# icameling/lidar_camera_calibration

Hardware: AMD Instinct MI355X
Metric: chessboard-corner frames/sec + max corner error (mm), VLP-16 cloud (higher is better)
Workload: dtype f32

## Files before the change

### include/ilcc_hip.h

```cpp
#ifndef ILCC_HIP_H_
#define ILCC_HIP_H_

#include <stdint.h>

#ifdef __cplusplus
extern "C" {
#endif

#define ILCC_MAX_CORNERS 256
#define ILCC_ABI_VERSION 5

enum {
  ILCC_OK = 0,
  ILCC_NO_ROI_POINTS = 1,
  ILCC_NO_CLUSTER = 2,
  ILCC_NO_PLANE = 3,
  ILCC_DEGENERATE_HIST = 4,
  ILCC_TOO_FEW_POINTS = 5,
  ILCC_BAD_ARGUMENT = 6,
  ILCC_CAPACITY = 7,
  ILCC_HIP_ERROR = 8,
  ILCC_IO_ERROR = 9,
  ILCC_BOARD_NOT_FOUND = 10,
  ILCC_AMBIGUOUS = 11
};

enum {
  ILCC_FLAG_TIE_OVERFLOW = 1,
  ILCC_FLAG_REFINE_CAPPED = 2,
  ILCC_FLAG_BORDER_RISK = 8,
  ILCC_FLAG_LOW_COVERAGE = 4
};

enum {
  ILCC_SOLVER_REFERENCE_LOCAL = 0,
  ILCC_SOLVER_GRID = 1
};

enum {
  ILCC_CLOUD_ROI = 0,
  ILCC_CLOUD_CLUSTER = 1,
  ILCC_CLOUD_CHESSBOARD = 2,
  ILCC_CLOUD_PCA = 3,
  ILCC_CLOUD_OPTIM = 4
};

typedef struct ilcc_params {
  double roi_half[3];
  double cluster_tol;
  int32_t cluster_min;
  int32_t cluster_max;
  double ransac_thresh;
  int32_t ransac_hyp;
  uint32_t ransac_seed;
  int32_t hist_bins;
  double gray_rate;
  double huber_delta;
  double grid_length;
  int32_t board_w;
  int32_t board_h;
  int32_t solver;
  int32_t phase_mode;
  int32_t max_iterations;
  int32_t grid_prune;
  int32_t n_th, n_ty, n_tz;
  double th_min, th_step;
  double ty_min, ty_step;
  double tz_min, tz_step;
  int32_t refine_div;
  int32_t refine_max_rounds;
  int32_t refine_th_margin;
  int32_t reserved0;
  double ambiguity_eps;
  double online_cluster_tol;
  double min_cell_coverage;
  double ransac_probability;
} ilcc_params;


typedef struct ilcc_result {
  int32_t status;
  int32_t n_points;
  int32_t n_roi, n_cluster, n_plane;
  int32_t n_black, n_gray, n_white;
  int32_t n_corners;
  int32_t phase;
  int32_t iters_a, iters_b;
  int32_t grid_index;
  int32_t found_board;
  float grid_cost;
  float plane[4];
  float pca[16];
  double gray_zone[2];
  double theta_t[3];
  double cost_a, cost_b;
  double sel_cost;
  double basin_margin;
  int32_t flags;
  int32_t grid_ties;
  int32_t cells_hit;
  int32_t n_oob;
  float corners[ILCC_MAX_CORNERS * 3];
} ilcc_result;

typedef struct ilcc_handle ilcc_handle;

typedef struct ilcc_timing {
  float roi_crop, cluster, ransac_plane, plane_frame_hist, grid_cost, refine_corners, total;
  uint32_t grid_cost_launches;
  double grid_cost_ms_sum;
  uint64_t grid_cost_evals_sum;
  uint64_t grid_cost_evals_nominal_sum;
  uint64_t grid_cost_evals_interior_sum;
  uint64_t grid_cost_box_evals_sum;
  double grid_cost_kernel_ms_sum;
  double grid_cost_full_ms_sum;
  double walk_order_ms_sum;
  double grid_cost_prepass_ms_sum;
  double grid_cost_locate_ms_sum;
  uint64_t batches;
  double stage_ms_sum[7];
  double roi_count_ms_sum;
  uint64_t online_second_tier_frames;
} ilcc_timing;

int32_t ilcc_abi_version(void);
const char* ilcc_strerror(int32_t status);
const char* ilcc_last_error(const ilcc_handle* h);

void ilcc_default_params(ilcc_params* p);

int32_t ilcc_set_chessboard_param(ilcc_params* p, const char* cam_yaml);

ilcc_handle* ilcc_create(int32_t device, const ilcc_params* p, uint32_t max_frames,
                         uint64_t max_total_points);
void ilcc_destroy(ilcc_handle* h);
int32_t ilcc_set_params(ilcc_handle* h, const ilcc_params* p);
int32_t ilcc_reserve(ilcc_handle* h, uint32_t labelled_points_per_frame, uint32_t roi_points_per_frame);

int32_t ilcc_extract(ilcc_handle* h, const float* xyzi, uint32_t n, const float click[3],
                     ilcc_result* out);

int32_t ilcc_extract_batch(ilcc_handle* h, const float* xyzi, const uint64_t* offsets,
                           uint32_t n_frames, const float* clicks, ilcc_result* out);

int32_t ilcc_extract_batch_device(ilcc_handle* h, const float* d_xyzi, const uint64_t* offsets,
                                  uint32_t n_frames, const float* d_clicks, ilcc_result* out);

int32_t ilcc_submit_batch_device(ilcc_handle* h, const float* d_xyzi, const uint64_t* offsets,
                                 uint32_t n_frames, const float* d_clicks, int32_t* ticket);
int32_t ilcc_submit_batch(ilcc_handle* h, const float* xyzi, const uint64_t* offsets, uint32_t n_frames,
                          const float* clicks, int32_t* ticket);
int32_t ilcc_wait(ilcc_handle* h, int32_t ticket, ilcc_result* out);
#define ILCC_RECORD_HEADER 20
int32_t ilcc_wait_records_device(ilcc_handle* h, int32_t ticket, ilcc_result* out, void* d_records, uint32_t n_corners,
                                 uint32_t tag_base);

enum { ILCC_RESULTS_FULL = 0, ILCC_RESULTS_COMPACT = 1 };
int32_t ilcc_set_result_mode(ilcc_handle* h, int32_t mode);
int32_t ilcc_wait_compact(ilcc_handle* h, int32_t ticket, float* records, uint64_t capacity_floats);
uint32_t ilcc_record_floats(const ilcc_handle* h, int32_t ticket);
int32_t ilcc_fetch_results(ilcc_handle* h, uint32_t first, uint32_t n, ilcc_result* out);

int32_t ilcc_chessboard_by_point_batch(ilcc_handle* h, const float* xyzi, const uint64_t* offsets,
                                       uint32_t n_frames, const float* points, int32_t min_plane_points,
                                       ilcc_result* out);
int32_t ilcc_submit_chessboard_by_point(ilcc_handle* h, const float* xyzi, const uint64_t* offsets, uint32_t n_frames,
                                        const float* points, int32_t* ticket);
int32_t ilcc_wait_chessboard_by_point(ilcc_handle* h, int32_t ticket, int32_t min_plane_points, ilcc_result* out);
int64_t ilcc_fetch_classes(ilcc_handle* h, uint32_t frame, uint8_t* out_class, uint64_t cap_points);

int64_t ilcc_fetch_cloud(ilcc_handle* h, uint32_t frame, int32_t which, float* out_xyzi,
                         uint64_t cap_points);
int64_t ilcc_fetch_labelled(ilcc_handle* h, uint32_t frame, float* out_yz, uint8_t* out_label,
                            uint64_t cap_points);
int64_t ilcc_fetch_walk(ilcc_handle* h, uint32_t frame, float* out_yz, uint8_t* out_label, uint64_t cap_points,
                        uint32_t counts[2]);

int32_t ilcc_grid_cost(ilcc_handle* h, const float* yz, const uint8_t* label, uint32_t m,
                       int32_t use_oob, float* cost_out, int32_t* best_index, float* best_cost);

int32_t ilcc_grid_solve(ilcc_handle* h, const float* yz, const uint8_t* label, uint32_t m, int32_t* grid_index, float* grid_cost,
                        int32_t lat[3], int32_t* phase, int64_t* cost_q, int64_t* alt_cost_q, int32_t* rounds, int32_t* hops,
                        int32_t* flags, int32_t* ties);

int32_t ilcc_pattern_refine(ilcc_handle* h, const float* yz, const uint8_t* label, uint32_t m, int32_t lat[3],
                            int32_t* phase, int64_t* cost_q, int64_t* alt_cost_q, int32_t* rounds, int32_t* hops);

int32_t ilcc_get_theta_t(ilcc_handle* h, const float* yz, const uint8_t* label, uint32_t m,
                         int32_t topleft_white, int32_t use_oob, double theta_t[3], double* cost,
                         int32_t* iterations);

#define ILCC_SOLVE_REC_DOUBLES 6
#define ILCC_SOLVE_REC_INTS 4
int32_t ilcc_debug_reference_solve(ilcc_handle* h, const float* yz, const uint8_t* label, const uint64_t* offsets,
                                   const int32_t* status_in, uint32_t n_frames, double* rec_f64, int32_t* rec_i32,
                                   ilcc_result* results, uint32_t* lds_points);

#define ILCC_TIMELINE_COLS 15
int32_t ilcc_debug_timeline_enable(ilcc_handle* h, int32_t on);
int32_t ilcc_debug_timeline_fetch(ilcc_handle* h, double* rows, uint32_t cap_rows);

int32_t ilcc_debug_separate_launches(ilcc_handle* h, int32_t on);

#define ILCC_CLUSTER_HOME_RULE 0
#define ILCC_CLUSTER_HOME_LDS 1
#define ILCC_CLUSTER_HOME_L2 2
#define ILCC_CLUSTER_LAUNCH_WORDS 6
int32_t ilcc_debug_cluster_home(ilcc_handle* h, int32_t home);
int32_t ilcc_debug_cluster_launch(const ilcc_handle* h, uint32_t out[ILCC_CLUSTER_LAUNCH_WORDS]);

void ilcc_get_timing(const ilcc_handle* h, ilcc_timing* t);
void ilcc_reset_timing(ilcc_handle* h);

int32_t ilcc_save_corners2txt(const float* corners_xyz, uint32_t n_corners, const char* filename);
int32_t ilcc_read_lidar_corners(const char* filename, uint32_t num, double* out_xyz);

#ifdef __cplusplus
}
#endif
#endif
```

### lidar_camera_calibration_amd/_native.py

```python
from __future__ import annotations

import ctypes as C
import os

import numpy as np

_HERE = os.path.dirname(os.path.abspath(__file__))
LIB_PATH = os.environ.get("ILCC_HIP_LIB") or os.path.join(_HERE, "libilcc_hip.so")
MAX_CORNERS = 256

OK, NO_ROI_POINTS, NO_CLUSTER, NO_PLANE, DEGENERATE_HIST, TOO_FEW_POINTS, BAD_ARGUMENT, CAPACITY, \
    HIP_ERROR, IO_ERROR, BOARD_NOT_FOUND, AMBIGUOUS = range(12)
FLAG_TIE_OVERFLOW, FLAG_REFINE_CAPPED, FLAG_LOW_COVERAGE, FLAG_BORDER_RISK = 1, 2, 4, 8
FLAGS_FP32_ONLY = FLAG_TIE_OVERFLOW | FLAG_BORDER_RISK
RECORD_HEADER = 20
TIMELINE_COLS = 15
COST_Q_ONE = float(1 << 40)
SOLVER_REFERENCE_LOCAL, SOLVER_GRID = 0, 1
CLOUD_ROI, CLOUD_CLUSTER, CLOUD_CHESSBOARD, CLOUD_PCA, CLOUD_OPTIM = range(5)

EXPORTS = [
    "ilcc_abi_version", "ilcc_strerror", "ilcc_last_error", "ilcc_default_params",
    "ilcc_set_chessboard_param", "ilcc_create", "ilcc_destroy", "ilcc_set_params", "ilcc_reserve", "ilcc_extract",
    "ilcc_extract_batch", "ilcc_extract_batch_device", "ilcc_submit_batch_device", "ilcc_submit_batch", "ilcc_wait", "ilcc_wait_records_device", "ilcc_fetch_cloud", "ilcc_fetch_labelled", "ilcc_fetch_walk", "ilcc_chessboard_by_point_batch", "ilcc_submit_chessboard_by_point", "ilcc_wait_chessboard_by_point", "ilcc_fetch_classes",
    "ilcc_grid_cost", "ilcc_grid_solve", "ilcc_pattern_refine", "ilcc_get_theta_t", "ilcc_get_timing", "ilcc_reset_timing",
    "ilcc_save_corners2txt", "ilcc_read_lidar_corners",
    "ilcc_set_result_mode", "ilcc_wait_compact", "ilcc_record_floats", "ilcc_fetch_results",
    "ilcc_debug_timeline_enable", "ilcc_debug_timeline_fetch", "ilcc_debug_separate_launches",
    "ilcc_debug_cluster_home", "ilcc_debug_cluster_launch", "ilcc_debug_reference_solve",
]
ABI_VERSION = 5
RESULTS_FULL, RESULTS_COMPACT = 0, 1
CLUSTER_HOME_RULE, CLUSTER_HOME_LDS, CLUSTER_HOME_L2 = 0, 1, 2
CLUSTER_LAUNCH_WORDS = 6
SOLVE_REC_DOUBLES, SOLVE_REC_INTS = 6, 4


class Params(C.Structure):
    _fields_ = [
        ("roi_half", C.c_double * 3),
        ("cluster_tol", C.c_double),
        ("cluster_min", C.c_int32),
        ("cluster_max", C.c_int32),
        ("ransac_thresh", C.c_double),
        ("ransac_hyp", C.c_int32),
        ("ransac_seed", C.c_uint32),
        ("hist_bins", C.c_int32),
        ("gray_rate", C.c_double),
        ("huber_delta", C.c_double),
        ("grid_length", C.c_double),
        ("board_w", C.c_int32),
        ("board_h", C.c_int32),
        ("solver", C.c_int32),
        ("phase_mode", C.c_int32),
        ("max_iterations", C.c_int32),
        ("grid_prune", C.c_int32),
        ("n_th", C.c_int32), ("n_ty", C.c_int32), ("n_tz", C.c_int32),
        ("th_min", C.c_double), ("th_step", C.c_double),
        ("ty_min", C.c_double), ("ty_step", C.c_double),
        ("tz_min", C.c_double), ("tz_step", C.c_double),
        ("refine_div", C.c_int32), ("refine_max_rounds", C.c_int32),
        ("refine_th_margin", C.c_int32), ("reserved0", C.c_int32),
        ("ambiguity_eps", C.c_double),
        ("online_cluster_tol", C.c_double),
        ("min_cell_coverage", C.c_double),
        ("ransac_probability", C.c_double),
    ]


class Result(C.Structure):
    _fields_ = [
        ("status", C.c_int32),
        ("n_points", C.c_int32),
        ("n_roi", C.c_int32), ("n_cluster", C.c_int32), ("n_plane", C.c_int32),
        ("n_black", C.c_int32), ("n_gray", C.c_int32), ("n_white", C.c_int32),
        ("n_corners", C.c_int32),
        ("phase", C.c_int32),
        ("iters_a", C.c_int32), ("iters_b", C.c_int32),
        ("grid_index", C.c_int32),
        ("found_board", C.c_int32),
        ("grid_cost", C.c_float),
        ("plane", C.c_float * 4),
        ("pca", C.c_float * 16),
        ("gray_zone", C.c_double * 2),
        ("theta_t", C.c_double * 3),
        ("cost_a", C.c_double), ("cost_b", C.c_double),
        ("sel_cost", C.c_double),
        ("basin_margin", C.c_double),
        ("flags", C.c_int32),
        ("grid_ties", C.c_int32),
        ("cells_hit", C.c_int32),
        ("n_oob", C.c_int32),
        ("corners", C.c_float * (MAX_CORNERS * 3)),
    ]

    def corners_array(self) -> np.ndarray:
        return np.ctypeslib.as_array(self.corners)[:3 * self.n_corners].reshape(-1, 3).copy()


class Timing(C.Structure):
    _fields_ = [
        ("roi_crop", C.c_float), ("cluster", C.c_float), ("ransac_plane", C.c_float),
        ("plane_frame_hist", C.c_float), ("grid_cost", C.c_float), ("refine_corners", C.c_float),
        ("total", C.c_float),
        ("grid_cost_launches", C.c_uint32),
        ("grid_cost_ms_sum", C.c_double),
        ("grid_cost_evals_sum", C.c_uint64),
        ("grid_cost_evals_nominal_sum", C.c_uint64),
        ("grid_cost_evals_interior_sum", C.c_uint64),
        ("grid_cost_box_evals_sum", C.c_uint64),
        ("grid_cost_kernel_ms_sum", C.c_double),
        ("grid_cost_full_ms_sum", C.c_double),
        ("walk_order_ms_sum", C.c_double),
        ("grid_cost_prepass_ms_sum", C.c_double),
        ("grid_cost_locate_ms_sum", C.c_double),
        ("batches", C.c_uint64),
        ("stage_ms_sum", C.c_double * 7),
        ("roi_count_ms_sum", C.c_double),
        ("online_second_tier_frames", C.c_uint64),
    ]


_lib = None


def lib():
    global _lib
    if _lib is None:
        if not os.path.exists(LIB_PATH):
            raise OSError(f"{LIB_PATH} not found: build it with `python -c 'import __graft_entry__ as g; "
                          "g.build()'` (hipcc --offload-arch=gfx950); there is no CPU fallback")
        L = C.CDLL(LIB_PATH)
        vp, fp = C.c_void_p, C.POINTER(C.c_float)
        pp, rp = C.POINTER(Params), C.POINTER(Result)
        L.ilcc_abi_version.restype = C.c_int32
        got = L.ilcc_abi_version()
        if got != ABI_VERSION:
            raise OSError(f"{LIB_PATH} implements ABI {got}, this package declares ABI {ABI_VERSION}: rebuild it "
                          "(python -c 'import __graft_entry__ as g; g.build()')")
        L.ilcc_strerror.argtypes = [C.c_int32]
        L.ilcc_strerror.restype = C.c_char_p
        L.ilcc_last_error.argtypes = [vp]
        L.ilcc_last_error.restype = C.c_char_p
        L.ilcc_default_params.argtypes = [pp]
        L.ilcc_set_chessboard_param.argtypes = [pp, C.c_char_p]
        L.ilcc_set_chessboard_param.restype = C.c_int32
        L.ilcc_create.argtypes = [C.c_int32, pp, C.c_uint32, C.c_uint64]
        L.ilcc_create.restype = vp
        L.ilcc_destroy.argtypes = [vp]
        L.ilcc_set_params.argtypes = [vp, pp]
        L.ilcc_set_params.restype = C.c_int32
        L.ilcc_reserve.argtypes = [vp, C.c_uint32, C.c_uint32]
        L.ilcc_reserve.restype = C.c_int32
        L.ilcc_extract.argtypes = [vp, fp, C.c_uint32, fp, rp]
        L.ilcc_extract.restype = C.c_int32
        L.ilcc_extract_batch.argtypes = [vp, fp, C.POINTER(C.c_uint64), C.c_uint32, fp, rp]
        L.ilcc_extract_batch.restype = C.c_int32
        L.ilcc_extract_batch_device.argtypes = [vp, vp, C.POINTER(C.c_uint64), C.c_uint32, vp, rp]
        L.ilcc_extract_batch_device.restype = C.c_int32
        L.ilcc_submit_batch_device.argtypes = [vp, vp, C.POINTER(C.c_uint64), C.c_uint32, vp, C.POINTER(C.c_int32)]
        L.ilcc_submit_batch_device.restype = C.c_int32
        L.ilcc_submit_batch.argtypes = [vp, vp, C.POINTER(C.c_uint64), C.c_uint32, vp, C.POINTER(C.c_int32)]
        L.ilcc_submit_batch.restype = C.c_int32
        L.ilcc_wait.argtypes = [vp, C.c_int32, rp]
        L.ilcc_wait.restype = C.c_int32
        L.ilcc_wait_records_device.argtypes = [vp, C.c_int32, rp, vp, C.c_uint32, C.c_uint32]
        L.ilcc_wait_records_device.restype = C.c_int32
        L.ilcc_chessboard_by_point_batch.argtypes = [vp, fp, C.POINTER(C.c_uint64), C.c_uint32, fp, C.c_int32, rp]
        L.ilcc_chessboard_by_point_batch.restype = C.c_int32
        L.ilcc_submit_chessboard_by_point.argtypes = [vp, C.c_void_p, C.POINTER(C.c_uint64), C.c_uint32, C.c_void_p, C.POINTER(C.c_int32)]
        L.ilcc_submit_chessboard_by_point.restype = C.c_int32
        L.ilcc_wait_chessboard_by_point.argtypes = [vp, C.c_int32, C.c_int32, rp]
        L.ilcc_wait_chessboard_by_point.restype = C.c_int32
        L.ilcc_fetch_classes.argtypes = [vp, C.c_uint32, C.POINTER(C.c_uint8), C.c_uint64]
        L.ilcc_fetch_classes.restype = C.c_int64
        L.ilcc_fetch_cloud.argtypes = [vp, C.c_uint32, C.c_int32, fp, C.c_uint64]
        L.ilcc_fetch_cloud.restype = C.c_int64
        L.ilcc_fetch_labelled.argtypes = [vp, C.c_uint32, fp, C.POINTER(C.c_uint8), C.c_uint64]
        L.ilcc_fetch_labelled.restype = C.c_int64
        L.ilcc_fetch_walk.argtypes = [vp, C.c_uint32, fp, C.POINTER(C.c_uint8), C.c_uint64, C.POINTER(C.c_uint32)]
        L.ilcc_fetch_walk.restype = C.c_int64
        L.ilcc_grid_cost.argtypes = [vp, fp, C.POINTER(C.c_uint8), C.c_uint32, C.c_int32, fp,
                                     C.POINTER(C.c_int32), fp]
        L.ilcc_grid_cost.restype = C.c_int32
        L.ilcc_grid_solve.argtypes = [vp, fp, C.POINTER(C.c_uint8), C.c_uint32, C.POINTER(C.c_int32), fp, C.POINTER(C.c_int32),
                                      C.POINTER(C.c_int32), C.POINTER(C.c_int64), C.POINTER(C.c_int64), C.POINTER(C.c_int32),
                                      C.POINTER(C.c_int32), C.POINTER(C.c_int32), C.POINTER(C.c_int32)]
        L.ilcc_grid_solve.restype = C.c_int32
        L.ilcc_pattern_refine.argtypes = [vp, fp, C.POINTER(C.c_uint8), C.c_uint32, C.POINTER(C.c_int32),
                                          C.POINTER(C.c_int32), C.POINTER(C.c_int64), C.POINTER(C.c_int64),
                                          C.POINTER(C.c_int32), C.POINTER(C.c_int32)]
        L.ilcc_pattern_refine.restype = C.c_int32
        L.ilcc_get_theta_t.argtypes = [vp, fp, C.POINTER(C.c_uint8), C.c_uint32, C.c_int32, C.c_int32,
                                       C.POINTER(C.c_double), C.POINTER(C.c_double), C.POINTER(C.c_int32)]
        L.ilcc_get_theta_t.restype = C.c_int32
        L.ilcc_get_timing.argtypes = [vp, C.POINTER(Timing)]
        L.ilcc_reset_timing.argtypes = [vp]
        L.ilcc_save_corners2txt.argtypes = [fp, C.c_uint32, C.c_char_p]
        L.ilcc_save_corners2txt.restype = C.c_int32
        L.ilcc_read_lidar_corners.argtypes = [C.c_char_p, C.c_uint32, C.POINTER(C.c_double)]
        L.ilcc_read_lidar_corners.restype = C.c_int32
        L.ilcc_set_result_mode.argtypes = [vp, C.c_int32]
        L.ilcc_set_result_mode.restype = C.c_int32
        L.ilcc_wait_compact.argtypes = [vp, C.c_int32, fp, C.c_uint64]
        L.ilcc_wait_compact.restype = C.c_int32
        L.ilcc_record_floats.argtypes = [vp, C.c_int32]
        L.ilcc_record_floats.restype = C.c_uint32
        L.ilcc_debug_timeline_enable.argtypes = [vp, C.c_int32]
        L.ilcc_debug_timeline_enable.restype = C.c_int32
        L.ilcc_debug_timeline_fetch.argtypes = [vp, C.POINTER(C.c_double), C.c_uint32]
        L.ilcc_debug_timeline_fetch.restype = C.c_int32
        if hasattr(L, "ilcc_debug_separate_launches"):
            L.ilcc_debug_separate_launches.argtypes = [vp, C.c_int32]
            L.ilcc_debug_separate_launches.restype = C.c_int32
        if hasattr(L, "ilcc_debug_cluster_home"):
            L.ilcc_debug_cluster_home.argtypes = [vp, C.c_int32]
            L.ilcc_debug_cluster_home.restype = C.c_int32
            L.ilcc_debug_cluster_launch.argtypes = [vp, C.POINTER(C.c_uint32)]
            L.ilcc_debug_cluster_launch.restype = C.c_int32
        L.ilcc_debug_reference_solve.argtypes = [vp, fp, C.POINTER(C.c_uint8), C.POINTER(C.c_uint64), C.POINTER(C.c_int32), C.c_uint32,
                                                 C.POINTER(C.c_double), C.POINTER(C.c_int32), rp, C.POINTER(C.c_uint32)]
        L.ilcc_debug_reference_solve.restype = C.c_int32
        L.ilcc_fetch_results.argtypes = [vp, C.c_uint32, C.c_uint32, rp]
        L.ilcc_fetch_results.restype = C.c_int32
        _lib = L
    return _lib


def default_params() -> Params:
    p = Params()
    lib().ilcc_default_params(C.byref(p))
    return p


def strerror(status: int) -> str:
    return lib().ilcc_strerror(int(status)).decode()


def fptr(a: np.ndarray):
    return a.ctypes.data_as(C.POINTER(C.c_float))
```

### lidar_camera_calibration_amd/csrc/ilcc_api.cpp

```cpp
#include <hip/hip_runtime.h>

#include <array>
#include <cmath>
#include <cstdio>
#include <cstdlib>
#include <cstring>
#include <mutex>
#include <new>
#include <string>
#include <vector>

#include "ilcc_internal.h"
#include "k15_seed.h"
#include "k6_common.h"
#include "k7_common.h"

using namespace ilcc;

namespace ilcc {
bool params_ok(const ilcc_params& p, std::string& why);
}

#ifndef ILCC_SLOTS
#define ILCC_SLOTS 4
#endif
constexpr int kSlots = ILCC_SLOTS;
constexpr int kStreams = 3;

enum BatchEvent {
  kEvStart,
  kEvCropCounted,
  kEvCropped,
  kEvClustered,
  kEvPlane,
  kEvLabelled,
  kEvWalkOrdered,
  kEvSeeded,
  kEvRefined,
  kEvAnchored,
  kEvPrepassed,
  kEvFullStart,
  kEvSearched,
  kEvEnd,
  kEvCount
};
static_assert(kEvCount == ILCC_TIMELINE_COLS - 1, "a timeline row is the slot and one time per event");

enum BatchKind { kRoiPipeline, kByPoint };

struct Slot {
  hipEvent_t ev[kEvCount]{};
  hipEvent_t done = nullptr;
  hipEvent_t late = nullptr;
  hipEvent_t k6_done = nullptr;
  bool allocated = false;
  float4* d_xyzi = nullptr;
  float* d_clicks = nullptr;
  uint64_t* d_off = nullptr;
  ilcc_result* d_res = nullptr;
  float4 *d_roi = nullptr, *d_cluster = nullptr, *d_board = nullptr, *d_pca = nullptr, *d_optim = nullptr;
  float2 *d_yz = nullptr, *d_walk_yz = nullptr;
  uint8_t* d_walk_lab = nullptr;
  uint32_t *d_walk_mi = nullptr, *d_walk_nrim = nullptr;
  uint8_t *d_lab = nullptr, *d_cls = nullptr;
  uint32_t *d_nlab = nullptr, *d_walk = nullptr, *d_counts = nullptr, *d_parent = nullptr, *d_count = nullptr;
  unsigned long long* d_masks = nullptr;
  uint32_t *d_hash_head = nullptr, *d_hash_next = nullptr;
  uint32_t *d_flags = nullptr, *d_nfinite = nullptr, *d_counts_fin = nullptr;
  uint32_t* h_online = nullptr;
  uint32_t* d_list = nullptr;
  void* d_list_frames = nullptr;
  GridPartial *d_partial = nullptr, *d_partial2 = nullptr, *d_partial3 = nullptr, *d_partial4 = nullptr;
  SolveRec* d_solverec = nullptr;
  uint32_t *d_bound = nullptr, *d_bound_sub = nullptr;
  uint32_t* d_tie_count = nullptr;
  GridPartial* d_tie_list = nullptr;
  unsigned long long* d_iters = nullptr;
  uint32_t *d_grp_alive = nullptr, *d_grp_mask = nullptr;
  size_t grp_alive_cap = 0, grp_mask_cap = 0;
  float* h_rec_dev = nullptr;
  unsigned long long* h_iters_dev = nullptr;
  float* h_rec = nullptr;
  ilcc_result* h_res = nullptr;
  unsigned long long* h_iters = nullptr;
  uint64_t* h_off = nullptr;
  std::vector<uint64_t> off;
  uint32_t n_frames = 0;
  bool busy = false, grid = false;
  BatchKind kind = kRoiPipeline;
  bool h_res_valid = false;
  bool compact = false;
  uint32_t rec_corners = 0;
};

struct ilcc_handle {
  int device = 0;
  ilcc_params p{};
  uint32_t max_frames = 0;
  uint64_t max_points = 0;
  uint32_t max_theta = 0;
  uint32_t crop_chunks_cap = 0;
  Slot slots[kSlots];
  hipStream_t stream[kStreams]{};
  uint64_t seq = 0;
  uint64_t stream_last[kStreams]{};
  hipEvent_t entry_done = nullptr;
  int next_slot = 0;
  int last_slot = -1;
  int k6_last = -1;
  float *d_cth = nullptr, *d_sth = nullptr, *d_ay = nullptr, *d_az = nullptr;
  float *d_cth2 = nullptr, *d_sth2 = nullptr, *d_ay2 = nullptr, *d_az2 = nullptr;
  GridTables grid{}, seed_grid{};
  SeedMap seed_map{2, 12, 6};
  double2* d_th_lattice = nullptr;
  size_t th_lattice_cap = 0;
  int32_t th_lat_lo = 0, th_lat_hi = 0, hop_y = 0, hop_z = 0;
  double* d_solve = nullptr;
  RefineOut* d_refine_io = nullptr;
  uint32_t grid_lds_points = 1024;
  uint64_t group_prepass_skipped = 0;
  uint32_t cluster_lds_points = 2048;
  uint32_t cluster_cells_cap = kClusterCellsMin;
  uint32_t list_grid = 1024;
  bool poisoned = false;
  int32_t result_mode = ILCC_RESULTS_FULL;
  ilcc_timing timing{};
  hipEvent_t tl_ref = nullptr;
  bool tl_on = false;
  bool separate_launches = false;
  ClusterLimits cluster_limits{};
  int32_t cluster_home = kClusterHomeRule;
  ClusterLaunch cluster_last{};
  std::vector<double> tl_rows;
  std::string err;
};

namespace {

thread_local std::string g_err;

#define HIP_TRY(h, expr)                                                                   \
  do {                                                                                     \
    hipError_t e_ = (expr);                                                                \
    if (e_ != hipSuccess) {                                                                \
      (h)->err = std::string(#expr) + ": " + hipGetErrorString(e_);                        \
      return ILCC_HIP_ERROR;                                                               \
    }                                                                                      \
  } while (0)

#define ILCC_TRY(expr)                   \
  do {                                   \
    const int32_t st_ = (expr);          \
    if (st_ != ILCC_OK) return st_;      \
  } while (0)

int32_t near_zero_index(double vmin, double step, int32_t n) {
  long c = std::lround(-vmin / step);
  if (c < 0) c = 0;
  if (c > n - 1) c = n - 1;
  return (int32_t)c;
}

int32_t sync_own(ilcc_handle* h, hipStream_t s) {
  HIP_TRY(h, hipEventRecord(h->entry_done, s));
  HIP_TRY(h, hipEventSynchronize(h->entry_done));
  return ILCC_OK;
}

int32_t sync_all(ilcc_handle* h) {
  for (hipStream_t s : h->stream)
    if (s) HIP_TRY(h, hipStreamSynchronize(s));
  return ILCC_OK;
}

int32_t upload_tables(ilcc_handle* h) {
  const ilcc_params& p = h->p;
  if ((uint32_t)p.n_th > h->max_theta || (uint32_t)p.n_ty > h->max_theta || (uint32_t)p.n_tz > h->max_theta) {
    h->err = "grid axis longer than the handle's table capacity";
    return ILCC_CAPACITY;
  }
  hipStream_t st = h->stream[0];
  std::vector<float> cth(p.n_th), sth(p.n_th), ay(p.n_ty), az(p.n_tz);
  const double g = p.grid_length;
  for (int k = 0; k < p.n_th; ++k) {
    const double th = p.th_min + k * p.th_step;
    cth[k] = (float)(std::cos(th) / g);
    sth[k] = (float)(std::sin(th) / g);
  }
  for (int a = 0; a < p.n_ty; ++a) ay[a] = (float)(((p.ty_min + a * p.ty_step) + p.board_w * g / 2.0) / g);
  for (int b = 0; b < p.n_tz; ++b) az[b] = (float)(((p.tz_min + b * p.tz_step) + p.board_h * g / 2.0) / g);
  HIP_TRY(h, hipMemcpyAsync(h->d_cth, cth.data(), sizeof(float) * p.n_th, hipMemcpyHostToDevice, st));
  HIP_TRY(h, hipMemcpyAsync(h->d_sth, sth.data(), sizeof(float) * p.n_th, hipMemcpyHostToDevice, st));
  HIP_TRY(h, hipMemcpyAsync(h->d_ay, ay.data(), sizeof(float) * p.n_ty, hipMemcpyHostToDevice, st));
  HIP_TRY(h, hipMemcpyAsync(h->d_az, az.data(), sizeof(float) * p.n_tz, hipMemcpyHostToDevice, st));
#ifndef ILCC_SEED_THETAS
#define ILCC_SEED_THETAS 5
#endif
#ifndef ILCC_REFINE_RADIUS_DIV
#define ILCC_REFINE_RADIUS_DIV 3
#endif
  SeedMap& map = h->seed_map;
  map.stride_th = std::max(2, p.n_th / ILCC_SEED_THETAS);
  map.stride_t = std::max(1, std::min(p.n_ty, p.n_tz) / 8);
  map.off_th = map.stride_th / 2;
  std::vector<float> cth2, sth2, ay2, az2;
  for (int k = map.off_th; k < p.n_th; k += map.stride_th) {
    cth2.push_back(cth[k]);
    sth2.push_back(sth[k]);
  }
  for (int a = 0; a < p.n_ty; a += map.stride_t) ay2.push_back(ay[a]);
  for (int b = 0; b < p.n_tz; b += map.stride_t) az2.push_back(az[b]);
  GridTables& full = h->grid;
  full = GridTables{h->d_cth, h->d_sth, h->d_ay, h->d_az, p.n_th, p.n_ty, p.n_tz, near_zero_index(p.th_min, p.th_step, p.n_th),
                    near_zero_index(p.ty_min, p.ty_step, p.n_ty), near_zero_index(p.tz_min, p.tz_step, p.n_tz)};
  GridTables& seed = h->seed_grid;
  seed = GridTables{h->d_cth2, h->d_sth2, h->d_ay2, h->d_az2, (int32_t)cth2.size(), (int32_t)ay2.size(), (int32_t)az2.size(), 0, 0, 0};
  seed.c_th = std::min(std::max(full.c_th / map.stride_th, 0), seed.n_th - 1);
  seed.c_ty = std::min(full.c_ty / map.stride_t, seed.n_ty - 1);
  seed.c_tz = std::min(full.c_tz / map.stride_t, seed.n_tz - 1);
  if (seed.n_th > 0) {
    HIP_TRY(h, hipMemcpyAsync(h->d_cth2, cth2.data(), sizeof(float) * cth2.size(), hipMemcpyHostToDevice, st));
    HIP_TRY(h, hipMemcpyAsync(h->d_sth2, sth2.data(), sizeof(float) * sth2.size(), hipMemcpyHostToDevice, st));
    HIP_TRY(h, hipMemcpyAsync(h->d_ay2, ay2.data(), sizeof(float) * ay2.size(), hipMemcpyHostToDevice, st));
    HIP_TRY(h, hipMemcpyAsync(h->d_az2, az2.data(), sizeof(float) * az2.size(), hipMemcpyHostToDevice, st));
  }
  {
    const int div = p.refine_div > 0 ? p.refine_div : 1;
    h->th_lat_lo = -p.refine_th_margin * div;
    h->th_lat_hi = (p.n_th - 1 + p.refine_th_margin) * div;
    const size_t n = (size_t)(h->th_lat_hi - h->th_lat_lo) + 1;
    if (n > h->th_lattice_cap) {
      if (h->d_th_lattice) (void)hipFree(h->d_th_lattice);
      h->d_th_lattice = nullptr;
      h->th_lattice_cap = 0;
      HIP_TRY(h, hipMalloc((void**)&h->d_th_lattice, sizeof(double2) * n));
      h->th_lattice_cap = n;
    }
    std::vector<double2> tab(n);
    for (size_t i = 0; i < n; ++i) {
      const double th = p.th_min + (double)(h->th_lat_lo + (int64_t)i) * (p.th_step / (double)div);
      tab[i] = make_double2(std::cos(th), std::sin(th));
    }
    HIP_TRY(h, hipMemcpyAsync(h->d_th_lattice, tab.data(), sizeof(double2) * n, hipMemcpyHostToDevice, st));
    const int32_t sst = sync_own(h, st);
    if (sst != ILCC_OK) return sst;
    h->hop_y = (int32_t)std::lround(p.grid_length / (p.ty_step / (double)div));
    h->hop_z = (int32_t)std::lround(p.grid_length / (p.tz_step / (double)div));
  }
  return sync_own(h, st);
}

struct Buffer {
  void** ptr;
  size_t bytes;
};
template <class T>
Buffer buffer(T*& p, size_t count) { return {reinterpret_cast<void**>(&p), sizeof(T) * count}; }

auto handle_buffers(ilcc_handle* h) {
  const size_t mt = h->max_theta;
  return std::array{buffer(h->d_cth, mt),  buffer(h->d_sth, mt),  buffer(h->d_ay, mt),  buffer(h->d_az, mt),
                    buffer(h->d_cth2, mt), buffer(h->d_sth2, mt), buffer(h->d_ay2, mt), buffer(h->d_az2, mt),
                    buffer(h->d_solve, 8), buffer(h->d_refine_io, 1), buffer(h->d_th_lattice, 0) };
}

auto slot_device_buffers(const ilcc_handle* h, Slot& sl) {
  const size_t np = h->max_points, mf = h->max_frames, chunks = h->crop_chunks_cap, mt = h->max_theta;
  return std::array{
      buffer(sl.d_xyzi, np),
      buffer(sl.d_clicks, 3 * mf),
      buffer(sl.d_off, mf + 1),
      buffer(sl.d_res, mf),
      buffer(sl.d_roi, np),
      buffer(sl.d_cluster, np),
      buffer(sl.d_board, np),
      buffer(sl.d_pca, np),
      buffer(sl.d_optim, np),
      buffer(sl.d_yz, np),
      buffer(sl.d_walk_yz, np),
      buffer(sl.d_walk_lab, np),
      buffer(sl.d_walk_mi, mf),
      buffer(sl.d_walk_nrim, mf),
      buffer(sl.d_lab, np),
      buffer(sl.d_cls, np),
      buffer(sl.d_nlab, mf),
      buffer(sl.d_walk, mf),
      buffer(sl.d_counts, chunks),
      buffer(sl.d_counts_fin, chunks),
      buffer(sl.d_flags, mf),
      buffer(sl.d_nfinite, mf),
      buffer(sl.d_list, mf + 1),
      Buffer{&sl.d_list_frames, 64 * mf},
      buffer(sl.d_masks, chunks * (kCropChunk / 64)),
      buffer(sl.d_parent, np),
      buffer(sl.d_count, np),
      buffer(sl.d_hash_head, mf * kClusterHashSize),
      buffer(sl.d_hash_next, np),
      buffer(sl.d_partial, mf * mt),
      buffer(sl.d_partial2, mf * mt),
      buffer(sl.d_partial3, mf * mt),
      buffer(sl.d_partial4, mf * 4),
      buffer(sl.d_solverec, 2 * mf),
      buffer(sl.d_bound, mf),
      buffer(sl.d_bound_sub, mf),
      buffer(sl.d_tie_count, mf),
      buffer(sl.d_tie_list, mf * kTieCap),
      buffer(sl.d_iters, kBatchWords),
      buffer(sl.d_grp_alive, 0),
      buffer(sl.d_grp_mask, 0),
  };
}

auto slot_pinned_buffers(const ilcc_handle* h, Slot& sl) {
  const size_t mf = h->max_frames;
  return std::array{
      buffer(sl.h_res, mf),
      buffer(sl.h_rec, mf * (ILCC_RECORD_HEADER + 3 * ILCC_MAX_CORNERS)),
      buffer(sl.h_iters, kBatchWords),
      buffer(sl.h_off, mf + 1),
      buffer(sl.h_online, 2 * mf),
  };
}

struct SlotEvent {
  hipEvent_t* ev;
  unsigned flags;
};
auto slot_events(Slot& sl) {
  std::array<SlotEvent, kEvCount + 3> evs;
  for (int k = 0; k < kEvCount; ++k) evs[k] = {&sl.ev[k], hipEventDefault};
  evs[kEvCount] = {&sl.done, hipEventDisableTiming};
  evs[kEvCount + 1] = {&sl.late, hipEventDisableTiming};
  evs[kEvCount + 2] = {&sl.k6_done, hipEventDisableTiming};
  return evs;
}

void free_slot(const ilcc_handle* h, Slot& sl) {
  for (const Buffer& b : slot_device_buffers(h, sl))
    if (*b.ptr) (void)hipFree(*b.ptr);
  for (const Buffer& b : slot_pinned_buffers(h, sl))
    if (*b.ptr) (void)hipHostFree(*b.ptr);
  for (const SlotEvent& e : slot_events(sl))
    if (*e.ev) (void)hipEventDestroy(*e.ev);
  sl = Slot{};
}

void warn_hw_queues_once() {
  static std::once_flag once;
  std::call_once(once, [] {
    const char* v = std::getenv("GPU_MAX_HW_QUEUES");
    if (!v || std::atoi(v) >= kStreams + 1) return;
    std::fprintf(stderr,
                 "libilcc_hip: GPU_MAX_HW_QUEUES=%s: with fewer than %d hardware queues two of the handle's stage streams "
                 "(or one and the host's stream) share a queue and serialise (the library does not modify the "
                 "environment)\n", v, kStreams + 1);
  });
}

struct GroupPrepassPlan {
  bool box = false;
  bool on = false;
  uint32_t groups = 0, words = 0;
};
GroupPrepassPlan group_prepass_plan(const ilcc_params& p) {
  GroupPrepassPlan g;
  const bool box = p.grid_prune != 0 && 3.0 * p.ty_step < 0.9 * p.grid_length && 3.0 * p.tz_step < 0.9 * p.grid_length;
  const double gl = p.grid_length;
  const double ty_hi = p.ty_min + (p.n_ty - 1) * p.ty_step, tz_hi = p.tz_min + (p.n_tz - 1) * p.tz_step;
  const bool centre_in = p.ty_min > -0.45 * p.board_w * gl && ty_hi < 0.45 * p.board_w * gl && p.tz_min > -0.45 * p.board_h * gl &&
                         tz_hi < 0.45 * p.board_h * gl;
  const uint32_t n_tiles = (uint32_t)grid_tiles(p.n_ty, p.n_tz);
  g.box = box;
  g.on = box && p.n_th >= kThetaGroup && centre_in && n_tiles <= (uint32_t)kBoxTilesMax;
  g.groups = (uint32_t)((p.n_th + kThetaGroup - 1) / kThetaGroup);
  g.words = (n_tiles + 31u) / 32u;
  return g;
}

int32_t size_group_prepass(ilcc_handle* h, Slot& sl) {
  const GroupPrepassPlan g = group_prepass_plan(h->p);
  if (!g.on) return ILCC_OK;
  const size_t need_alive = (size_t)h->max_frames * g.groups, need_mask = need_alive * g.words;
  if (need_alive > sl.grp_alive_cap) {
    if (sl.d_grp_alive) (void)hipFree(sl.d_grp_alive);
    sl.d_grp_alive = nullptr;
    sl.grp_alive_cap = 0;
    HIP_TRY(h, hipMalloc((void**)&sl.d_grp_alive, sizeof(uint32_t) * need_alive));
    sl.grp_alive_cap = need_alive;
  }
  if (need_mask > sl.grp_mask_cap) {
    if (sl.d_grp_mask) (void)hipFree(sl.d_grp_mask);
    sl.d_grp_mask = nullptr;
    sl.grp_mask_cap = 0;
    HIP_TRY(h, hipMalloc((void**)&sl.d_grp_mask, sizeof(uint32_t) * need_mask));
    sl.grp_mask_cap = need_mask;
  }
  return ILCC_OK;
}

int32_t alloc_slot_parts(ilcc_handle* h, Slot& sl) {
  for (const SlotEvent& e : slot_events(sl)) HIP_TRY(h, hipEventCreateWithFlags(e.ev, e.flags));
  for (const Buffer& b : slot_device_buffers(h, sl))
    if (b.bytes) HIP_TRY(h, hipMalloc(b.ptr, b.bytes));
  for (const Buffer& b : slot_pinned_buffers(h, sl)) HIP_TRY(h, hipHostMalloc(b.ptr, b.bytes, hipHostMallocDefault));
  HIP_TRY(h, hipHostGetDevicePointer((void**)&sl.h_rec_dev, sl.h_rec, 0));
  HIP_TRY(h, hipHostGetDevicePointer((void**)&sl.h_iters_dev, sl.h_iters, 0));
  return size_group_prepass(h, sl);
}

int32_t alloc_slot(ilcc_handle* h, Slot& sl) {
  if (sl.allocated) return ILCC_OK;
  const int32_t st = alloc_slot_parts(h, sl);
  if (st != ILCC_OK) {
    free_slot(h, sl);
    return st;
  }
  sl.allocated = true;
  return ILCC_OK;
}

Ctx make_ctx(ilcc_handle* h, Slot& sl, const float4* d_xyzi, const float* d_clicks, uint32_t n_frames,
             uint32_t crop_chunks) {
  Ctx c{};
  c.xyzi = d_xyzi;
  c.off = sl.d_off;
  c.clicks = d_clicks;
  c.n_frames = n_frames;
  c.crop_chunks = crop_chunks;
  c.res = sl.d_res;
  c.roi = sl.d_roi;
  c.cluster = sl.d_cluster;
  c.board = sl.d_board;
  c.pca = sl.d_pca;
  c.optim = sl.d_optim;
  c.yz = sl.d_yz;
  c.lab = sl.d_lab;
  c.cls = sl.d_cls;
  c.n_lab = sl.d_nlab;
  c.walk_stride = sl.d_walk;
  c.walk_yz = sl.d_walk_yz;
  c.walk_lab = sl.d_walk_lab;
  c.walk_mi = sl.d_walk_mi;
  c.walk_nrim = sl.d_walk_nrim;
  c.crop_counts = sl.d_counts;
  c.crop_masks = sl.d_masks;
  c.uf_parent = sl.d_parent;
  c.uf_count = sl.d_count;
  c.uf_hash_head = sl.d_hash_head;
  c.uf_hash_next = sl.d_hash_next;
  c.cluster_lds_points = h->cluster_lds_points;
  c.cluster_cells_cap = h->cluster_cells_cap;
  c.wide = 0u;
  c.cluster_bits = cluster_bits_default();
  c.online_tier = 0u;
  c.online_window = 0.f;
  c.frame_flags = sl.d_flags;
  c.n_finite = sl.d_nfinite;
  c.crop_fin = sl.d_counts_fin;
  c.list_count = sl.d_list;
  c.list = sl.d_list + 1;
  c.list_frames = sl.d_list_frames;
  c.list_grid = h->list_grid;
  c.partial = sl.d_partial;
  c.solve_rec = sl.d_solverec;
  c.grid_blocks = (uint32_t)h->p.n_th;
  c.grid_lds_points = h->grid_lds_points;
  c.grid_bound = sl.d_bound;
  c.grid_bound_sub = sl.d_bound_sub;
  c.tie_count = sl.d_tie_count;
  c.tie_list = sl.d_tie_list;
  c.grid_iters = sl.d_iters;
  c.grid = h->grid;
  c.th_lattice = h->d_th_lattice;
  c.th_lat_lo = h->th_lat_lo;
  c.th_lat_hi = h->th_lat_hi;
  c.refine_hop_y = h->hop_y;
  c.refine_hop_z = h->hop_z;
  c.p = h->p;
  return c;
}

int32_t check_offsets(ilcc_handle* h, const uint64_t* offsets, uint32_t n_frames) {
  if (!offsets || n_frames == 0) {
    h->err = "no frames";
    return ILCC_BAD_ARGUMENT;
  }
  if (n_frames > h->max_frames) {
    h->err = "n_frames exceeds the handle's max_frames";
    return ILCC_CAPACITY;
  }
  if (offsets[0] != 0) {
    h->err = "offsets[0] must be 0";
    return ILCC_BAD_ARGUMENT;
  }
  for (uint32_t f = 0; f < n_frames; ++f)
    if (offsets[f + 1] < offsets[f] || offsets[f + 1] - offsets[f] > 0x7FFFFFFFull) {
      h->err = "offsets must be non-decreasing, frames < 2^31 points";
      return ILCC_BAD_ARGUMENT;
    }
  if (offsets[n_frames] > h->max_points) {
    h->err = "total points exceed the handle's max_total_points";
    return ILCC_CAPACITY;
  }
  return ILCC_OK;
}

int take_stream(ilcc_handle* h) {
  const int k = (int)(h->seq % kStreams);
  h->stream_last[k] = ++h->seq;
  return k;
}

hipStream_t late_stream(const ilcc_handle* h) {
  int best = 0;
  for (int k = 1; k < kStreams; ++k)
    if (h->stream_last[k] < h->stream_last[best]) best = k;
  return h->stream[best];
}

void fit_cluster_lds(ilcc_handle* h) {
  while (cluster_lds_bytes(h->cluster_lds_points, h->cluster_cells_cap, cluster_bits_online()) > (size_t)kClusterLdsMax && h->cluster_lds_points > 0)
    h->cluster_lds_points = h->cluster_lds_points > 512u ? h->cluster_lds_points - 512u : 0u;
}

uint32_t board_corners(const ilcc_params& p) { return (uint32_t)((p.board_w - 1) * (p.board_h - 1)); }
size_t trimmed_bytes(uint32_t n_corners) { return offsetof(ilcc_result, corners) + sizeof(float) * 3 * (size_t)n_corners; }

hipError_t copy_results_trimmed(ilcc_result* dst, const ilcc_result* d_src, uint32_t n_frames, uint32_t n_corners, hipStream_t s) {
  if (n_frames == 0) return hipSuccess;
  return hipMemcpy2DAsync(dst, sizeof(ilcc_result), d_src, sizeof(ilcc_result), trimmed_bytes(n_corners), n_frames,
                          hipMemcpyDeviceToHost, s);
}

#ifndef ILCC_SEED_POINTS
#define ILCC_SEED_POINTS 128
#endif
#ifndef ILCC_BOX_POINTS
#define ILCC_BOX_POINTS 48
#endif
constexpr int kAnchorRadius = 1;
#ifndef ILCC_ANCHOR_ROUNDS
#define ILCC_ANCHOR_ROUNDS 2
#endif
constexpr int kAnchorRounds = ILCC_ANCHOR_ROUNDS;


GridPass whole_grid_pass(const Ctx& c, const GridTables& t, GridPartial* out) {
  GridPass g{};
  g.t = t;
  g.out = out;
  g.blocks = (uint32_t)t.n_th;
  g.bound = c.grid_bound;
  return g;
}

GridSeed full_table_records(const GridPartial* records, uint32_t blocks) { return GridSeed{records, blocks, SeedMap{1, 1, 0}}; }

GridPass seed_pass(const ilcc_handle* h, const Slot& sl, const Ctx& c) {
  GridPass g = whole_grid_pass(c, h->seed_grid, sl.d_partial2);
  g.walk_limit = (uint32_t)ILCC_SEED_POINTS;
  g.bound = c.grid_bound_sub;
  return g;
}

GridPass refine_pass(const ilcc_handle* h, const Slot& sl, const Ctx& c, int32_t refine_radius) {
  GridPass g = whole_grid_pass(c, h->grid, sl.d_partial3);
  g.seed = GridSeed{sl.d_partial2, (uint32_t)h->seed_grid.n_th, h->seed_map};
  g.window_tiles = h->seed_map.stride_t > 2 * kTile ? 4 : 2;
  g.radius_th = (refine_radius / kRefineThetaStride) * kRefineThetaStride;
  g.step_th = kRefineThetaStride;
  g.blocks = std::min((uint32_t)(2 * (g.radius_th / kRefineThetaStride) + 1), h->max_theta);
  g.walk_limit = (uint32_t)ILCC_SEED_POINTS;
  g.bound = c.grid_bound_sub;
  return g;
}

GridPass anchor_pass(const ilcc_handle* h, const Ctx& c, const GridSeed& seed, GridPartial* out) {
  GridPass g = whole_grid_pass(c, h->grid, out);
  g.seed = seed;
  g.radius_th = kAnchorRadius;
  g.blocks = 2 * kAnchorRadius + 1;
  return g;
}

GridPass full_pass(const ilcc_handle* h, const Ctx& c, const GridSeed& seed) {
  GridPass g = whole_grid_pass(c, h->grid, c.partial);
  g.seed = seed;
  g.collect_ties = 1u;
  return g;
}

LocatePlan locate_plan(const ilcc_handle* h, const Slot& sl, const Ctx& c) {
  LocatePlan lp{};
  lp.seed = h->seed_grid;
  lp.map = h->seed_map;
  lp.refine_radius = std::max(1, h->seed_map.stride_th / ILCC_REFINE_RADIUS_DIV);
  lp.sample_min = (uint32_t)ILCC_SEED_POINTS;
  lp.sample_cap = std::max((uint32_t)ILCC_SEED_POINTS, ((c.grid_lds_points >> 3) + 63u) & ~63u);
  lp.out = sl.d_partial4;
  return lp;
}

int32_t enqueue_locate_launches(ilcc_handle* h, Slot& sl, const Ctx& c, hipStream_t s, int32_t refine_radius, GridSeed& located) {
  launch_grid_cost(c, seed_pass(h, sl, c), s, 1, nullptr, true);
  HIP_TRY(h, hipEventRecord(sl.ev[kEvSeeded], s));
  const GridPass refine = refine_pass(h, sl, c, refine_radius);
  launch_grid_cost(c, refine, s, 1, nullptr, true);
  HIP_TRY(h, hipEventRecord(sl.ev[kEvRefined], s));
  located = full_table_records(refine.out, refine.blocks);
  GridPartial* const ping[2] = {sl.d_partial4, sl.d_partial2};
  for (int round = 0; round < kAnchorRounds; ++round) {
    const GridPass anchor = anchor_pass(h, c, located, ping[round & 1]);
    launch_anchor(c, anchor, s);
    located = full_table_records(anchor.out, anchor.blocks);
  }
  return ILCC_OK;
}

int32_t enqueue_grid_search(ilcc_handle* h, Slot& sl, const Ctx& c, hipStream_t s, uint32_t n_frames, bool chain, bool walk_laid_out = false) {
  const bool prune = h->p.grid_prune != 0;
  if (!walk_laid_out) launch_walk_order(c, s);
  HIP_TRY(h, hipEventRecord(sl.ev[kEvWalkOrdered], s));
  GridSeed located{};
  if (h->seed_grid.n_th > 0 && h->p.n_th >= 8 && h->p.n_ty >= 8 && h->p.n_tz >= 8) {
    const LocatePlan lp = locate_plan(h, sl, c);
    const bool fused = n_frames >= (uint32_t)kLocateMinFrames && lp.seed.n_th <= 16 &&
                       locate_lds_bytes(lp.sample_cap, h->grid.n_ty, h->grid.n_tz, lp.seed.n_ty, lp.seed.n_tz) <= (size_t)kLocateLdsMax;
    if (fused) {
      launch_locate(c, s, lp);
      HIP_TRY(h, hipEventRecord(sl.ev[kEvSeeded], s));
      HIP_TRY(h, hipEventRecord(sl.ev[kEvRefined], s));
      located = full_table_records(lp.out, 1);
    } else {
      ILCC_TRY(enqueue_locate_launches(h, sl, c, s, lp.refine_radius, located));
    }
  } else {
    HIP_TRY(h, hipEventRecord(sl.ev[kEvSeeded], s));
    HIP_TRY(h, hipEventRecord(sl.ev[kEvRefined], s));
  }
  HIP_TRY(h, hipEventRecord(sl.ev[kEvAnchored], s));
  GridPass full = full_pass(h, c, located);
  const GroupPrepassPlan gp = group_prepass_plan(h->p);
  full.box_points = gp.box ? (uint32_t)ILCC_BOX_POINTS : 0u;
  if (full.box_points != 0u && gp.on && (size_t)n_frames * gp.groups <= sl.grp_alive_cap &&
      (size_t)n_frames * gp.groups * gp.words <= sl.grp_mask_cap) {
    full.grp_alive = sl.d_grp_alive;
    full.grp_mask = sl.d_grp_mask;
    full.grp_count = gp.groups;
    full.grp_words = gp.words;
    launch_group_prepass(c, full, s);
  } else if (full.box_points != 0u && gp.on) {
    if (h->group_prepass_skipped++ == 0) h->err = "note: k6_group_prepass skipped (mask buffers smaller than this batch needs): slower, results unaffected";
  }
  HIP_TRY(h, hipEventRecord(sl.ev[kEvPrepassed], s));
  const int si = (int)(&sl - h->slots);
  if (chain && h->k6_last >= 0 && h->k6_last != si && h->slots[h->k6_last].busy)
    HIP_TRY(h, hipStreamWaitEvent(s, h->slots[h->k6_last].k6_done, 0));
  HIP_TRY(h, hipEventRecord(sl.ev[kEvFullStart], s));
  launch_grid_cost(c, full, s, 1, nullptr, prune);
  if (chain) {
    HIP_TRY(h, hipEventRecord(sl.k6_done, s));
    h->k6_last = si;
  }
  return ILCC_OK;
}

int32_t enqueue_impl(ilcc_handle* h, int si, hipStream_t s, const float4* d_xyzi, const uint64_t* offsets, uint32_t n_frames,
                     const float* d_clicks, BatchKind kind) {
  Slot& sl = h->slots[si];
  uint64_t max_n = 0;
  for (uint32_t f = 0; f < n_frames; ++f) max_n = std::max<uint64_t>(max_n, offsets[f + 1] - offsets[f]);
  uint32_t chunks = (uint32_t)((max_n + kCropChunk - 1) / kCropChunk);
  if (chunks == 0) chunks = 1;
  if ((uint64_t)chunks * n_frames > (uint64_t)h->crop_chunks_cap) {
    h->err = "crop chunk table too small for this (very ragged) batch";
    return ILCC_CAPACITY;
  }
  sl.off.assign(offsets, offsets + n_frames + 1);
  sl.n_frames = n_frames;
  std::memcpy(sl.h_off, sl.off.data(), sizeof(uint64_t) * (n_frames + 1));
  HIP_TRY(h, hipMemcpyAsync(sl.d_off, sl.h_off, sizeof(uint64_t) * (n_frames + 1), hipMemcpyHostToDevice, s));
  Ctx c = make_ctx(h, sl, d_xyzi, d_clicks, n_frames, chunks);
  HIP_TRY(h, hipEventRecord(sl.ev[kEvStart], s));
  if (kind == kRoiPipeline) {
    launch_roi_crop(c, s, sl.ev[kEvCropCounted], !h->separate_launches && n_frames >= (uint32_t)kCropFrameMinFrames);
    HIP_TRY(h, hipEventRecord(sl.ev[kEvCropped], s));
    h->cluster_last = launch_cluster(c, s, h->cluster_limits, h->cluster_home);
  } else {
    c.p.cluster_tol = c.p.online_cluster_tol;
    c.wide = 1u;
    Ctx t1 = c;
    t1.online_tier = 1u;
    t1.online_window = 1.25f;
    t1.p.roi_half[0] = t1.p.roi_half[1] = t1.p.roi_half[2] = (double)t1.online_window;
    t1.cluster_bits = cluster_bits_online();
    launch_roi_crop(t1, s, sl.ev[kEvCropCounted]);
    HIP_TRY(h, hipEventRecord(sl.ev[kEvCropped], s));
    h->cluster_last = launch_cluster(t1, s, h->cluster_limits, h->cluster_home);
    Ctx t2 = c;
    t2.online_tier = 2u;
    t2.p.roi_half[0] = t2.p.roi_half[1] = t2.p.roi_half[2] = (double)INFINITY;
    launch_roi_crop(t2, s, nullptr);
    (void)launch_cluster(t2, s, h->cluster_limits, h->cluster_home);
    HIP_TRY(h, hipMemcpyAsync(sl.h_online, sl.d_flags, sizeof(uint32_t) * n_frames, hipMemcpyDeviceToHost, s));
    HIP_TRY(h, hipMemcpyAsync(sl.h_online + h->max_frames, sl.d_nfinite, sizeof(uint32_t) * n_frames, hipMemcpyDeviceToHost, s));
  }
  HIP_TRY(h, hipEventRecord(sl.ev[kEvClustered], s));
  sl.grid = kind == kRoiPipeline && h->p.solver == ILCC_SOLVER_GRID;
  const bool one_launch = !h->separate_launches && front_end_fusable(c);
  if (one_launch) {
    launch_front_end(c, s, sl.grid);
    HIP_TRY(h, hipEventRecord(sl.ev[kEvPlane], s));
  } else {
    launch_ransac_plane(c, s);
    HIP_TRY(h, hipEventRecord(sl.ev[kEvPlane], s));
    launch_plane_frame_hist(c, s);
  }
  HIP_TRY(h, hipEventRecord(sl.ev[kEvLabelled], s));
  if (sl.grid) {
    ILCC_TRY(enqueue_grid_search(h, sl, c, s, n_frames, true, one_launch));
  }
  HIP_TRY(h, hipEventRecord(sl.ev[kEvSearched], s));
  if (kind == kRoiPipeline) {
    if (sl.grid) {
      launch_pattern_refine(c, s);
    } else {
      launch_reference_solve(c, s);
    }
    launch_corners(c, s, solve_slots(c.p));
  }
  HIP_TRY(h, hipEventRecord(sl.ev[kEvEnd], s));
  HIP_TRY(h, hipGetLastError());
  sl.compact = h->result_mode == ILCC_RESULTS_COMPACT;
  sl.rec_corners = board_corners(h->p);
  if (sl.compact) {
    launch_pack_records(sl.d_res, n_frames, sl.rec_corners, 0u, sl.h_rec_dev, s);
  } else {
    HIP_TRY(h, copy_results_trimmed(sl.h_res, sl.d_res, n_frames, sl.rec_corners, s));
  }
  launch_store_to_host(sl.d_iters, sl.h_iters_dev, sizeof(unsigned long long) * kBatchWords, s);
  HIP_TRY(h, hipGetLastError());
  HIP_TRY(h, hipEventRecord(sl.done, s));
  sl.busy = true;
  sl.kind = kind;
  return ILCC_OK;
}

int32_t enqueue(ilcc_handle* h, int si, hipStream_t s, const float4* d_xyzi, const uint64_t* offsets, uint32_t n_frames,
                const float* d_clicks, BatchKind kind) {
  if (h->poisoned) {
    h->err = "handle unusable: a failed ilcc_set_params could not restore the device tables";
    return ILCC_HIP_ERROR;
  }
  const int32_t st = enqueue_impl(h, si, s, d_xyzi, offsets, n_frames, d_clicks, kind);
  if (st != ILCC_OK) {
    const std::string why = h->err;
    (void)hipStreamSynchronize(s);
    (void)hipGetLastError();
    h->slots[si].busy = false;
    h->err = why;
  }
  return st;
}

int32_t run_late(ilcc_handle* h, Slot& sl, hipStream_t s) {
  HIP_TRY(h, hipEventRecord(sl.late, s));
  HIP_TRY(h, hipEventSynchronize(sl.late));
  return ILCC_OK;
}

int32_t ensure_full(ilcc_handle* h, Slot& sl) {
  if (sl.h_res_valid) return ILCC_OK;
  const hipStream_t s = late_stream(h);
  HIP_TRY(h, copy_results_trimmed(sl.h_res, sl.d_res, sl.n_frames, sl.rec_corners, s));
  ILCC_TRY(run_late(h, sl, s));
  sl.h_res_valid = true;
  return ILCC_OK;
}


int32_t wait_batch(ilcc_handle* h, Slot& sl, bool want_compact, float* d_records, uint32_t n_corners, uint32_t tag_base) {
  HIP_TRY(h, hipSetDevice(h->device));
  HIP_TRY(h, hipEventSynchronize(sl.done));
  const bool pack_now = want_compact && !sl.compact;
  const hipStream_t ls = late_stream(h);
  if (d_records) launch_pack_records(sl.d_res, sl.n_frames, n_corners, tag_base, d_records, ls);
  if (pack_now) launch_pack_records(sl.d_res, sl.n_frames, sl.rec_corners, 0u, sl.h_rec_dev, ls);
  if (d_records || pack_now) {
    ILCC_TRY(run_late(h, sl, ls));
  }
  sl.busy = false;
  sl.h_res_valid = !sl.compact;
  h->last_slot = (int)(&sl - h->slots);
  return ILCC_OK;
}

size_t record_floats(const Slot& sl) { return (size_t)ILCC_RECORD_HEADER + 3 * (size_t)sl.rec_corners; }

int32_t hand_over(ilcc_handle* h, Slot& sl, ilcc_result* out, float* out_compact) {
  if (out) {
    ILCC_TRY(ensure_full(h, sl));
    const size_t row = trimmed_bytes(sl.rec_corners);
    for (uint32_t f = 0; f < sl.n_frames; ++f) std::memcpy(&out[f], &sl.h_res[f], row);
  }
  if (out_compact) std::memcpy(out_compact, sl.h_rec, sizeof(float) * sl.n_frames * record_floats(sl));
  return ILCC_OK;
}

struct BatchCounts {
  uint32_t max_lab = 0, max_roi = 0;
  uint64_t evals = 0;
};
BatchCounts count_batch(const ilcc_handle* h, const Slot& sl) {
  BatchCounts n;
  for (uint32_t f = 0; f < sl.n_frames; ++f) {
    int32_t status, n_roi;
    uint32_t m;
    if (sl.h_res_valid) {
      const ilcc_result& r = sl.h_res[f];
      status = r.status;
      n_roi = r.n_roi;
      m = (uint32_t)(r.n_black + r.n_white);
    } else {
      const float* r = sl.h_rec + (size_t)f * record_floats(sl);
      status = (int32_t)r[0];
      n_roi = (int32_t)r[19];
      m = (uint32_t)r[13] + (uint32_t)r[14];
    }
    if (n_roi > 0 && (uint32_t)n_roi <= (uint32_t)kClusterLdsPointsMax) n.max_roi = std::max(n.max_roi, (uint32_t)n_roi);
    if (status != ILCC_OK && status != ILCC_AMBIGUOUS) continue;
    n.max_lab = std::max(n.max_lab, m);
    n.evals += (uint64_t)m * (uint64_t)h->p.n_th * h->p.n_ty * h->p.n_tz;
  }
  return n;
}

int32_t account_timing(ilcc_handle* h, const Slot& sl, uint64_t evals) {
  auto span = [&](BatchEvent from, BatchEvent to, float& ms_out) { return hipEventElapsedTime(&ms_out, sl.ev[from], sl.ev[to]); };
  float ms[6];
  const BatchEvent stage[7] = {kEvStart, kEvCropped, kEvClustered, kEvPlane, kEvLabelled, kEvSearched, kEvEnd};
  for (int k = 0; k < 6; ++k) HIP_TRY(h, span(stage[k], stage[k + 1], ms[k]));
  float k6k[6] = {0.f, 0.f, 0.f, 0.f, 0.f, 0.f};
  if (sl.grid) {
    const BatchEvent part[6] = {kEvLabelled, kEvWalkOrdered, kEvSeeded, kEvRefined, kEvAnchored, kEvPrepassed};
    for (int k = 0; k < 5; ++k) HIP_TRY(h, span(part[k], part[k + 1], k6k[k]));
    HIP_TRY(h, span(kEvFullStart, kEvSearched, k6k[5]));
    float pre = 0.f;
    HIP_TRY(h, span(kEvLabelled, kEvPrepassed, pre));
    ms[4] = pre + k6k[5];
  }
  float tot = 0;
  HIP_TRY(h, span(kEvStart, kEvEnd, tot));
  if (h->tl_on && h->tl_ref && sl.grid) {
    h->tl_rows.push_back((double)(&sl - h->slots));
    for (hipEvent_t e : sl.ev) {
      float t = 0.f;
      HIP_TRY(h, hipEventElapsedTime(&t, h->tl_ref, e));
      h->tl_rows.push_back((double)t);
    }
  }
  ilcc_timing& t = h->timing;
  t.roi_crop = ms[0];
  t.cluster = ms[1];
  t.ransac_plane = ms[2];
  t.plane_frame_hist = ms[3];
  t.grid_cost = ms[4];
  t.refine_corners = ms[5];
  t.total = tot;
  t.batches += 1;
  for (int k = 0; k < 6; ++k) t.stage_ms_sum[k] += ms[k];
  t.stage_ms_sum[6] += tot;
  {
    float cnt = 0.f;
    HIP_TRY(h, span(kEvStart, kEvCropCounted, cnt));
    t.roi_count_ms_sum += cnt;
  }
  if (sl.grid) {
    t.grid_cost_launches += 1;
    t.grid_cost_ms_sum += ms[4];
    t.walk_order_ms_sum += k6k[0];
    t.grid_cost_kernel_ms_sum += (double)k6k[1] + k6k[2] + k6k[3] + k6k[4] + k6k[5];
    t.grid_cost_locate_ms_sum += (double)k6k[1] + k6k[2] + k6k[3];
    t.grid_cost_prepass_ms_sum += k6k[4];
    t.grid_cost_full_ms_sum += k6k[5];
    t.grid_cost_evals_nominal_sum += evals;
    unsigned long long iters = 0;
    unsigned long long iters_in = 0;
    for (int k = 0; k < kIterSlots; ++k) {
      iters += sl.h_iters[k];
      iters_in += sl.h_iters[kIterSlots + k];
      t.grid_cost_box_evals_sum += sl.h_iters[2 * kIterSlots + k];
    }
    t.grid_cost_evals_sum += (uint64_t)iters * grid_cost_evals_per_count();
    t.grid_cost_evals_interior_sum += (uint64_t)iters_in * grid_cost_evals_per_count();
  }
  return ILCC_OK;
}

uint32_t lds_capacity(uint32_t need, uint32_t step, uint32_t lo, uint32_t hi) {
  return std::min(hi, std::max(lo, (need + step - 1u) & ~(step - 1u)));
}
uint32_t grid_lds_capacity(uint32_t labelled_points) { return lds_capacity(labelled_points, 256u, 1024u, (uint32_t)kGridLdsPointsMax); }
uint32_t cluster_lds_capacity(uint32_t roi_points, uint32_t lo) { return lds_capacity(roi_points, 512u, lo, (uint32_t)kClusterLdsPointsMax); }
uint32_t cluster_cells_capacity(uint64_t cells) {
  const uint32_t need = (uint32_t)std::min<uint64_t>(cells, (uint64_t)kClusterCellsMax);
  return lds_capacity(need, 256u, (uint32_t)kClusterCellsMin, (uint32_t)kClusterCellsMax);
}
void raise_capacities(ilcc_handle* h, uint32_t grid_points, uint32_t cluster_points, uint32_t cluster_cells) {
  h->grid_lds_points = std::max(h->grid_lds_points, grid_points);
  h->cluster_lds_points = std::max(h->cluster_lds_points, cluster_points);
  h->cluster_cells_cap = std::max(h->cluster_cells_cap, cluster_cells);
  fit_cluster_lds(h);
}

constexpr int kGridStaticLds = 3072;
constexpr uint32_t grid_points_two_per_cu(int n_ty, int n_tz) {
  const int64_t room = (int64_t)kCuLdsBytes / 2 - kGridStaticLds - (int64_t)grid_lds_bytes(0, n_ty, n_tz);
  return room > 0 ? (uint32_t)(room / (int64_t)grid_lds_bytes(1, 0, 0)) & ~255u : 0u;
}
static_assert(grid_points_two_per_cu(40, 40) == 6400, "BASELINE config 2 (the default grid: 40 x 40 translations)");
static_assert(grid_points_two_per_cu(129, 129) == 6400, "BASELINE config 5 (129 x 129 translations)");
void grow_capacities(ilcc_handle* h, const BatchCounts& n, uint64_t cells_needed) {
  const uint32_t two_per_cu = grid_points_two_per_cu(h->p.n_ty, h->p.n_tz);
  raise_capacities(h, std::min(grid_lds_capacity(n.max_lab), std::max(1024u, two_per_cu)), cluster_lds_capacity(n.max_roi, 0u),
                   cluster_cells_capacity(cells_needed + cells_needed / 8));
}

int32_t finish(ilcc_handle* h, Slot& sl, ilcc_result* out, float* out_compact = nullptr, float* d_records = nullptr,
               uint32_t n_corners = 0, uint32_t tag_base = 0) {
  ILCC_TRY(wait_batch(h, sl, out_compact != nullptr, d_records, n_corners, tag_base));
  ILCC_TRY(hand_over(h, sl, out, out_compact));
  const BatchCounts n = count_batch(h, sl);
  ILCC_TRY(account_timing(h, sl, n.evals));
  grow_capacities(h, n, sl.h_iters[3 * kIterSlots]);
  return ILCC_OK;
}

int32_t run_batch(ilcc_handle* h, BatchKind kind, bool on_device, const float* xyzi, const uint64_t* offsets, uint32_t n_frames,
                  const float* clicks, int32_t* ticket, ilcc_result* out) {
  HIP_TRY(h, hipSetDevice(h->device));
  ILCC_TRY(check_offsets(h, offsets, n_frames));
  const int si = ticket ? h->next_slot : 0;
  Slot& sl = h->slots[si];
  if (sl.busy) {
    h->err = ticket ? "every pipeline slot holds a batch: wait for the oldest ticket first" : "synchronous call while ticket 0 is in flight";
    return ticket ? ILCC_CAPACITY : ILCC_BAD_ARGUMENT;
  }
  if (ticket) ILCC_TRY(alloc_slot(h, sl));
  const hipStream_t s = h->stream[take_stream(h)];
  if (!on_device) {
    if (offsets[n_frames] > 0)
      HIP_TRY(h, hipMemcpyAsync(sl.d_xyzi, xyzi, sizeof(float4) * offsets[n_frames], hipMemcpyHostToDevice, s));
    HIP_TRY(h, hipMemcpyAsync(sl.d_clicks, clicks, sizeof(float) * 3 * n_frames, hipMemcpyHostToDevice, s));
    xyzi = reinterpret_cast<const float*>(sl.d_xyzi);
    clicks = sl.d_clicks;
  }
  ILCC_TRY(enqueue(h, si, s, reinterpret_cast<const float4*>(xyzi), offsets, n_frames, clicks, kind));
  if (!ticket) return finish(h, sl, out);
  *ticket = si;
  h->next_slot = (si + 1) % kSlots;
  return ILCC_OK;
}


const Slot* busy_slot(const ilcc_handle* h, int32_t ticket) {
  return h && ticket >= 0 && ticket < kSlots && h->slots[ticket].busy ? &h->slots[ticket] : nullptr;
}

Slot* ticket_slot(ilcc_handle* h, int32_t ticket, const char* fn, BatchKind kind, bool args_ok) {
  if (!h) return nullptr;
  Slot* sl = const_cast<Slot*>(busy_slot(h, ticket));
  if (!args_ok || !sl) {
    h->err = std::string(fn) + ": bad argument or no batch in flight under this ticket";
    return nullptr;
  }
  if (sl->kind != kind) {
    h->err = std::string(fn) + (sl->kind == kByPoint ? ": this ticket came from ilcc_submit_chessboard_by_point: wait with ilcc_wait_chessboard_by_point"
                                                     : ": this ticket came from ilcc_submit_batch[_device]: wait with ilcc_wait / ilcc_wait_compact / ilcc_wait_records_device");
    return nullptr;
  }
  return sl;
}

bool any_batch_in_flight(ilcc_handle* h, const char* fn) {
  for (const Slot& sl : h->slots)
    if (sl.busy) {
      h->err = std::string(fn) + " with a batch in flight: ilcc_wait first";
      return true;
    }
  return false;
}

void finish_chessboard_by_point(ilcc_handle* h, Slot& sl, uint32_t n_frames, int32_t min_plane_points, ilcc_result* out) {
  for (uint32_t f = 0; f < n_frames; ++f)
    if (sl.h_online[f] == 0u && out[f].status != ILCC_NO_ROI_POINTS) out[f].n_roi = (int32_t)sl.h_online[h->max_frames + f];
  for (uint32_t f = 0; f < n_frames; ++f) h->timing.online_second_tier_frames += sl.h_online[f] != 0u ? 1u : 0u;
  for (uint32_t f = 0; f < n_frames; ++f)
    if (out[f].status == ILCC_OK && (out[f].n_plane < min_plane_points || !out[f].found_board)) {
      out[f].status = ILCC_BOARD_NOT_FOUND;
      sl.h_res[f].status = ILCC_BOARD_NOT_FOUND;
    }
}


int32_t fetch_slot(ilcc_handle* h, uint32_t first, uint32_t n, Slot*& slot) {
  if (!h || h->last_slot < 0) return ILCC_BAD_ARGUMENT;
  Slot& sl = h->slots[h->last_slot];
  if (sl.busy || first > sl.n_frames || n > sl.n_frames - first) {
    h->err = "fetch: no completed batch, or the frames asked for exceed it";
    return ILCC_BAD_ARGUMENT;
  }
  HIP_TRY(h, hipSetDevice(h->device));
  slot = &sl;
  return ILCC_OK;
}

int64_t fetch_labelled_points(const float2* d_yz, const uint8_t* d_lab, uint32_t n, float* out_yz, uint8_t* out_label, uint64_t cap_points) {
  const uint64_t m = std::min<uint64_t>(n, cap_points);
  if (m > 0 && ((out_yz && hipMemcpy(out_yz, d_yz, sizeof(float2) * m, hipMemcpyDeviceToHost) != hipSuccess) ||
                (out_label && hipMemcpy(out_label, d_lab, m, hipMemcpyDeviceToHost) != hipSuccess)))
    return -(int64_t)ILCC_HIP_ERROR;
  return (int64_t)n;
}

int32_t stage_labelled(ilcc_handle* h, hipStream_t s, const float* yz, const uint8_t* label, uint32_t m) {
  if (!h || (m > 0 && (!yz || !label))) return ILCC_BAD_ARGUMENT;
  if (m > h->max_points) {
    h->err = "more points than the handle holds";
    return ILCC_CAPACITY;
  }
  Slot& sl = h->slots[0];
  if (sl.busy) {
    h->err = "diagnostic entry while ticket 0 is in flight";
    return ILCC_BAD_ARGUMENT;
  }
  HIP_TRY(h, hipSetDevice(h->device));
  const uint64_t off[2] = {0, m};
  ilcc_result r;
  std::memset(&r, 0, sizeof(r));
  r.status = ILCC_OK;
  HIP_TRY(h, hipMemcpyAsync(sl.d_off, off, sizeof(off), hipMemcpyHostToDevice, s));
  HIP_TRY(h, hipMemcpyAsync(sl.d_res, &r, sizeof(r), hipMemcpyHostToDevice, s));
  HIP_TRY(h, hipMemcpyAsync(sl.d_nlab, &m, sizeof(m), hipMemcpyHostToDevice, s));
  const uint32_t stride = walk_stride(m);
  HIP_TRY(h, hipMemcpyAsync(sl.d_walk, &stride, sizeof(stride), hipMemcpyHostToDevice, s));
  if (m > 0) {
    HIP_TRY(h, hipMemcpyAsync(sl.d_yz, yz, sizeof(float2) * m, hipMemcpyHostToDevice, s));
    HIP_TRY(h, hipMemcpyAsync(sl.d_lab, label, m, hipMemcpyHostToDevice, s));
  }
  ILCC_TRY(sync_own(h, s));
  sl.n_frames = 0;
  return ILCC_OK;
}

Ctx diagnostic_ctx(ilcc_handle* h, Slot& sl, uint32_t m) {
  Ctx c = make_ctx(h, sl, nullptr, nullptr, 1, 1);
  uint32_t lds = 1024;
  while (lds < m && lds < (uint32_t)kGridLdsPointsMax) lds <<= 1;
  c.grid_lds_points = std::max(c.grid_lds_points, lds);
  return c;
}

}

namespace ilcc {
void set_global_error(const std::string& s) { g_err = s; }
HandleView handle_view(const ilcc_handle* h) { return HandleView{h->device, h->p, h->max_frames, h->max_points}; }
int32_t handle_fail(ilcc_handle* h, int32_t code, const std::string& what) {
  h->err = what;
  return code;
}
}

extern "C" {

const char* ilcc_last_error(const ilcc_handle* h) { return h ? h->err.c_str() : g_err.c_str(); }

ilcc_handle* ilcc_create(int32_t device, const ilcc_params* p, uint32_t max_frames, uint64_t max_total_points) {
  g_err.clear();
  int ndev = 0;
  if (hipGetDeviceCount(&ndev) != hipSuccess || ndev == 0) {
    g_err = "no HIP device: libilcc_hip has no CPU fallback";
    return nullptr;
  }
  if (!p || max_frames == 0 || max_total_points == 0) {
    g_err = "bad arguments to ilcc_create";
    return nullptr;
  }
  std::string why;
  if (!params_ok(*p, why)) {
    g_err = why;
    return nullptr;
  }
  ilcc_handle* h = new (std::nothrow) ilcc_handle();
  if (!h) return nullptr;
  h->p = *p;
  h->max_frames = max_frames;
  h->max_points = max_total_points;
  h->max_theta = 4096;
  h->crop_chunks_cap =
      (uint32_t)std::min<uint64_t>(0xFFFFFFFFull, max_total_points / kCropChunk + (uint64_t)max_frames + 1);
  auto fail = [&](const std::string& what) {
    g_err = what;
    ilcc_destroy(h);
    return (ilcc_handle*)nullptr;
  };
  hipError_t e;
  if (device >= 0) {
    if ((e = hipSetDevice(device)) != hipSuccess) return fail(std::string("hipSetDevice: ") + hipGetErrorString(e));
    h->device = device;
  } else {
    (void)hipGetDevice(&h->device);
  }
  {
    int cus = 0;
    if (hipDeviceGetAttribute(&cus, hipDeviceAttributeMultiprocessorCount, h->device) == hipSuccess && cus > 0)
      h->list_grid = (uint32_t)(4 * cus);
  }
  if ((e = set_kernel_attributes_k2()) != hipSuccess || (e = set_kernel_attributes_k6()) != hipSuccess ||
      (e = set_kernel_attributes_k7a()) != hipSuccess || (e = set_kernel_attributes_k7r()) != hipSuccess)
    return fail(std::string("hipFuncSetAttribute(MaxDynamicSharedMemorySize): ") + hipGetErrorString(e));
  if ((e = cluster_limits(h->device, &h->cluster_limits)) != hipSuccess)
    return fail(std::string("cluster_limits: ") + hipGetErrorString(e));
  for (const Buffer& b : handle_buffers(h))
    if (b.bytes && (e = hipMalloc(b.ptr, b.bytes)) != hipSuccess) return fail(std::string("hipMalloc: ") + hipGetErrorString(e));
  warn_hw_queues_once();
  for (hipStream_t& s : h->stream)
    if ((e = hipStreamCreateWithFlags(&s, hipStreamNonBlocking)) != hipSuccess)
      return fail(std::string("hipStreamCreateWithFlags: ") + hipGetErrorString(e));
  if ((e = hipEventCreateWithFlags(&h->entry_done, hipEventDisableTiming)) != hipSuccess)
    return fail(std::string("hipEventCreateWithFlags: ") + hipGetErrorString(e));
  if (alloc_slot(h, h->slots[0]) != ILCC_OK) return fail(h->err);
  if (upload_tables(h) != ILCC_OK) return fail(h->err);
  return h;
}

void ilcc_destroy(ilcc_handle* h) {
  if (!h) return;
  for (hipStream_t s : h->stream)
    if (s) (void)hipStreamSynchronize(s);
  for (Slot& sl : h->slots) free_slot(h, sl);
  for (hipStream_t s : h->stream)
    if (s) (void)hipStreamDestroy(s);
  for (const Buffer& b : handle_buffers(h))
    if (*b.ptr) (void)hipFree(*b.ptr);
  if (h->tl_ref) (void)hipEventDestroy(h->tl_ref);
  if (h->entry_done) (void)hipEventDestroy(h->entry_done);
  delete h;
}

int32_t ilcc_set_params(ilcc_handle* h, const ilcc_params* p) {
  if (!h || !p) return ILCC_BAD_ARGUMENT;
  std::string why;
  if (!params_ok(*p, why)) {
    h->err = why;
    return ILCC_BAD_ARGUMENT;
  }
  if (any_batch_in_flight(h, "ilcc_set_params")) return ILCC_BAD_ARGUMENT;
  ILCC_TRY(sync_all(h));
  const ilcc_params old = h->p;
  h->p = *p;
  int32_t st = upload_tables(h);
  for (Slot& sl : h->slots)
    if (st == ILCC_OK && sl.allocated) st = size_group_prepass(h, sl);
  if (st != ILCC_OK) {
    const std::string why = h->err;
    h->p = old;
    if (upload_tables(h) != ILCC_OK) h->poisoned = true;
    h->err = why;
  }
  return st;
}

int32_t ilcc_reserve(ilcc_handle* h, uint32_t labelled_points_per_frame, uint32_t roi_points_per_frame) {
  if (!h || any_batch_in_flight(h, "ilcc_reserve")) return ILCC_BAD_ARGUMENT;
  raise_capacities(h, grid_lds_capacity(labelled_points_per_frame), cluster_lds_capacity(roi_points_per_frame, (uint32_t)kClusterLdsPointsMin),
                   cluster_cells_capacity(roi_points_per_frame / 4u));
  return ILCC_OK;
}

int32_t ilcc_set_result_mode(ilcc_handle* h, int32_t mode) {
  if (!h || (mode != ILCC_RESULTS_FULL && mode != ILCC_RESULTS_COMPACT) || any_batch_in_flight(h, "ilcc_set_result_mode")) return ILCC_BAD_ARGUMENT;
  h->result_mode = mode;
  return ILCC_OK;
}


int32_t ilcc_submit_batch_device(ilcc_handle* h, const float* d_xyzi, const uint64_t* offsets, uint32_t n_frames,
                                 const float* d_clicks, int32_t* ticket) {
  if (!h || !d_xyzi || !d_clicks || !ticket) return ILCC_BAD_ARGUMENT;
  return run_batch(h, kRoiPipeline, true, d_xyzi, offsets, n_frames, d_clicks, ticket, nullptr);
}

int32_t ilcc_submit_batch(ilcc_handle* h, const float* xyzi, const uint64_t* offsets, uint32_t n_frames, const float* clicks,
                          int32_t* ticket) {
  if (!h || !xyzi || !clicks || !ticket) return ILCC_BAD_ARGUMENT;
  return run_batch(h, kRoiPipeline, false, xyzi, offsets, n_frames, clicks, ticket, nullptr);
}

int32_t ilcc_extract_batch_device(ilcc_handle* h, const float* d_xyzi, const uint64_t* offsets,
                                  uint32_t n_frames, const float* d_clicks, ilcc_result* out) {
  if (!h || !d_xyzi || !d_clicks || !out) return ILCC_BAD_ARGUMENT;
  return run_batch(h, kRoiPipeline, true, d_xyzi, offsets, n_frames, d_clicks, nullptr, out);
}

int32_t ilcc_extract_batch(ilcc_handle* h, const float* xyzi, const uint64_t* offsets, uint32_t n_frames,
                           const float* clicks, ilcc_result* out) {
  if (!h || !xyzi || !clicks || !out) return ILCC_BAD_ARGUMENT;
  return run_batch(h, kRoiPipeline, false, xyzi, offsets, n_frames, clicks, nullptr, out);
}

int32_t ilcc_extract(ilcc_handle* h, const float* xyzi, uint32_t n, const float click[3], ilcc_result* out) {
  const uint64_t off[2] = {0, n};
  return ilcc_extract_batch(h, xyzi, off, 1, click, out);
}

int32_t ilcc_chessboard_by_point_batch(ilcc_handle* h, const float* xyzi, const uint64_t* offsets, uint32_t n_frames,
                                       const float* points, int32_t min_plane_points, ilcc_result* out) {
  if (!h || !xyzi || !points || !out) return ILCC_BAD_ARGUMENT;
  ILCC_TRY(run_batch(h, kByPoint, false, xyzi, offsets, n_frames, points, nullptr, out));
  finish_chessboard_by_point(h, h->slots[0], n_frames, min_plane_points, out);
  return ILCC_OK;
}

int32_t ilcc_submit_chessboard_by_point(ilcc_handle* h, const float* xyzi, const uint64_t* offsets, uint32_t n_frames,
                                        const float* points, int32_t* ticket) {
  if (!h || !xyzi || !points || !ticket) return ILCC_BAD_ARGUMENT;
  return run_batch(h, kByPoint, false, xyzi, offsets, n_frames, points, ticket, nullptr);
}


int32_t ilcc_wait(ilcc_handle* h, int32_t ticket, ilcc_result* out) {
  Slot* sl = ticket_slot(h, ticket, "ilcc_wait", kRoiPipeline, out != nullptr);
  return sl ? finish(h, *sl, out) : ILCC_BAD_ARGUMENT;
}

int32_t ilcc_wait_records_device(ilcc_handle* h, int32_t ticket, ilcc_result* out, void* d_records, uint32_t n_corners,
                                 uint32_t tag_base) {
  Slot* sl = ticket_slot(h, ticket, "ilcc_wait_records_device", kRoiPipeline, d_records && n_corners <= ILCC_MAX_CORNERS);
  return sl ? finish(h, *sl, out, nullptr, static_cast<float*>(d_records), n_corners, tag_base) : ILCC_BAD_ARGUMENT;
}

uint32_t ilcc_record_floats(const ilcc_handle* h, int32_t ticket) {
  const Slot* sl = busy_slot(h, ticket);
  return sl ? (uint32_t)record_floats(*sl) : 0u;
}

int32_t ilcc_wait_compact(ilcc_handle* h, int32_t ticket, float* records, uint64_t capacity_floats) {
  Slot* sl = ticket_slot(h, ticket, "ilcc_wait_compact", kRoiPipeline, records != nullptr);
  if (!sl) return ILCC_BAD_ARGUMENT;
  const uint64_t need = (uint64_t)sl->n_frames * record_floats(*sl);
  if (capacity_floats < need) {
    h->err = "ilcc_wait_compact: the batch's records need " + std::to_string(need) + " floats, the buffer holds " +
             std::to_string(capacity_floats) + " (the batch stays in flight)";
    return ILCC_BAD_ARGUMENT;
  }
  return finish(h, *sl, nullptr, records);
}

int32_t ilcc_wait_chessboard_by_point(ilcc_handle* h, int32_t ticket, int32_t min_plane_points, ilcc_result* out) {
  Slot* sl = ticket_slot(h, ticket, "ilcc_wait_chessboard_by_point", kByPoint, out != nullptr);
  if (!sl) return ILCC_BAD_ARGUMENT;
  ILCC_TRY(finish(h, *sl, out));
  finish_chessboard_by_point(h, *sl, sl->n_frames, min_plane_points, out);
  return ILCC_OK;
}


int32_t ilcc_fetch_results(ilcc_handle* h, uint32_t first, uint32_t n, ilcc_result* out) {
  Slot* slp = nullptr;
  ILCC_TRY(out ? fetch_slot(h, first, n, slp) : ILCC_BAD_ARGUMENT);
  Slot& sl = *slp;
  ILCC_TRY(ensure_full(h, sl));
  const size_t row = trimmed_bytes(sl.rec_corners);
  for (uint32_t f = 0; f < n; ++f) std::memcpy(&out[f], &sl.h_res[first + f], row);
  return ILCC_OK;
}

int64_t ilcc_fetch_classes(ilcc_handle* h, uint32_t frame, uint8_t* out_class, uint64_t cap_points) {
  Slot* slp = nullptr;
  const int32_t st = fetch_slot(h, frame, 1, slp);
  if (st != ILCC_OK) return -(int64_t)st;
  Slot& sl = *slp;
  if (ensure_full(h, sl) != ILCC_OK) return -(int64_t)ILCC_HIP_ERROR;
  const ilcc_result& r = sl.h_res[frame];
  const int64_t n = (r.status == ILCC_OK || r.status == ILCC_AMBIGUOUS || r.status == ILCC_BOARD_NOT_FOUND) ? r.n_plane : 0;
  const int64_t m = std::min<int64_t>(n, (int64_t)cap_points);
  if (m > 0 && out_class &&
      hipMemcpy(out_class, sl.d_cls + sl.off[frame], (size_t)m, hipMemcpyDeviceToHost) != hipSuccess)
    return -(int64_t)ILCC_HIP_ERROR;
  return n;
}

int64_t ilcc_fetch_cloud(ilcc_handle* h, uint32_t frame, int32_t which, float* out_xyzi, uint64_t cap_points) {
  Slot* slp = nullptr;
  const int32_t st = fetch_slot(h, frame, 1, slp);
  if (st != ILCC_OK) return -(int64_t)st;
  Slot& sl = *slp;
  if (ensure_full(h, sl) != ILCC_OK) return -(int64_t)ILCC_HIP_ERROR;
  const ilcc_result& r = sl.h_res[frame];
  const float4* src = nullptr;
  int64_t n = 0;
  switch (which) {
    case ILCC_CLOUD_ROI: src = sl.d_roi; n = r.n_roi; break;
    case ILCC_CLOUD_CLUSTER: src = sl.d_cluster; n = r.n_cluster; break;
    case ILCC_CLOUD_CHESSBOARD: src = sl.d_board; n = r.n_plane; break;
    case ILCC_CLOUD_PCA:
      src = sl.d_pca;
      n = (r.status == ILCC_OK || r.status == ILCC_AMBIGUOUS || r.status == ILCC_DEGENERATE_HIST || r.status == ILCC_BOARD_NOT_FOUND) ? r.n_plane : 0;
      break;
    case ILCC_CLOUD_OPTIM: src = sl.d_optim; n = (r.status == ILCC_OK || r.status == ILCC_AMBIGUOUS) ? r.n_plane : 0; break;
    default: return -(int64_t)ILCC_BAD_ARGUMENT;
  }
  const int64_t m = std::min<int64_t>(n, (int64_t)cap_points);
  if (m > 0 && out_xyzi &&
      hipMemcpy(out_xyzi, src + sl.off[frame], sizeof(float4) * (size_t)m, hipMemcpyDeviceToHost) != hipSuccess)
    return -(int64_t)ILCC_HIP_ERROR;
  return n;
}

int64_t ilcc_fetch_labelled(ilcc_handle* h, uint32_t frame, float* out_yz, uint8_t* out_label, uint64_t cap_points) {
  Slot* slp = nullptr;
  const int32_t st = fetch_slot(h, frame, 1, slp);
  if (st != ILCC_OK) return -(int64_t)st;
  Slot& sl = *slp;
  uint32_t n = 0;
  if (hipMemcpy(&n, sl.d_nlab + frame, sizeof(n), hipMemcpyDeviceToHost) != hipSuccess) return -(int64_t)ILCC_HIP_ERROR;
  return fetch_labelled_points(sl.d_yz + sl.off[frame], sl.d_lab + sl.off[frame], n, out_yz, out_label, cap_points);
}

int64_t ilcc_fetch_walk(ilcc_handle* h, uint32_t frame, float* out_yz, uint8_t* out_label, uint64_t cap_points, uint32_t counts[2]) {
  Slot* slp = nullptr;
  const int32_t st = fetch_slot(h, frame, 1, slp);
  if (st != ILCC_OK) return -(int64_t)st;
  Slot& sl = *slp;
  if (!sl.grid) return -(int64_t)ILCC_BAD_ARGUMENT;
  uint32_t n = 0;
  if (hipMemcpy(&n, sl.d_nlab + frame, sizeof(n), hipMemcpyDeviceToHost) != hipSuccess) return -(int64_t)ILCC_HIP_ERROR;
  if (n > (uint32_t)kGridLdsPointsMax) n = 0;
  if (counts) {
    if (hipMemcpy(&counts[0], sl.d_walk_mi + frame, sizeof(uint32_t), hipMemcpyDeviceToHost) != hipSuccess ||
        hipMemcpy(&counts[1], sl.d_walk_nrim + frame, sizeof(uint32_t), hipMemcpyDeviceToHost) != hipSuccess)
      return -(int64_t)ILCC_HIP_ERROR;
  }
  return fetch_labelled_points(sl.d_walk_yz + sl.off[frame], sl.d_walk_lab + sl.off[frame], n, out_yz, out_label, cap_points);
}

int32_t ilcc_grid_cost(ilcc_handle* h, const float* yz, const uint8_t* label, uint32_t m, int32_t use_oob,
                       float* cost_out, int32_t* best_index, float* best_cost) {
  if (!h) return ILCC_BAD_ARGUMENT;
  const hipStream_t s = h->stream[take_stream(h)];
  ILCC_TRY(stage_labelled(h, s, yz, label, m));
  Slot& sl = h->slots[0];
  const size_t vol = (size_t)h->p.n_th * h->p.n_ty * h->p.n_tz * 2;
  float* d_vol = nullptr;
  if (cost_out) HIP_TRY(h, hipMalloc((void**)&d_vol, sizeof(float) * vol));
  struct VolGuard {
    float* p;
    ~VolGuard() { if (p) (void)hipFree(p); }
  } guard{d_vol};
  const Ctx c = diagnostic_ctx(h, sl, m);
  const uint32_t inf_bits = 0x7f800000u;
  HIP_TRY(h, hipMemcpyAsync(sl.d_bound, &inf_bits, sizeof(inf_bits), hipMemcpyHostToDevice, s));
  launch_walk_order(c, s);
  launch_grid_cost(c, whole_grid_pass(c, c.grid, c.partial), s, use_oob, d_vol, d_vol == nullptr && h->p.grid_prune != 0);
  std::vector<GridPartial> part(c.grid_blocks);
  hipError_t e = hipGetLastError();
  if (e == hipSuccess) e = hipMemcpyAsync(part.data(), sl.d_partial, sizeof(GridPartial) * c.grid_blocks, hipMemcpyDeviceToHost, s);
  if (e == hipSuccess && cost_out) e = hipMemcpyAsync(cost_out, d_vol, sizeof(float) * vol, hipMemcpyDeviceToHost, s);
  if (e == hipSuccess) e = hipEventRecord(h->entry_done, s);
  if (e == hipSuccess) e = hipEventSynchronize(h->entry_done);
  if (e != hipSuccess) {
    h->err = std::string("ilcc_grid_cost: ") + hipGetErrorString(e);
    return ILCC_HIP_ERROR;
  }
  GridPartial b = part[0];
  for (uint32_t k = 1; k < c.grid_blocks; ++k) {
    const GridPartial& t = part[k];
    if (t.cost < b.cost || (t.cost == b.cost && (t.d2 < b.d2 || (t.d2 == b.d2 && t.flat < b.flat)))) b = t;
  }
  if (best_index) *best_index = (int32_t)b.flat;
  if (best_cost) *best_cost = b.cost;
  return ILCC_OK;
}

int32_t ilcc_grid_solve(ilcc_handle* h, const float* yz, const uint8_t* label, uint32_t m, int32_t* grid_index, float* grid_cost,
                        int32_t lat[3], int32_t* phase, int64_t* cost_q, int64_t* alt_cost_q, int32_t* rounds, int32_t* hops,
                        int32_t* flags, int32_t* ties) {
  if (!h || h->p.solver != ILCC_SOLVER_GRID) {
    if (h) h->err = "ilcc_grid_solve needs ILCC_SOLVER_GRID";
    return ILCC_BAD_ARGUMENT;
  }
  const hipStream_t s = h->stream[take_stream(h)];
  ILCC_TRY(stage_labelled(h, s, yz, label, m));
  Slot& sl = h->slots[0];
  const Ctx c = diagnostic_ctx(h, sl, m);
  const uint32_t inf_bits = 0x7f800000u, zero = 0u;
  HIP_TRY(h, hipMemcpyAsync(sl.d_bound, &inf_bits, sizeof(inf_bits), hipMemcpyHostToDevice, s));
  HIP_TRY(h, hipMemcpyAsync(sl.d_bound_sub, &inf_bits, sizeof(inf_bits), hipMemcpyHostToDevice, s));
  HIP_TRY(h, hipMemcpyAsync(sl.d_tie_count, &zero, sizeof(zero), hipMemcpyHostToDevice, s));
  HIP_TRY(h, hipMemsetAsync(sl.d_iters, 0, sizeof(unsigned long long) * kBatchWords, s));
  ILCC_TRY(enqueue_grid_search(h, sl, c, s, 1, false));
  launch_pattern_refine(c, s);
  launch_corners(c, s, 1);
  HIP_TRY(h, hipGetLastError());
  SolveRec rec{};
  ilcc_result r;
  HIP_TRY(h, hipMemcpyAsync(&rec, sl.d_solverec, sizeof(rec), hipMemcpyDeviceToHost, s));
  HIP_TRY(h, hipMemcpyAsync(&r, sl.d_res, offsetof(ilcc_result, corners), hipMemcpyDeviceToHost, s));
  ILCC_TRY(sync_own(h, s));
  if (!rec.valid) {
    h->err = "ilcc_grid_solve: the grid search produced no candidate";
    return ILCC_TOO_FEW_POINTS;
  }
  const double div = (double)(h->p.refine_div > 0 ? h->p.refine_div : 1);
  if (grid_index) *grid_index = r.grid_index;
  if (grid_cost) *grid_cost = r.grid_cost;
  if (lat) {
    lat[0] = (int32_t)std::lround((rec.x[0] - h->p.th_min) / (h->p.th_step / div));
    lat[1] = (int32_t)std::lround((rec.x[1] - h->p.ty_min) / (h->p.ty_step / div));
    lat[2] = (int32_t)std::lround((rec.x[2] - h->p.tz_min) / (h->p.tz_step / div));
  }
  if (phase) *phase = rec.phase;
  if (cost_q) *cost_q = rec.cost_q;
  if (alt_cost_q) *alt_cost_q = rec.alt_q;
  if (rounds) *rounds = rec.iters_a;
  if (hops) *hops = rec.iters_b;
  if (flags) *flags = rec.flags;
  if (ties) *ties = rec.ties;
  return ILCC_OK;
}

int32_t ilcc_get_theta_t(ilcc_handle* h, const float* yz, const uint8_t* label, uint32_t m, int32_t topleft_white,
                         int32_t use_oob, double theta_t[3], double* cost, int32_t* iterations) {
  if (!h || !theta_t) return ILCC_BAD_ARGUMENT;
  const hipStream_t s = h->stream[take_stream(h)];
  ILCC_TRY(stage_labelled(h, s, yz, label, m));
  Slot& sl = h->slots[0];
  HIP_TRY(h, hipMemcpyAsync(h->d_solve, theta_t, sizeof(double) * 3, hipMemcpyHostToDevice, s));
  const Ctx c = diagnostic_ctx(h, sl, 0);
  launch_local_solve(c, s, topleft_white, use_oob, h->d_solve, h->d_solve + 3);
  HIP_TRY(h, hipGetLastError());
  double back[5];
  HIP_TRY(h, hipMemcpyAsync(back, h->d_solve, sizeof(back), hipMemcpyDeviceToHost, s));
  ILCC_TRY(sync_own(h, s));
  theta_t[0] = back[0];
  theta_t[1] = back[1];
  theta_t[2] = back[2];
  if (cost) *cost = back[3];
  if (iterations) *iterations = (int32_t)back[4];
  return ILCC_OK;
}

int32_t ilcc_debug_reference_solve(ilcc_handle* h, const float* yz, const uint8_t* label, const uint64_t* offsets,
                                   const int32_t* status_in, uint32_t n_frames, double* rec_f64, int32_t* rec_i32,
                                   ilcc_result* results, uint32_t* lds_points) {
  if (!h || !status_in || !rec_f64 || !rec_i32 || !results) return ILCC_BAD_ARGUMENT;
  Slot& sl = h->slots[0];
  if (sl.busy) {
    h->err = "diagnostic entry while ticket 0 is in flight";
    return ILCC_BAD_ARGUMENT;
  }
  if (h->p.solver != ILCC_SOLVER_REFERENCE_LOCAL) {
    h->err = "ilcc_debug_reference_solve needs ILCC_SOLVER_REFERENCE_LOCAL";
    return ILCC_BAD_ARGUMENT;
  }
  ILCC_TRY(check_offsets(h, offsets, n_frames));
  const uint64_t total = offsets[n_frames];
  if (total > 0 && (!yz || !label)) return ILCC_BAD_ARGUMENT;
  HIP_TRY(h, hipSetDevice(h->device));
  const hipStream_t s = h->stream[take_stream(h)];
  std::vector<uint32_t> n_lab(n_frames), stride(n_frames);
  std::vector<ilcc_result> res(n_frames);
  std::memset(res.data(), 0, sizeof(ilcc_result) * n_frames);
  for (uint32_t f = 0; f < n_frames; ++f) {
    n_lab[f] = (uint32_t)(offsets[f + 1] - offsets[f]);
    stride[f] = walk_stride(n_lab[f]);
    res[f].status = status_in[f];
  }
  HIP_TRY(h, hipMemcpyAsync(sl.d_off, offsets, sizeof(uint64_t) * (n_frames + 1), hipMemcpyHostToDevice, s));
  HIP_TRY(h, hipMemcpyAsync(sl.d_res, res.data(), sizeof(ilcc_result) * n_frames, hipMemcpyHostToDevice, s));
  HIP_TRY(h, hipMemcpyAsync(sl.d_nlab, n_lab.data(), sizeof(uint32_t) * n_frames, hipMemcpyHostToDevice, s));
  HIP_TRY(h, hipMemcpyAsync(sl.d_walk, stride.data(), sizeof(uint32_t) * n_frames, hipMemcpyHostToDevice, s));
  if (total > 0) {
    HIP_TRY(h, hipMemcpyAsync(sl.d_yz, yz, sizeof(float2) * total, hipMemcpyHostToDevice, s));
    HIP_TRY(h, hipMemcpyAsync(sl.d_lab, label, total, hipMemcpyHostToDevice, s));
  }
  HIP_TRY(h, hipMemsetAsync(sl.d_solverec, 0xFF, sizeof(SolveRec) * 2 * n_frames, s));
  sl.n_frames = 0;
  const Ctx c = make_ctx(h, sl, nullptr, nullptr, n_frames, 1);
  launch_reference_solve(c, s);
  launch_corners(c, s, solve_slots(c.p));
  HIP_TRY(h, hipGetLastError());
  std::vector<SolveRec> rec(2 * (size_t)n_frames);
  HIP_TRY(h, hipMemcpyAsync(rec.data(), sl.d_solverec, sizeof(SolveRec) * rec.size(), hipMemcpyDeviceToHost, s));
  HIP_TRY(h, hipMemcpyAsync(results, sl.d_res, sizeof(ilcc_result) * n_frames, hipMemcpyDeviceToHost, s));
  ILCC_TRY(sync_own(h, s));
  for (size_t k = 0; k < rec.size(); ++k) {
    const SolveRec& r = rec[k];
    const double d[ILCC_SOLVE_REC_DOUBLES] = {r.x[0], r.x[1], r.x[2], r.cost_a, r.cost_b, r.sel};
    const int32_t i[ILCC_SOLVE_REC_INTS] = {r.iters_a, r.iters_b, r.phase, r.valid};
    std::memcpy(rec_f64 + ILCC_SOLVE_REC_DOUBLES * k, d, sizeof(d));
    std::memcpy(rec_i32 + ILCC_SOLVE_REC_INTS * k, i, sizeof(i));
  }
  if (lds_points) *lds_points = c.grid_lds_points;
  return ILCC_OK;
}

int32_t ilcc_pattern_refine(ilcc_handle* h, const float* yz, const uint8_t* label, uint32_t m, int32_t lat[3],
                            int32_t* phase, int64_t* cost_q, int64_t* alt_cost_q, int32_t* rounds, int32_t* hops) {
  if (!h || !lat || !phase) return ILCC_BAD_ARGUMENT;
  if (lat[0] < h->th_lat_lo || lat[0] > h->th_lat_hi || (*phase != 0 && *phase != 1)) {
    h->err = "ilcc_pattern_refine: theta lattice coordinate outside [th_min - refine_th_margin, th_max + refine_th_margin] steps";
    return ILCC_BAD_ARGUMENT;
  }
  const hipStream_t s = h->stream[take_stream(h)];
  ILCC_TRY(stage_labelled(h, s, yz, label, m));
  Slot& sl = h->slots[0];
  RefineOut io{};
  io.lat[0] = lat[0];
  io.lat[1] = lat[1];
  io.lat[2] = lat[2];
  io.phase = *phase;
  HIP_TRY(h, hipMemcpyAsync(h->d_refine_io, &io, sizeof(io), hipMemcpyHostToDevice, s));
  const Ctx c = diagnostic_ctx(h, sl, 0);
  launch_pattern_refine_test(c, s, h->d_refine_io);
  HIP_TRY(h, hipGetLastError());
  HIP_TRY(h, hipMemcpyAsync(&io, h->d_refine_io, sizeof(io), hipMemcpyDeviceToHost, s));
  ILCC_TRY(sync_own(h, s));
  lat[0] = io.lat[0];
  lat[1] = io.lat[1];
  lat[2] = io.lat[2];
  *phase = io.phase;
  if (cost_q) *cost_q = io.cost_q;
  if (alt_cost_q) *alt_cost_q = io.alt_q;
  if (rounds) *rounds = io.rounds;
  if (hops) *hops = io.hops;
  return ILCC_OK;
}

int32_t ilcc_debug_timeline_enable(ilcc_handle* h, int32_t on) {
  if (!h) return ILCC_BAD_ARGUMENT;
  HIP_TRY(h, hipSetDevice(h->device));
  h->tl_rows.clear();
  h->tl_on = on != 0;
  if (h->tl_on) {
    if (!h->tl_ref) HIP_TRY(h, hipEventCreate(&h->tl_ref));
    HIP_TRY(h, hipEventRecord(h->tl_ref, h->stream[0]));
    HIP_TRY(h, hipEventSynchronize(h->tl_ref));
  }
  return ILCC_OK;
}

int32_t ilcc_debug_separate_launches(ilcc_handle* h, int32_t on) {
  if (!h || any_batch_in_flight(h, "ilcc_debug_separate_launches")) return ILCC_BAD_ARGUMENT;
  h->separate_launches = on != 0;
  return ILCC_OK;
}

int32_t ilcc_debug_cluster_home(ilcc_handle* h, int32_t home) {
  if (!h || any_batch_in_flight(h, "ilcc_debug_cluster_home")) return ILCC_BAD_ARGUMENT;
  if (home != ILCC_CLUSTER_HOME_RULE && home != ILCC_CLUSTER_HOME_LDS && home != ILCC_CLUSTER_HOME_L2) {
    h->err = "ilcc_debug_cluster_home: home must be ILCC_CLUSTER_HOME_RULE, _LDS or _L2";
    return ILCC_BAD_ARGUMENT;
  }
  h->cluster_home = home;
  return ILCC_OK;
}

int32_t ilcc_debug_cluster_launch(const ilcc_handle* h, uint32_t out[ILCC_CLUSTER_LAUNCH_WORDS]) {
  if (!h || !out) return ILCC_BAD_ARGUMENT;
  out[0] = (uint32_t)h->cluster_last.home;
  out[1] = h->cluster_last.lds_bytes;
  out[2] = h->cluster_last.threads;
  out[3] = h->cluster_limits.static_lds;
  out[4] = h->cluster_limits.lds_per_cu;
  out[5] = h->cluster_limits.cus;
  return ILCC_OK;
}

int32_t ilcc_debug_timeline_fetch(ilcc_handle* h, double* rows, uint32_t cap_rows) {
  if (!h || (!rows && cap_rows)) return -ILCC_BAD_ARGUMENT;
  const size_t have = h->tl_rows.size() / ILCC_TIMELINE_COLS;
  const size_t n = std::min<size_t>(have, cap_rows);
  if (n) std::memcpy(rows, h->tl_rows.data(), sizeof(double) * n * ILCC_TIMELINE_COLS);
  h->tl_rows.clear();
  return (int32_t)n;
}

void ilcc_get_timing(const ilcc_handle* h, ilcc_timing* t) {
  if (h && t) *t = h->timing;
}
void ilcc_reset_timing(ilcc_handle* h) {
  if (h) h->timing = ilcc_timing{};
}

}
```

### lidar_camera_calibration_amd/csrc/ilcc_internal.h

```cpp
#pragma once

#include <hip/hip_runtime.h>
#include <stdint.h>

#include "ilcc_hip.h"

#define ILCC_WAVE 64

namespace ilcc {

constexpr int kCuLdsBytes = 160 * 1024;
constexpr int kClusterLdsMax = kCuLdsBytes - 4 * 1024;
constexpr int kLocateLdsMax = 3 * (kCuLdsBytes / 8);
constexpr int kSolveLdsMax = kCuLdsBytes - 16 * 1024;

constexpr int kCropThreads = 256;
constexpr int kCropChunk = 4096;
#ifndef ILCC_K2_THREADS
#define ILCC_K2_THREADS 256
#endif
constexpr int kFrameThreads = ILCC_K2_THREADS;
#ifndef ILCC_K3_THREADS
#define ILCC_K3_THREADS 256
#endif
#ifndef ILCC_K45_THREADS
#define ILCC_K45_THREADS 256
#endif
constexpr int kPlaneThreads = ILCC_K3_THREADS;
constexpr int kPlaneThreadsSmallBatch = 1024;
#ifndef ILCC_SMALL_BATCH
#define ILCC_SMALL_BATCH 64
#endif
constexpr int kSmallBatchFrames = ILCC_SMALL_BATCH;
constexpr int kHistThreads = ILCC_K45_THREADS;
constexpr int kWalkThreads = 256;
#ifndef ILCC_K6_THREADS
#define ILCC_K6_THREADS 256
#endif
constexpr int kGridThreads = ILCC_K6_THREADS;
#ifndef ILCC_K6_THREADS_LARGE
#define ILCC_K6_THREADS_LARGE 512
#endif
constexpr int kGridThreadsLarge = ILCC_K6_THREADS_LARGE;
#ifndef ILCC_K6_LARGE_FROM
#define ILCC_K6_LARGE_FROM 2048
#endif
constexpr int kGridLargeFrom = ILCC_K6_LARGE_FROM;
#ifndef ILCC_K6_GROUP
#define ILCC_K6_GROUP 7
#endif
constexpr int kThetaGroup = ILCC_K6_GROUP;
constexpr int kGridLdsPointsMax = 8192;
constexpr int kGridTableMax = 8192;
#ifndef ILCC_K7_THREADS
#define ILCC_K7_THREADS 256
#endif
constexpr int kSolveThreads = ILCC_K7_THREADS;
#ifndef ILCC_K7R_THREADS
#define ILCC_K7R_THREADS 192
#endif
constexpr int kRefineThreads = ILCC_K7R_THREADS;
constexpr int kRefineThreadsSmallBatch = 768;
constexpr int kRefineList = 32;
constexpr int kTieCap = 256;
constexpr float kTieEps = 2e-5f;
constexpr int kCoverageCellsMax = 1024;
constexpr int kIterSlots = 64;
constexpr int kBatchWords = 3 * kIterSlots + 2;
constexpr int kClusterHashSize = 1 << 17;
constexpr int kClusterLdsPointsMax = 4096;
constexpr int kClusterLdsPointsMin = 1024;
constexpr int kClusterCellsMin = 512;
constexpr int kClusterCellsMax = 6144;

struct GridPartial {
  float cost;
  uint32_t d2;
  uint32_t flat;
  uint32_t pad;
};

struct SolveRec {
  double x[3];
  double cost_a, cost_b, sel;
  double margin;
  int32_t iters_a, iters_b, phase, valid;
  int32_t flags, ties;
  long long cost_q, alt_q;
};

struct RefineOut {
  long long cost_q, alt_q;
  int32_t lat[3];
  int32_t phase, rounds, hops;
};

struct GridTables {
  const float* cth;
  const float* sth;
  const float* ay;
  const float* az;
  int32_t n_th, n_ty, n_tz;
  int32_t c_th, c_ty, c_tz;
};

struct SeedMap {
  int32_t stride_t, stride_th, off_th;
};

struct GridSeed {
  const GridPartial* records;
  uint32_t blocks;
  SeedMap map;
};

struct GridPass {
  GridTables t;
  GridPartial* out;
  uint32_t blocks;
  uint32_t walk_limit;
  uint32_t* bound;
  GridSeed seed;
  int32_t window_tiles, radius_th, step_th;
  uint32_t collect_ties;
  uint32_t box_points;
  uint32_t* grp_alive;
  uint32_t* grp_mask;
  uint32_t grp_count, grp_words;
};

struct Ctx {
  const float4* xyzi;
  const uint64_t* off;
  const float* clicks;
  uint32_t n_frames;
  uint32_t crop_chunks;
  ilcc_result* res;
  float4* roi;
  float4* cluster;
  float4* board;
  float4* pca;
  float4* optim;
  float2* yz;
  uint8_t* lab;
  uint32_t* n_lab;
  uint32_t* walk_stride;
  float2* walk_yz;
  uint8_t* walk_lab;
  uint32_t *walk_mi, *walk_nrim;
  uint8_t* cls;
  uint32_t* crop_counts;
  unsigned long long* crop_masks;
  uint32_t* uf_parent;
  uint32_t* uf_count;
  uint32_t* uf_hash_head;
  uint32_t* uf_hash_next;
  uint32_t cluster_lds_points;
  uint32_t cluster_cells_cap;
  uint32_t wide;
  uint32_t cluster_bits;
  uint32_t online_tier;
  float online_window;
  uint32_t* frame_flags;
  uint32_t* n_finite;
  uint32_t* crop_fin;
  uint32_t* list_count;
  uint32_t* list;
  void* list_frames;
  uint32_t list_grid;
  GridPartial* partial;
  SolveRec* solve_rec;
  uint32_t grid_blocks;
  uint32_t grid_lds_points;
  uint32_t* grid_bound;
  uint32_t* grid_bound_sub;
  uint32_t* tie_count;
  GridPartial* tie_list;
  unsigned long long* grid_iters;
  GridTables grid;
  const double2* th_lattice;
  int32_t th_lat_lo, th_lat_hi;
  int32_t refine_hop_y, refine_hop_z;
  ilcc_params p;
};

__host__ __device__ inline uint32_t walk_stride(uint32_t M) {
  if (M <= 2) return 1u;
  uint32_t S = ((uint32_t)((float)M * 0.6180339f)) | 1u;
  for (;; S += 2u) {
    uint32_t a = S, b = M;
    while (b) {
      const uint32_t t = a % b;
      a = b;
      b = t;
    }
    if (a == 1u) break;
  }
  return S >= M ? 1u : S;
}

__device__ __forceinline__ int lane_id() { return threadIdx.x & (ILCC_WAVE - 1); }
__device__ __forceinline__ int wave_id() { return threadIdx.x >> 6; }

template <typename T>
__device__ __forceinline__ T wave_sum(T v) {
#pragma unroll
  for (int o = ILCC_WAVE / 2; o > 0; o >>= 1) v += __shfl_down(v, o, ILCC_WAVE);
  return v;
}

template <typename T>
__device__ __forceinline__ T block_sum(T v, T* scratch) {
  v = wave_sum(v);
  const int nw = (blockDim.x + ILCC_WAVE - 1) / ILCC_WAVE;
  __syncthreads();
  if (lane_id() == 0) scratch[wave_id()] = v;
  __syncthreads();
  if (threadIdx.x == 0) {
    T s = scratch[0];
    for (int w = 1; w < nw; ++w) s += scratch[w];
    scratch[16] = s;
  }
  __syncthreads();
  return scratch[16];
}

template <int NV>
__device__ __forceinline__ void block_sum_n(double (&v)[NV], double* scratch ) {
#pragma unroll
  for (int k = 0; k < NV; ++k) v[k] = wave_sum(v[k]);
  const int kW = (blockDim.x + ILCC_WAVE - 1) / ILCC_WAVE;
  __syncthreads();
  if (lane_id() == 0) {
#pragma unroll
    for (int k = 0; k < NV; ++k) scratch[wave_id() * NV + k] = v[k];
  }
  __syncthreads();
#pragma unroll
  for (int k = 0; k < NV; ++k) {
    double t = scratch[k];
    for (int w = 1; w < kW; ++w) t += scratch[w * NV + k];
    v[k] = t;
  }
}

__device__ __forceinline__ uint32_t block_rank(bool flag, uint32_t* scratch, uint32_t& total) {
  const unsigned long long m = __ballot(flag);
  const int lane = lane_id();
  const uint32_t in_wave = __popcll(m & ((1ull << lane) - 1ull));
  const int nw = (blockDim.x + ILCC_WAVE - 1) / ILCC_WAVE;
  __syncthreads();
  if (lane == 0) scratch[wave_id()] = __popcll(m);
  __syncthreads();
  uint32_t base = 0, tot = 0;
  for (int w = 0; w < nw; ++w) {
    const uint32_t c = scratch[w];
    if (w < wave_id()) base += c;
    tot += c;
  }
  total = tot;
  return base + in_wave;
}

struct LocatePlan {
  GridTables seed;
  SeedMap map;
  int32_t refine_radius;
  uint32_t sample_min, sample_cap;
  GridPartial* out;
};

size_t locate_lds_bytes(uint32_t sample_cap, int n_ty, int n_tz, int n_ty2, int n_tz2);
void launch_locate(const Ctx& c, hipStream_t s, const LocatePlan& lp);
void launch_anchor(const Ctx& c, const GridPass& pass, hipStream_t s);
constexpr int kRefineThetaStride = 2;
constexpr int kLocateMinFrames = 512;

void launch_roi_crop(const Ctx& c, hipStream_t s, hipEvent_t after_count = nullptr, bool one_pass = false);
constexpr int kCropFrameMinFrames = 512;
constexpr int32_t kClusterHomeRule = 0, kClusterHomeLds = 1, kClusterHomeL2 = 2;
struct ClusterLimits {
  uint32_t cus, lds_per_cu, threads_per_cu, static_lds;
};
struct ClusterLaunch {
  int32_t home;
  uint32_t lds_bytes, threads;
};
hipError_t cluster_limits(int device, ClusterLimits* out);
ClusterLaunch launch_cluster(const Ctx& c, hipStream_t s, const ClusterLimits& lim, int32_t home);
void launch_ransac_plane(const Ctx& c, hipStream_t s);
void launch_plane_frame_hist(const Ctx& c, hipStream_t s);
void launch_front_end(const Ctx& c, hipStream_t s, bool walk_layout);
inline bool front_end_fusable(const Ctx& c) {
  return kPlaneThreads == kHistThreads && kHistThreads == kWalkThreads && c.n_frames > (uint32_t)kSmallBatchFrames && !c.wide;
}
void launch_walk_order(const Ctx& c, hipStream_t s);
void launch_grid_cost(const Ctx& c, const GridPass& pass, hipStream_t s, int32_t use_oob, float* cost_volume , bool prune);
void launch_group_prepass(const Ctx& c, const GridPass& full, hipStream_t s);
uint32_t grid_cost_evals_per_count();
void launch_reference_solve(const Ctx& c, hipStream_t s);
void launch_pattern_refine(const Ctx& c, hipStream_t s);
void launch_corners(const Ctx& c, hipStream_t s, int n_slots);
void launch_pack_records(const ilcc_result* d_res, uint32_t n_frames, uint32_t n_corners, uint32_t tag_base, float* d_out,
                         hipStream_t s);
void launch_store_to_host(const void* d_src, void* h_dst, size_t bytes, hipStream_t s);
void launch_pattern_refine_test(const Ctx& c, hipStream_t s, RefineOut* d_io);
hipError_t set_kernel_attributes_k2();
size_t cluster_lds_bytes(uint32_t pts_cap, uint32_t cells_cap, uint32_t bits);
uint32_t cluster_bits_default();
uint32_t cluster_bits_online();
hipError_t set_kernel_attributes_k6();
hipError_t set_kernel_attributes_k7a();
hipError_t set_kernel_attributes_k7r();
void launch_local_solve(const Ctx& c, hipStream_t s, int32_t tlw, int32_t use_oob, double* theta_t,
                        double* cost_iters );

}
```

### lidar_camera_calibration_amd/csrc/k7_common.h

```cpp
#pragma once

#include "ilcc_internal.h"

namespace ilcc {

template <int CTRL, int BANK = 0xf>
__device__ __forceinline__ uint32_t dpp_u32(uint32_t old, uint32_t v) {
  return (uint32_t)__builtin_amdgcn_update_dpp((int)old, (int)v, CTRL, 0xf, BANK, false);
}
template <int MASK>
__device__ __forceinline__ uint32_t xor_lane_u32(uint32_t v) {
  if constexpr (MASK == 32) {
    const auto r = __builtin_amdgcn_permlane32_swap(v, v, false, false);
    return (lane_id() & 32) ? r[0] : r[1];
  } else if constexpr (MASK == 16) {
    const auto r = __builtin_amdgcn_permlane16_swap(v, v, false, false);
    return (lane_id() & 16) ? r[0] : r[1];
  } else if constexpr (MASK == 8) {
    return dpp_u32<0x128>(0u, v);
  } else if constexpr (MASK == 4) {
    const uint32_t lo = dpp_u32<0x124, 0xa>(0u, v);
    return dpp_u32<0x12C, 0x5>(lo, v);
  } else if constexpr (MASK == 2) {
    return dpp_u32<0x4E>(0u, v);
  } else {
    return dpp_u32<0xB1>(0u, v);
  }
}
template <int MASK>
__device__ __forceinline__ double xor_lane_f64(double v) {
  const unsigned long long b = (unsigned long long)__double_as_longlong(v);
  const uint32_t lo = xor_lane_u32<MASK>((uint32_t)b), hi = xor_lane_u32<MASK>((uint32_t)(b >> 32));
  return __longlong_as_double((long long)(((unsigned long long)hi << 32) | lo));
}
template <int MASK>
__device__ __forceinline__ unsigned long long xor_lane_u64(unsigned long long b) {
  const uint32_t lo = xor_lane_u32<MASK>((uint32_t)b), hi = xor_lane_u32<MASK>((uint32_t)(b >> 32));
  return ((unsigned long long)hi << 32) | lo;
}

struct StagedPoints {
  float2* yz;
  uint8_t* lab;
};
__host__ __device__ inline size_t staged_points_bytes(uint32_t cap, uint32_t frames) {
  return (sizeof(float2) + 1) * (size_t)cap * (size_t)frames;
}
__device__ __forceinline__ StagedPoints staged_points(unsigned char* smem, uint32_t cap, uint32_t frames, uint32_t k) {
  return StagedPoints{reinterpret_cast<float2*>(smem) + (size_t)k * cap,
                      smem + sizeof(float2) * (size_t)cap * (size_t)frames + (size_t)k * cap};
}

inline int solve_slots(const ilcc_params& p) { return (p.solver == ILCC_SOLVER_REFERENCE_LOCAL && p.phase_mode == 2) ? 2 : 1; }

}
```

### lidar_camera_calibration_amd/csrc/k7r_pattern_refine.hip

```cpp
#include <climits>
#include <type_traits>

#include "k7_common.h"

namespace ilcc {

constexpr double kCostQOne = 1099511627776.0;
#define kRefineWaves ((int)(blockDim.x >> 6))
static_assert(kRefineThreads % ILCC_WAVE == 0 && kRefineThreads / ILCC_WAVE >= 3 && kRefineThreads >= kRefineList &&
              kRefineThreadsSmallBatch % (3 * ILCC_WAVE) == 0,
              "ILCC_K7R_THREADS must be a multiple of 64, at least 192");
constexpr float kBorderRisk = 4e-6f;
constexpr int32_t kNoTheta = INT32_MIN;

struct RCand {
  int32_t q0, q1, q2, phase;
};
constexpr int kRefineWavesMax = kRefineThreadsSmallBatch / ILCC_WAVE;
constexpr double kExactDoubleSum = 9007199254740992.0;
constexpr int kActQueue = 128;
struct RefineShared {
  RCand cand[kRefineList];
  GridPartial meta[kRefineList];
  unsigned long long acc[3][kRefineList];
  uint32_t queue[kRefineWavesMax][kActQueue];
};

struct RefineState {
  int32_t lat[3];
  int32_t phase, rounds, hops, capped;
  int32_t skip_first;
  long long cost, alt;
};

__device__ __forceinline__ bool partial_less(const GridPartial& a, const GridPartial& b) {
  return a.cost < b.cost || (a.cost == b.cost && (a.d2 < b.d2 || (a.d2 == b.d2 && a.flat < b.flat)));
}

struct GridCell {
  int gk, ga, gb;
  RCand at;
};
struct Lattice {
  const Ctx& c;
  int div;
  double u_th, u_ty, u_tz;
  __device__ __forceinline__ explicit Lattice(const Ctx& ctx) : c(ctx), div(ctx.p.refine_div > 0 ? ctx.p.refine_div : 1) {
    u_th = c.p.th_step / (double)div;
    u_ty = c.p.ty_step / (double)div;
    u_tz = c.p.tz_step / (double)div;
  }
  __device__ __forceinline__ double theta(int32_t q) const { return c.p.th_min + (double)q * u_th; }
  __device__ __forceinline__ double ty(int32_t q) const { return c.p.ty_min + (double)q * u_ty; }
  __device__ __forceinline__ double tz(int32_t q) const { return c.p.tz_min + (double)q * u_tz; }
  __device__ __forceinline__ int32_t theta_or_none(int q0) const { return (q0 < c.th_lat_lo || q0 > c.th_lat_hi) ? kNoTheta : q0; }
  __device__ __forceinline__ double2 cs(int32_t q0) const { return c.th_lattice[q0 - c.th_lat_lo]; }
  __device__ __forceinline__ GridCell from_flat(uint32_t flat) const {
    const uint32_t cell = flat >> 1, n_ty = (uint32_t)c.p.n_ty, n_tz = (uint32_t)c.p.n_tz;
    GridCell g;
    g.gk = (int)(cell / (n_tz * n_ty));
    g.ga = (int)((cell / n_tz) % n_ty);
    g.gb = (int)(cell % n_tz);
    g.at = RCand{g.gk * div, g.ga * div, g.gb * div, (int32_t)(flat & 1u)};
    return g;
  }
};

struct Board {
  double W, H, g, delta;
  double inv_g;
};
__device__ __forceinline__ Board make_board(const ilcc_params& p) {
  return Board{(double)p.board_w, (double)p.board_h, p.grid_length, p.huber_delta, 1.0 / p.grid_length};
}
struct BoardIJ {
  double i, j;
};
__device__ __forceinline__ BoardIJ board_ij(const Board& bd, double2 cs, double x1, double x2, float2 v) {
  const double y = (double)v.x, z = (double)v.y;
  const double ry = cs.x * y - cs.y * z;
  const double rz = cs.y * y + cs.x * z;
  return BoardIJ{((ry + x1) + bd.W * bd.g / 2.0) * bd.inv_g, ((rz + x2) + bd.H * bd.g / 2.0) * bd.inv_g};
}

struct AxisTerms {
  double in_dist;
  double out_dist;
  bool inside;
  bool odd;
};
__device__ __forceinline__ AxisTerms axis_terms(double v, double n) {
  AxisTerms t;
  t.inside = v > 0 && v < n;
  const double fl = floor(v);
  t.odd = (((int)fl) & 1) != 0;
  const double fr = v - fl;
  t.in_dist = (fr > 0.5) ? (fl + 1.0) - v : fr;
  t.out_dist = fmin(fabs(v), fabs(v - n));
  return t;
}
__device__ __forceinline__ double term_q(const AxisTerms& ai, const AxisTerms& aj, bool tlw, bool laser_white, double delta) {
  double res = 0.0;
  if (ai.inside && aj.inside) {
    const bool white = (ai.odd == aj.odd) ? tlw : !tlw;
    if (laser_white != white) res = ai.in_dist + aj.in_dist;
  } else {
    res = ai.out_dist + aj.out_dist;
  }
  const double r0 = (res > delta) ? 2.0 * delta * res - delta * delta : res * res;
  return rint(r0 * (0.5 * kCostQOne));
}

struct Frame {
  const Ctx& c;
  Board bd;
  Lattice lat;
  const float2* yz;
  const uint8_t* lab;
  uint32_t n;
  RefineShared& sh;
  int sweep;
};
__device__ __forceinline__ Frame begin_frame(const Ctx& c, RefineShared& sh, const float2* yz, const uint8_t* lab, uint32_t n) {
  if (threadIdx.x < kRefineList) sh.acc[0][threadIdx.x] = 0ull;
  return Frame{c, make_board(c.p), Lattice(c), yz, lab, n, sh, 0};
}

__device__ __forceinline__ int sweep_begin(Frame& fr) {
  if (threadIdx.x < kRefineList) fr.sh.acc[(fr.sweep + 1) % 3][threadIdx.x] = 0ull;
  __syncthreads();
  return fr.sweep % 3;
}
__device__ __forceinline__ void sweep_end(Frame& fr) {
  __syncthreads();
  ++fr.sweep;
}

__device__ __forceinline__ int refine_sweep(Frame& fr, int n_cand) {
  const int buf = sweep_begin(fr);
  const int lane = lane_id();
  const int slices = ILCC_WAVE / n_cand;
  const int cand = lane % n_cand, slice = lane / n_cand;
  if (slice < slices) {
    const RCand cd = fr.sh.cand[cand];
    if (cd.q0 != kNoTheta) {
      const double2 cs = fr.lat.cs(cd.q0);
      const double x1 = fr.lat.ty(cd.q1), x2 = fr.lat.tz(cd.q2);
      const bool tlw = cd.phase != 0;
      long long sum = 0;
      for (uint32_t p = (uint32_t)(wave_id() * slices + slice); p < fr.n; p += (uint32_t)(kRefineWaves * slices)) {
        const BoardIJ at = board_ij(fr.bd, cs, x1, x2, fr.yz[p]);
        const AxisTerms ai = axis_terms(at.i, fr.bd.W);
        const AxisTerms aj = axis_terms(at.j, fr.bd.H);
        sum += (long long)term_q(ai, aj, tlw, fr.lab[p] != 0, fr.bd.delta);
      }
      atomicAdd(&fr.sh.acc[buf][cand], (unsigned long long)sum);
    }
  }
  sweep_end(fr);
  return buf;
}

__device__ __forceinline__ int stencil_sweep(Frame& fr, int n_th, const int32_t th[3], const int32_t ty[3], const int32_t tz[3],
                                             int phase, bool parity) {
  const Ctx& c = fr.c;
  const Board& bd = fr.bd;
  const float2* yz = fr.yz;
  const uint8_t* lab = fr.lab;
  const uint32_t n = fr.n;
  const int buf = sweep_begin(fr);
  const int wid = __builtin_amdgcn_readfirstlane(wave_id());
  const int waves_per_theta = kRefineWaves / n_th;
  const int it = wid % n_th, grp = wid / n_th;
  const int32_t q0 = th[it];
  if (grp < waves_per_theta && q0 != kNoTheta) {
    const int lane = lane_id();
    const double2 cs = fr.lat.cs(q0);
    double x1[3], x2[3];
#pragma unroll
    for (int k = 0; k < 3; ++k) {
      x1[k] = fr.lat.ty(ty[k]);
      x2[k] = fr.lat.tz(tz[k]);
    }
    const uint32_t n_slices = (uint32_t)(waves_per_theta * ILCC_WAVE);
    const bool skip_silent = !parity && ty[0] <= ty[1] && ty[1] <= ty[2] && tz[0] <= tz[1] && tz[1] <= tz[2] && c.p.ty_step > 0.0 && c.p.tz_step > 0.0;
    auto walk = [&](auto* acc) {
      using Acc = std::remove_reference_t<decltype(acc[0])>;
#pragma unroll
      for (int e = 0; e < 9; ++e) acc[e] = (Acc)0;
      auto eval_point = [&](uint32_t p) {
        const float2 v = yz[p];
        const bool laser_white = lab[p] != 0;
        AxisTerms ai[3], aj[3];
#pragma unroll
        for (int k = 0; k < 3; ++k) {
          const BoardIJ at = board_ij(bd, cs, x1[k], x2[k], v);
          ai[k] = axis_terms(at.i, bd.W);
          aj[k] = axis_terms(at.j, bd.H);
        }
#pragma unroll
        for (int a = 0; a < 3; ++a)
#pragma unroll
          for (int b = 0; b < 3; ++b) {
            const bool tlw = ((phase ^ (parity ? ((a + b) & 1) : 0)) != 0);
            acc[a * 3 + b] += (Acc)term_q(ai[a], aj[b], tlw, laser_white, bd.delta);
          }
      };
      if (skip_silent) {
        uint32_t* queue = fr.sh.queue[wid];
        uint32_t head = 0, tail = 0;
        const bool tlw0 = phase != 0;
        for (uint32_t base = (uint32_t)(grp * ILCC_WAVE); base < n; base += n_slices) {
          const uint32_t p = base + (uint32_t)lane;
          bool active = false;
          if (p < n) {
            const float2 v = yz[p];
            const BoardIJ lo = board_ij(bd, cs, x1[0], x2[0], v), hi = board_ij(bd, cs, x1[2], x2[2], v);
            const double fi = floor(lo.i), fj = floor(lo.j);
            const bool one_cell = lo.i > 0 && hi.i < bd.W && lo.j > 0 && hi.j < bd.H && fi == floor(hi.i) && fj == floor(hi.j);
            const bool odd_i = (((int)fi) & 1) != 0, odd_j = (((int)fj) & 1) != 0;
            const bool white = (odd_i == odd_j) ? tlw0 : !tlw0;
            active = !(one_cell && (lab[p] != 0) == white);
          }
          const unsigned long long m = __ballot(active);
          if (m != 0ull) {
            if (active) queue[(tail + (uint32_t)__popcll(m & ((1ull << lane) - 1ull))) & (kActQueue - 1)] = p;
            tail += (uint32_t)__popcll(m);
            __builtin_amdgcn_fence(__ATOMIC_RELEASE, "wavefront");
            __builtin_amdgcn_wave_barrier();
            __builtin_amdgcn_fence(__ATOMIC_ACQUIRE, "wavefront");
            while (tail - head >= (uint32_t)ILCC_WAVE) {
              eval_point(queue[(head + (uint32_t)lane) & (kActQueue - 1)]);
              head += ILCC_WAVE;
            }
            __builtin_amdgcn_fence(__ATOMIC_RELEASE, "wavefront");
            __builtin_amdgcn_wave_barrier();
          }
        }
        if ((uint32_t)lane < tail - head) eval_point(queue[(head + (uint32_t)lane) & (kActQueue - 1)]);
        __builtin_amdgcn_fence(__ATOMIC_RELEASE, "wavefront");
        __builtin_amdgcn_wave_barrier();
      } else {
        for (uint32_t p = (uint32_t)(grp * ILCC_WAVE + lane); p < n; p += n_slices) eval_point(p);
      }
    };
    unsigned long long tot[9];
    {
      double acc[9];
      walk(acc);
      bool rounded = false;
#pragma unroll
      for (int e = 0; e < 9; ++e) {
        rounded |= !(acc[e] < kExactDoubleSum);
        tot[e] = (unsigned long long)(long long)acc[e];
      }
      if (__ballot(rounded) != 0ull) {
        long long iacc[9];
        walk(iacc);
#pragma unroll
        for (int e = 0; e < 9; ++e) tot[e] = (unsigned long long)iacc[e];
      }
    }
#pragma unroll
    for (int e = 0; e < 9; ++e) {
      unsigned long long t = tot[e];
      t += xor_lane_u64<8>(t);
      t += xor_lane_u64<4>(t);
      t += xor_lane_u64<2>(t);
      t += xor_lane_u64<1>(t);
      if ((lane & 15) == 0) atomicAdd(&fr.sh.acc[buf][it * 9 + e], t);
    }
  }
  sweep_end(fr);
  return buf;
}

__device__ __forceinline__ GridPartial grid_argmin(const Ctx& c, uint32_t f) {
  const GridPartial* gp = c.partial + (uint64_t)f * c.grid_blocks;
  GridPartial b{__builtin_inff(), 0xFFFFFFFFu, 0xFFFFFFFFu, 0u};
  for (uint32_t k = lane_id(); k < c.grid_blocks; k += ILCC_WAVE) {
    const GridPartial t = gp[k];
    if (partial_less(t, b)) b = t;
  }
#pragma unroll
  for (int o = ILCC_WAVE / 2; o > 0; o >>= 1) {
    GridPartial t;
    t.cost = __shfl_xor(b.cost, o, ILCC_WAVE);
    t.d2 = __shfl_xor(b.d2, o, ILCC_WAVE);
    t.flat = __shfl_xor(b.flat, o, ILCC_WAVE);
    if (partial_less(t, b)) b = t;
  }
  return b;
}

__device__ __forceinline__ uint32_t recount_near_ties(Frame& fr, uint32_t f, GridPartial& b, int& flags) {
  const Ctx& c = fr.c;
  RefineShared& sh = fr.sh;
  if (c.tie_count == nullptr) return 0;
  const uint32_t n_ties = c.tie_count[f];
  if (n_ties > (uint32_t)kTieCap) {
    flags |= ILCC_FLAG_TIE_OVERFLOW;
    return n_ties;
  }
  const GridPartial* tl = c.tie_list + (uint64_t)f * kTieCap;
  const float window = b.cost * (1.f + kTieEps);
  uint32_t close = 0;
  for (uint32_t e = 0; e < n_ties; ++e) close += (tl[e].cost <= window && tl[e].flat != b.flat) ? 1u : 0u;
  if (close > 0) {
    long long best_q = LLONG_MAX;
    GridPartial pick = b;
    int k = 0;
    for (uint32_t e = 0; e <= n_ties; ++e) {
      const GridPartial t = (e < n_ties) ? tl[e] : b;
      const bool take = (t.cost <= window) && !(e < n_ties && t.flat == b.flat);
      if (take) {
        if (threadIdx.x == 0) {
          sh.cand[k] = fr.lat.from_flat(t.flat).at;
          sh.meta[k] = t;
        }
        ++k;
      }
      if (k == kRefineList || (e == n_ties && k > 0)) {
        const int bf = refine_sweep(fr, k);
        for (int j = 0; j < k; ++j) {
          const long long cq = (long long)sh.acc[bf][j];
          const GridPartial m = sh.meta[j];
          if (cq < best_q || (cq == best_q && (m.d2 < pick.d2 || (m.d2 == pick.d2 && m.flat < pick.flat)))) {
            best_q = cq;
            pick = m;
          }
        }
        k = 0;
        __syncthreads();
      }
    }
    b = pick;
  }
  return n_ties;
}

__device__ __forceinline__ bool first_round_is_settled(const Frame& fr, const GridCell& at, int& flags) {
  const Ctx& c = fr.c;
  const int gk = at.gk, ga = at.ga, gb = at.gb, n_ty = c.p.n_ty, n_tz = c.p.n_tz;
  bool risk = false;
  for (uint32_t i = threadIdx.x; i < fr.n; i += blockDim.x) {
    const float2 v = fr.yz[i];
#pragma unroll
    for (int dk = -1; dk <= 1; ++dk) {
      const int k = gk + dk;
      if (k < 0 || k >= c.p.n_th) continue;
      const float cth = c.grid.cth[k], sth = c.grid.sth[k];
      const float pi = fmaf(-sth, v.y, cth * v.x), pj = fmaf(cth, v.y, sth * v.x);
#pragma unroll
      for (int d = -1; d <= 1; ++d) {
        const int a = ga + d, b = gb + d;
        if (a >= 0 && a < n_ty) {
          const float x = pi + c.grid.ay[a];
          risk |= fabsf(x - rintf(x)) < kBorderRisk;
        }
        if (b >= 0 && b < n_tz) {
          const float x = pj + c.grid.az[b];
          risk |= fabsf(x - rintf(x)) < kBorderRisk;
        }
      }
    }
  }
  risk = __syncthreads_or(risk ? 1 : 0) != 0;
  if (risk) flags |= ILCC_FLAG_BORDER_RISK;
  return !risk && !(flags & ILCC_FLAG_TIE_OVERFLOW) && gk > 0 && gk < c.p.n_th - 1 && ga > 0 && ga < n_ty - 1 && gb > 0 && gb < n_tz - 1;
}

__device__ __forceinline__ void pattern_refine(Frame& fr, RefineState& st) {
  const Ctx& c = fr.c;
  const RefineShared& sh = fr.sh;
  const bool refine = c.p.refine_div > 0;
  const int div = fr.lat.div;
  st.rounds = 0;
  st.hops = 0;
  st.capped = 0;
  st.cost = 0;
  st.alt = 0;
  for (;;) {
    int stride = div, r = 0;
    if (st.skip_first && refine && div >= 2 && c.p.refine_max_rounds >= 1) {
      stride = div >> 1;
      r = 1;
    }
    st.skip_first = 0;
    while (refine && stride >= 1 && r < c.p.refine_max_rounds) {
      int32_t th[3], ty[3], tz[3];
#pragma unroll
      for (int k = 0; k < 3; ++k) {
        th[k] = fr.lat.theta_or_none(st.lat[0] + (k - 1) * stride);
        ty[k] = st.lat[1] + (k - 1) * stride;
        tz[k] = st.lat[2] + (k - 1) * stride;
      }
      const int b = stencil_sweep(fr, 3, th, ty, tz, st.phase, false);
      long long bc = LLONG_MAX;
      int bd2 = 0, be = -1;
      for (int e = 0; e < 27; ++e) {
        if (e == 13) continue;
        const int dk = e / 9 - 1, da = (e / 3) % 3 - 1, db = e % 3 - 1;
        if (fr.lat.theta_or_none(st.lat[0] + dk * stride) == kNoTheta) continue;
        const long long cc = (long long)sh.acc[b][e];
        const int d2 = dk * dk + da * da + db * db;
        if (cc < bc || (cc == bc && d2 < bd2)) {
          bc = cc;
          bd2 = d2;
          be = e;
        }
      }
      const long long centre = (long long)sh.acc[b][13];
      ++r;
      if (be >= 0 && bc < centre) {
        st.lat[0] += (be / 9 - 1) * stride;
        st.lat[1] += ((be / 3) % 3 - 1) * stride;
        st.lat[2] += (be % 3 - 1) * stride;
      } else {
        stride >>= 1;
      }
    }
    st.rounds += r;
    if (refine && stride >= 1) st.capped = 1;
    const int32_t th1[3] = {st.lat[0], kNoTheta, kNoTheta};
    const int32_t hy[3] = {st.lat[1] - c.refine_hop_y, st.lat[1], st.lat[1] + c.refine_hop_y};
    const int32_t hz[3] = {st.lat[2] - c.refine_hop_z, st.lat[2], st.lat[2] + c.refine_hop_z};
    const int b = stencil_sweep(fr, 1, th1, hy, hz, st.phase, true);
    st.cost = (long long)sh.acc[b][4];
    long long alt = LLONG_MAX;
    int ae = -1;
    for (int e = 0; e < 9; ++e) {
      if (e == 4) continue;
      const long long cc = (long long)sh.acc[b][e];
      if (cc < alt) {
        alt = cc;
        ae = e;
      }
    }
    st.alt = alt;
    if (alt < st.cost && st.hops < 2 && refine) {
      const int da = ae / 3 - 1, db = ae % 3 - 1;
      ++st.hops;
      st.lat[1] += da * c.refine_hop_y;
      st.lat[2] += db * c.refine_hop_z;
      st.phase ^= (da + db) & 1;
      continue;
    }
    break;
  }
}

__device__ __forceinline__ RefineState start_at(const RCand& at, bool skip_first) {
  RefineState st;
  st.lat[0] = at.q0;
  st.lat[1] = at.q1;
  st.lat[2] = at.q2;
  st.phase = at.phase;
  st.skip_first = skip_first ? 1 : 0;
  return st;
}

__device__ __forceinline__ void store_record(const Lattice& lat, const RefineState& st, int flags, uint32_t n_ties, SolveRec* out) {
  out->x[0] = lat.theta(st.lat[0]);
  out->x[1] = lat.ty(st.lat[1]);
  out->x[2] = lat.tz(st.lat[2]);
  out->cost_a = out->sel = (double)st.cost / kCostQOne;
  out->cost_b = (double)st.alt / kCostQOne;
  out->margin = ((double)st.alt - (double)st.cost) / (double)(st.cost > 0 ? st.cost : 1);
  out->iters_a = st.rounds;
  out->iters_b = st.hops;
  out->phase = st.phase;
  out->valid = 1;
  out->flags = flags | (st.capped ? ILCC_FLAG_REFINE_CAPPED : 0);
  out->ties = (int32_t)n_ties;
  out->cost_q = st.cost;
  out->alt_q = st.alt;
}

template <bool LDS_POINTS>
__device__ __forceinline__ void refine_frame(const Ctx& c, SolveRec* rec, const StagedPoints& lds, RefineShared& sh) {
  const uint32_t f = blockIdx.x;
  const uint64_t beg = c.off[f];
  SolveRec* out = &rec[2 * f];
  Frame fr = begin_frame(c, sh, c.yz + beg, c.lab + beg, c.n_lab[f]);
  if (LDS_POINTS) {
    for (uint32_t i = threadIdx.x; i < fr.n; i += blockDim.x) {
      lds.yz[i] = fr.yz[i];
      lds.lab[i] = fr.lab[i];
    }
    fr.yz = lds.yz;
    fr.lab = lds.lab;
  }
  __syncthreads();

  GridPartial b = grid_argmin(c, f);
  if (b.flat == 0xFFFFFFFFu) {
    if (threadIdx.x == 0) out->valid = 0;
    return;
  }
  int flags = 0;
  const uint32_t n_ties = recount_near_ties(fr, f, b, flags);
  if (threadIdx.x == 0) {
    c.res[f].grid_index = (int32_t)b.flat;
    c.res[f].grid_cost = b.cost;
  }
  const GridCell start = fr.lat.from_flat(b.flat);
  RefineState st = start_at(start.at, first_round_is_settled(fr, start, flags));
  pattern_refine(fr, st);
  if (threadIdx.x == 0) store_record(fr.lat, st, flags, n_ties, out);
}

__global__ __launch_bounds__(kRefineThreadsSmallBatch) void k7r_pattern_refine(Ctx c, SolveRec* rec) {
  extern __shared__ __align__(16) unsigned char smem[];
  __shared__ RefineShared sh;
  const uint32_t f = blockIdx.x;
  if (c.res[f].status != ILCC_OK) {
    if (threadIdx.x == 0) rec[2 * f].valid = 0;
    return;
  }
  const StagedPoints lds = staged_points(smem, c.grid_lds_points, 1, 0);
  if (c.n_lab[f] <= c.grid_lds_points)
    refine_frame<true>(c, rec, lds, sh);
  else
    refine_frame<false>(c, rec, lds, sh);
}

__global__ __launch_bounds__(kRefineThreads) void k7r_pattern_refine_test(Ctx c, RefineOut* io) {
  __shared__ RefineShared sh;
  Frame fr = begin_frame(c, sh, c.yz, c.lab, c.n_lab[0]);
  RefineState st = start_at(RCand{io->lat[0], io->lat[1], io->lat[2], io->phase}, false);
  __syncthreads();
  pattern_refine(fr, st);
  if (threadIdx.x == 0) {
    io->lat[0] = st.lat[0];
    io->lat[1] = st.lat[1];
    io->lat[2] = st.lat[2];
    io->phase = st.phase;
    io->rounds = st.rounds;
    io->hops = st.hops;
    io->cost_q = st.cost;
    io->alt_q = st.alt;
  }
}

hipError_t set_kernel_attributes_k7r() {
  return hipFuncSetAttribute((const void*)k7r_pattern_refine, hipFuncAttributeMaxDynamicSharedMemorySize,
                             (int)staged_points_bytes(kGridLdsPointsMax, 1));
}

void launch_pattern_refine(const Ctx& c, hipStream_t s) {
  const int threads = c.n_frames <= (uint32_t)kSmallBatchFrames ? kRefineThreadsSmallBatch : kRefineThreads;
  hipLaunchKernelGGL(k7r_pattern_refine, dim3(c.n_frames), dim3(threads), staged_points_bytes(c.grid_lds_points, 1), s, c, c.solve_rec);
}

void launch_pattern_refine_test(const Ctx& c, hipStream_t s, RefineOut* d_io) {
  hipLaunchKernelGGL(k7r_pattern_refine_test, dim3(1), dim3(kRefineThreads), 0, s, c, d_io);
}

}
```

### lidar_camera_calibration_amd/lidar_corners_est.py

```python
from __future__ import annotations

import ctypes as C
from typing import Optional, Sequence

import numpy as np

from . import _native as N


class IlccError(RuntimeError):
    def __init__(self, status: int, detail: str = ""):
        self.status = int(status)
        msg = N.strerror(status)
        super().__init__(f"{msg}: {detail}" if detail else msg)


class LidarCornersEst:

    def __init__(self, device: int = -1, max_frames: int = 1, max_points_per_frame: int = 150_000,
                 params: Optional[N.Params] = None):
        self._lib = N.lib()
        self.params = params if params is not None else N.default_params()
        self._device = device
        self._max_frames = int(max_frames)
        self._max_points = int(max_frames) * int(max_points_per_frame)
        self._h = None
        self._cloud = None
        self._click = None
        self._result: Optional[N.Result] = None
        self.accept_ambiguous = False
        self.accept_low_coverage = False
        self.m_click_point = None
        self.m_cloud_ROI = self.m_cloud_chessboard = self.m_cloud_PCA = None
        self.m_cloud_optim = self.m_cloud_corners = None

    def _handle(self):
        if self._h is None:
            h = self._lib.ilcc_create(self._device, C.byref(self.params), self._max_frames, self._max_points)
            if not h:
                raise IlccError(N.HIP_ERROR, self._lib.ilcc_last_error(None).decode())
            self._h = h
        return self._h

    def close(self):
        if self._h is not None:
            self._lib.ilcc_destroy(self._h)
            self._h = None

    def __del__(self):
        try:
            self.close()
        except Exception:
            pass

    def _check(self, st: int):
        if st != N.OK:
            raise IlccError(st, self._lib.ilcc_last_error(self._h).decode() if self._h else "")

    def set_params(self, params: N.Params):
        self.params = params
        if self._h is not None:
            self._check(self._lib.ilcc_set_params(self._h, C.byref(self.params)))

    def register_viewer(self):
        """LidarCornersEst.h:26-37 opens two PCLVisualizer windows; there is no display on a GPU
        node, candidates are accepted automatically (keys 'o' and 'k')."""

    def set_chessboard_param(self, cam_yaml: str) -> bool:
        st = self._lib.ilcc_set_chessboard_param(C.byref(self.params), cam_yaml.encode())
        if st != N.OK:
            print("can not open " + cam_yaml)
            return False
        if self._h is not None:
            self._check(self._lib.ilcc_set_params(self._h, C.byref(self.params)))
        print("grid_length:", self.params.grid_length)
        print("grid_in_x:", self.params.board_w)
        print("grid_in_y:", self.params.board_h)
        return True

    def setROI(self, cloud: np.ndarray, point: Sequence[float]):
        cloud = np.ascontiguousarray(cloud, dtype=np.float32)
        if cloud.ndim != 2 or cloud.shape[1] != 4:
            raise ValueError("cloud must be n x 4 (x, y, z, intensity)")
        self._cloud = cloud
        self._click = np.ascontiguousarray(point, dtype=np.float32).reshape(3)
        self.m_click_point = self._click.copy()
        self._result = None

    def find_board(self, cloud: np.ndarray, seed_params=None):
        from . import seed as S
        self.setROI(cloud, (0.0, 0.0, 0.0))
        h = self._handle()
        sp = seed_params if seed_params is not None else S.default_seed_params(self.params)
        if seed_params is None:
            sp.max_seeds = max(1, min(sp.max_seeds, self._max_frames))
        res, seeds, ranks = S.extract_auto(self, self._cloud, None, sp)
        self._click = seeds[0].copy()
        self.m_click_point = self._click.copy()
        if ranks[0] < 0:
            self._result = None
            return False, self._click
        res1 = N.Result()
        self._check(self._lib.ilcc_extract(h, N.fptr(self._cloud), len(self._cloud), N.fptr(self._click), C.byref(res1)))
        self._result = res1
        return True, self._click

    def _run(self):
        if self._result is None:
            if self._cloud is None:
                raise RuntimeError("setROI must be called first")
            res = N.Result()
            st = self._lib.ilcc_extract(self._handle(), N.fptr(self._cloud), len(self._cloud),
                                        N.fptr(self._click), C.byref(res))
            self._check(st)
            self._result = res
        return self._result

    def _fetch(self, which: int) -> np.ndarray:
        n = self._lib.ilcc_fetch_cloud(self._h, 0, which, None, 0)
        if n < 0:
            raise IlccError(-n)
        out = np.zeros((max(n, 1), 4), dtype=np.float32)
        self._lib.ilcc_fetch_cloud(self._h, 0, which, N.fptr(out), n)
        return out[:n]

    def get_chessboard_by_point(self, incloud: np.ndarray, point: Sequence[float], min_plane_points: int = 500):
        cloud = np.ascontiguousarray(incloud, dtype=np.float32)
        pt = np.ascontiguousarray(point, dtype=np.float32).reshape(3)
        off = np.array([0, len(cloud)], dtype=np.uint64)
        res = (N.Result * 1)()
        st = self._lib.ilcc_chessboard_by_point_batch(self._handle(), N.fptr(cloud),
                                                      off.ctypes.data_as(C.POINTER(C.c_uint64)), 1, N.fptr(pt),
                                                      int(min_plane_points), res)
        self._check(st)
        self._front = res[0]
        self._result = None
        out = self._fetch(N.CLOUD_CHESSBOARD) if res[0].status in (N.OK, N.BOARD_NOT_FOUND) else np.zeros((0, 4), np.float32)
        return res[0].status == N.OK, out

    def get_gray_zone(self, cloud=None, rate: Optional[float] = None) -> np.ndarray:
        src = self._result if self._result is not None else getattr(self, "_front", None)
        if src is None:
            raise RuntimeError("no plane cloud yet: call get_chessboard_by_point or PCA first")
        return np.array(src.gray_zone)

    def color_by_gray_zone(self) -> np.ndarray:
        n = self._lib.ilcc_fetch_classes(self._h, 0, None, 0)
        if n < 0:
            raise IlccError(-n)
        cl = np.zeros(max(n, 1), dtype=np.uint8)
        self._lib.ilcc_fetch_classes(self._h, 0, cl.ctypes.data_as(C.POINTER(C.c_uint8)), n)
        lut = np.array([[10, 10, 10], [255, 0, 0], [255, 255, 255]], dtype=np.uint8)
        return lut[cl[:n]]

    def EuclideanCluster(self) -> bool:
        res = self._run()
        self.m_cloud_ROI = self._fetch(N.CLOUD_ROI)
        if res.status in (N.NO_ROI_POINTS, N.NO_CLUSTER, N.NO_PLANE):
            return False
        self.m_cloud_chessboard = self._fetch(N.CLOUD_CHESSBOARD)
        print("chessboard plane size:", len(self.m_cloud_chessboard))
        return True

    def PCA(self):
        res = self._run()
        self.m_cloud_PCA = self._fetch(N.CLOUD_PCA)
        self.pca_matrix = np.array(res.pca, dtype=np.float32).reshape(4, 4)
        self.m_gray_zone = np.array(res.gray_zone)

    def get_corners(self, corners: list) -> bool:
        res = self._run()
        if res.status == N.AMBIGUOUS and not self.accept_ambiguous:
            print("reject this scan (ambiguous: basin margin %.3g)" % res.basin_margin)
            return False
        if res.status not in (N.OK, N.AMBIGUOUS):
            print("reject this scan")
            return False
        if (res.flags & N.FLAG_LOW_COVERAGE) and not self.accept_low_coverage:
            print("reject this scan (pattern under-sampled: %d of %d squares hold points)"
                  % (res.cells_hit, self.params.board_w * self.params.board_h))
            return False
        c = res.corners_array()
        self.m_cloud_optim = self._fetch(N.CLOUD_OPTIM)
        self.m_cloud_corners = np.concatenate([c, np.full((len(c), 1), 50.0, np.float32)], 1)
        corners.extend(map(tuple, c.astype(np.float64)))
        return True

    @property
    def result(self) -> Optional[N.Result]:
        return self._result


class LidarCornersBatch:

    def __init__(self, max_frames: int, max_points_per_frame: int, params: Optional[N.Params] = None,
                 device: int = -1):
        self._lib = N.lib()
        self.params = params if params is not None else N.default_params()
        self._h = self._lib.ilcc_create(device, C.byref(self.params), int(max_frames),
                                        int(max_frames) * int(max_points_per_frame))
        if not self._h:
            raise IlccError(N.HIP_ERROR, self._lib.ilcc_last_error(None).decode())

    def close(self):
        if self._h:
            self._lib.ilcc_destroy(self._h)
            self._h = None

    def __del__(self):
        try:
            self.close()
        except Exception:
            pass

    def _err(self):
        return self._lib.ilcc_last_error(self._h).decode()

    def set_params(self, params: N.Params):
        self.params = params
        st = self._lib.ilcc_set_params(self._h, C.byref(params))
        if st != N.OK:
            raise IlccError(st, self._err())

    def set_result_mode(self, mode: int):
        st = self._lib.ilcc_set_result_mode(self._h, int(mode))
        if st != N.OK:
            raise IlccError(st, self._err())

    def debug_separate_launches(self, on: bool):
        st = self._lib.ilcc_debug_separate_launches(self._h, 1 if on else 0)
        if st != N.OK:
            raise IlccError(st, self._err())

    def debug_cluster_home(self, home: int):
        st = self._lib.ilcc_debug_cluster_home(self._h, int(home))
        if st != N.OK:
            raise IlccError(st, self._err())

    def debug_cluster_launch(self) -> dict:
        out = (C.c_uint32 * N.CLUSTER_LAUNCH_WORDS)()
        st = self._lib.ilcc_debug_cluster_launch(self._h, out)
        if st != N.OK:
            raise IlccError(st, self._err())
        return dict(zip(("home", "lds_bytes", "threads", "static_lds_bytes", "lds_per_cu", "cus"), (int(v) for v in out)))

    def wait_compact(self, ticket) -> np.ndarray:
        t, n_frames = ticket
        width = int(self._lib.ilcc_record_floats(self._h, t))
        if width == 0:
            raise IlccError(N.BAD_ARGUMENT, "wait_compact: no batch in flight under this ticket")
        rec = np.empty((n_frames, width), dtype=np.float32)
        st = self._lib.ilcc_wait_compact(self._h, t, N.fptr(rec), rec.size)
        if st != N.OK:
            raise IlccError(st, self._err())
        return rec

    def fetch_results(self, first: int, n: int):
        res = (N.Result * n)()
        st = self._lib.ilcc_fetch_results(self._h, int(first), int(n), res)
        if st != N.OK:
            raise IlccError(st, self._err())
        return res

    def reserve(self, labelled_points_per_frame: int, roi_points_per_frame: int):
        st = self._lib.ilcc_reserve(self._h, int(labelled_points_per_frame), int(roi_points_per_frame))
        if st != N.OK:
            raise IlccError(st, self._err())

    def extract(self, clouds: np.ndarray, clicks: np.ndarray, offsets: Optional[np.ndarray] = None):
        clouds = np.ascontiguousarray(clouds, dtype=np.float32)
        clicks = np.ascontiguousarray(clicks, dtype=np.float32).reshape(-1, 3)
        f = len(clicks)
        if offsets is None:
            n = clouds.shape[-2]
            offsets = np.arange(f + 1, dtype=np.uint64) * np.uint64(n)
        offsets = np.ascontiguousarray(offsets, dtype=np.uint64)
        res = (N.Result * f)()
        st = self._lib.ilcc_extract_batch(self._h, N.fptr(clouds), offsets.ctypes.data_as(C.POINTER(C.c_uint64)),
                                          f, N.fptr(clicks), res)
        if st != N.OK:
            raise IlccError(st, self._err())
        return res

    def extract_device(self, d_xyzi_ptr: int, n_frames: int, n_points: int, d_clicks_ptr: int):
        offsets = np.arange(n_frames + 1, dtype=np.uint64) * np.uint64(n_points)
        res = (N.Result * n_frames)()
        st = self._lib.ilcc_extract_batch_device(self._h, C.c_void_p(d_xyzi_ptr),
                                                 offsets.ctypes.data_as(C.POINTER(C.c_uint64)), n_frames,
                                                 C.c_void_p(d_clicks_ptr), res)
        if st != N.OK:
            raise IlccError(st, self._err())
        return res

    def submit_device(self, d_xyzi_ptr: int, n_frames: int, n_points: int, d_clicks_ptr: int):
        offsets = np.arange(n_frames + 1, dtype=np.uint64) * np.uint64(n_points)
        ticket = C.c_int32(-1)
        st = self._lib.ilcc_submit_batch_device(self._h, C.c_void_p(d_xyzi_ptr),
                                                offsets.ctypes.data_as(C.POINTER(C.c_uint64)), n_frames,
                                                C.c_void_p(d_clicks_ptr), C.byref(ticket))
        if st != N.OK:
            raise IlccError(st, self._err())
        return ticket.value, n_frames

    def submit_host(self, xyzi_ptr: int, n_frames: int, n_points: int, clicks_ptr: int):
        offsets = np.arange(n_frames + 1, dtype=np.uint64) * np.uint64(n_points)
        ticket = C.c_int32(-1)
        st = self._lib.ilcc_submit_batch(self._h, C.c_void_p(xyzi_ptr), offsets.ctypes.data_as(C.POINTER(C.c_uint64)),
                                         n_frames, C.c_void_p(clicks_ptr), C.byref(ticket))
        if st != N.OK:
            raise IlccError(st, self._err())
        return ticket.value, n_frames

    def wait(self, ticket, d_records_ptr: Optional[int] = None, n_corners: int = 0, tag_base: int = 0,
             want_results: bool = True):
        t, n_frames = ticket
        res = (N.Result * n_frames)() if (want_results or d_records_ptr is None) else None
        if d_records_ptr is not None:
            st = self._lib.ilcc_wait_records_device(self._h, t, res, C.c_void_p(d_records_ptr), n_corners,
                                                    int(tag_base) & 0xFFFFFFFF)
        else:
            st = self._lib.ilcc_wait(self._h, t, res)
        if st != N.OK:
            raise IlccError(st, self._err())
        return res

    def fetch_cloud(self, frame: int, which: int) -> np.ndarray:
        n = self._lib.ilcc_fetch_cloud(self._h, frame, which, None, 0)
        if n < 0:
            raise IlccError(-n)
        out = np.zeros((max(n, 1), 4), dtype=np.float32)
        self._lib.ilcc_fetch_cloud(self._h, frame, which, N.fptr(out), n)
        return out[:n]

    def chessboard_by_point(self, clouds: np.ndarray, points: np.ndarray, min_plane_points: int = 500,
                            offsets: Optional[np.ndarray] = None):
        clouds = np.ascontiguousarray(clouds, dtype=np.float32)
        points = np.ascontiguousarray(points, dtype=np.float32).reshape(-1, 3)
        f = len(points)
        if offsets is None:
            offsets = np.arange(f + 1, dtype=np.uint64) * np.uint64(clouds.shape[-2])
        offsets = np.ascontiguousarray(offsets, dtype=np.uint64)
        res = (N.Result * f)()
        st = self._lib.ilcc_chessboard_by_point_batch(self._h, N.fptr(clouds),
                                                      offsets.ctypes.data_as(C.POINTER(C.c_uint64)), f,
                                                      N.fptr(points), int(min_plane_points), res)
        if st != N.OK:
            raise IlccError(st, self._err())
        return res

    def submit_chessboard_by_point(self, xyzi_ptr: int, n_frames: int, n_points: int, points_ptr: int):
        offsets = np.arange(n_frames + 1, dtype=np.uint64) * np.uint64(n_points)
        ticket = C.c_int32(-1)
        st = self._lib.ilcc_submit_chessboard_by_point(self._h, C.c_void_p(xyzi_ptr), offsets.ctypes.data_as(C.POINTER(C.c_uint64)),
                                                       n_frames, C.c_void_p(points_ptr), C.byref(ticket))
        if st != N.OK:
            raise IlccError(st, self._err())
        return ticket.value, n_frames

    def wait_chessboard_by_point(self, ticket, min_plane_points: int = 500):
        t, n_frames = ticket
        res = (N.Result * n_frames)()
        st = self._lib.ilcc_wait_chessboard_by_point(self._h, t, int(min_plane_points), res)
        if st != N.OK:
            raise IlccError(st, self._err())
        return res

    def fetch_classes(self, frame: int) -> np.ndarray:
        n = self._lib.ilcc_fetch_classes(self._h, frame, None, 0)
        if n < 0:
            raise IlccError(-n)
        cl = np.zeros(max(n, 1), dtype=np.uint8)
        self._lib.ilcc_fetch_classes(self._h, frame, cl.ctypes.data_as(C.POINTER(C.c_uint8)), n)
        return cl[:n]

    def fetch_labelled(self, frame: int):
        n = self._lib.ilcc_fetch_labelled(self._h, frame, None, None, 0)
        if n < 0:
            raise IlccError(-n)
        yz = np.zeros((max(n, 1), 2), dtype=np.float32)
        lab = np.zeros(max(n, 1), dtype=np.uint8)
        self._lib.ilcc_fetch_labelled(self._h, frame, N.fptr(yz), lab.ctypes.data_as(C.POINTER(C.c_uint8)), n)
        return yz[:n], lab[:n]

    def fetch_walk(self, frame: int):
        counts = (C.c_uint32 * 2)()
        n = self._lib.ilcc_fetch_walk(self._h, frame, None, None, 0, counts)
        if n < 0:
            raise IlccError(-n)
        yz = np.zeros((max(n, 1), 2), dtype=np.float32)
        lab = np.zeros(max(n, 1), dtype=np.uint8)
        self._lib.ilcc_fetch_walk(self._h, frame, N.fptr(yz), lab.ctypes.data_as(C.POINTER(C.c_uint8)), n, counts)
        return yz[:n], lab[:n], int(counts[0]), int(counts[1])

    def grid_cost(self, yz: np.ndarray, label: np.ndarray, use_oob: bool = True, want_volume: bool = False):
        yz = np.ascontiguousarray(yz, dtype=np.float32).reshape(-1, 2)
        label = np.ascontiguousarray(label, dtype=np.uint8)
        p = self.params
        vol = np.zeros(p.n_th * p.n_ty * p.n_tz * 2, dtype=np.float32) if want_volume else None
        bi, bc = C.c_int32(-1), C.c_float(0)
        st = self._lib.ilcc_grid_cost(self._h, N.fptr(yz), label.ctypes.data_as(C.POINTER(C.c_uint8)), len(label),
                                      int(use_oob), N.fptr(vol) if want_volume else None, C.byref(bi), C.byref(bc))
        if st != N.OK:
            raise IlccError(st, self._err())
        return bi.value, bc.value, vol

    def pattern_refine(self, yz: np.ndarray, label: np.ndarray, lat, phase: int):
        yz = np.ascontiguousarray(yz, dtype=np.float32).reshape(-1, 2)
        label = np.ascontiguousarray(label, dtype=np.uint8)
        q = np.array(lat, dtype=np.int32)
        ph, rounds, hops = C.c_int32(int(phase)), C.c_int32(0), C.c_int32(0)
        cq, aq = C.c_int64(0), C.c_int64(0)
        st = self._lib.ilcc_pattern_refine(self._h, N.fptr(yz), label.ctypes.data_as(C.POINTER(C.c_uint8)), len(label),
                                           q.ctypes.data_as(C.POINTER(C.c_int32)), C.byref(ph), C.byref(cq),
                                           C.byref(aq), C.byref(rounds), C.byref(hops))
        if st != N.OK:
            raise IlccError(st, self._err())
        return q, ph.value, cq.value, aq.value, rounds.value, hops.value

    def grid_solve(self, yz: np.ndarray, label: np.ndarray) -> dict:
        yz = np.ascontiguousarray(yz, dtype=np.float32).reshape(-1, 2)
        label = np.ascontiguousarray(label, dtype=np.uint8)
        q = np.zeros(3, dtype=np.int32)
        gi, ph, rounds, hops, flags, ties = (C.c_int32(0) for _ in range(6))
        gc = C.c_float(0)
        cq, aq = C.c_int64(0), C.c_int64(0)
        st = self._lib.ilcc_grid_solve(self._h, N.fptr(yz), label.ctypes.data_as(C.POINTER(C.c_uint8)), len(label), C.byref(gi),
                                       C.byref(gc), q.ctypes.data_as(C.POINTER(C.c_int32)), C.byref(ph), C.byref(cq), C.byref(aq),
                                       C.byref(rounds), C.byref(hops), C.byref(flags), C.byref(ties))
        if st != N.OK:
            raise IlccError(st, self._err())
        return dict(grid_index=gi.value, grid_cost=gc.value, lat=q, phase=ph.value, cost_q=cq.value, alt_cost_q=aq.value,
                    rounds=rounds.value, hops=hops.value, flags=flags.value, ties=ties.value)

    def get_theta_t(self, yz: np.ndarray, label: np.ndarray, topleft_white: bool, use_oob: bool,
                    theta_t0=(0.0, 0.0, 0.0)):
        yz = np.ascontiguousarray(yz, dtype=np.float32).reshape(-1, 2)
        label = np.ascontiguousarray(label, dtype=np.uint8)
        t = np.array(theta_t0, dtype=np.float64)
        cost, it = C.c_double(0), C.c_int32(0)
        st = self._lib.ilcc_get_theta_t(self._h, N.fptr(yz), label.ctypes.data_as(C.POINTER(C.c_uint8)), len(label),
                                        int(topleft_white), int(use_oob), t.ctypes.data_as(C.POINTER(C.c_double)),
                                        C.byref(cost), C.byref(it))
        if st != N.OK:
            raise IlccError(st, self._err())
        return t, cost.value, it.value

    def debug_reference_solve(self, frames, status_in=None) -> dict:
        f = len(frames)
        counts = [len(lab) for _, lab in frames]
        offsets = np.zeros(f + 1, dtype=np.uint64)
        offsets[1:] = np.cumsum(counts, dtype=np.uint64)
        yz = np.ascontiguousarray(np.concatenate([np.asarray(a, np.float32).reshape(-1, 2) for a, _ in frames] or
                                                 [np.zeros((0, 2), np.float32)]), dtype=np.float32)
        label = np.ascontiguousarray(np.concatenate([np.asarray(b, np.uint8).reshape(-1) for _, b in frames] or
                                                    [np.zeros(0, np.uint8)]), dtype=np.uint8)
        status = np.ascontiguousarray(np.zeros(f, np.int32) if status_in is None else status_in, dtype=np.int32)
        if len(status) != f:
            raise IlccError(N.BAD_ARGUMENT, "debug_reference_solve: one status per frame")
        d = np.zeros((f, 2, N.SOLVE_REC_DOUBLES), dtype=np.float64)
        i = np.zeros((f, 2, N.SOLVE_REC_INTS), dtype=np.int32)
        res = (N.Result * max(f, 1))()
        lds = C.c_uint32(0)
        st = self._lib.ilcc_debug_reference_solve(self._h, N.fptr(yz), label.ctypes.data_as(C.POINTER(C.c_uint8)),
                                                  offsets.ctypes.data_as(C.POINTER(C.c_uint64)),
                                                  status.ctypes.data_as(C.POINTER(C.c_int32)), f,
                                                  d.ctypes.data_as(C.POINTER(C.c_double)), i.ctypes.data_as(C.POINTER(C.c_int32)),
                                                  res, C.byref(lds))
        if st != N.OK:
            raise IlccError(st, self._err())
        return dict(x=d[:, :, 0:3].copy(), cost_a=d[:, :, 3].copy(), cost_b=d[:, :, 4].copy(), sel=d[:, :, 5].copy(),
                    iters_a=i[:, :, 0].copy(), iters_b=i[:, :, 1].copy(), phase=i[:, :, 2].copy(), valid=i[:, :, 3].copy(),
                    results=res, lds_points=int(lds.value))

    def timing(self) -> N.Timing:
        t = N.Timing()
        self._lib.ilcc_get_timing(self._h, C.byref(t))
        return t

    def reset_timing(self):
        self._lib.ilcc_reset_timing(self._h)


def save_corners2txt(corners_xyz: np.ndarray, filename: str):
    c = np.ascontiguousarray(corners_xyz, dtype=np.float32).reshape(-1, 3)
    st = N.lib().ilcc_save_corners2txt(N.fptr(c), len(c), filename.encode())
    if st != N.OK:
        raise IlccError(st, filename)


def read_lidar_corners(filename: str, num: int) -> np.ndarray:
    out = np.zeros((num, 3), dtype=np.float64)
    n = N.lib().ilcc_read_lidar_corners(filename.encode(), num, out.ctypes.data_as(C.POINTER(C.c_double)))
    if n < 0:
        raise IlccError(-n, filename)
    return out[:n]
```

Before: 1.353 million.

## Split pattern refine into budgeted head and resumable tail launches

Adds an optional two-launch pattern refine. A wide head kernel runs a limited number of sweeps per frame and saves resume state, and a narrower tail kernel finishes only the frames still pending. The per-wave activity queue moves from static shared memory into dynamic LDS, and uses 16-bit indices when points are staged, which shrinks static LDS. The split is off by default (head sweeps -1 means a single launch), so the default path only picks up the LDS relayout and the extra template and state plumbing.

Measured after the change: 1.350 million. No clear change (-0.2%).

```diff
diff --git a/include/ilcc_hip.h b/include/ilcc_hip.h
--- a/include/ilcc_hip.h
+++ b/include/ilcc_hip.h
@@ -210,6 +210,15 @@
 int32_t ilcc_debug_cluster_home(ilcc_handle* h, int32_t home);
 int32_t ilcc_debug_cluster_launch(const ilcc_handle* h, uint32_t out[ILCC_CLUSTER_LAUNCH_WORDS]);
 
+#define ILCC_REFINE_SPLIT_ONE_LAUNCH (-1)
+#define ILCC_REFINE_SPLIT_RULE (-2)
+#define ILCC_REFINE_LAUNCH_WORDS 8
+int32_t ilcc_debug_refine_split(ilcc_handle* h, int32_t head_sweeps);
+int32_t ilcc_debug_refine_launch(ilcc_handle* h, int32_t out[ILCC_REFINE_LAUNCH_WORDS]);
+int32_t ilcc_debug_pattern_refine_batch(ilcc_handle* h, const float* yz, const uint8_t* label, const uint64_t* offsets,
+                                        uint32_t n_frames, int32_t* lat, int32_t* phase, int64_t* cost_q, int64_t* alt_cost_q,
+                                        int32_t* rounds, int32_t* hops);
+
 void ilcc_get_timing(const ilcc_handle* h, ilcc_timing* t);
 void ilcc_reset_timing(ilcc_handle* h);
 
diff --git a/lidar_camera_calibration_amd/_native.py b/lidar_camera_calibration_amd/_native.py
--- a/lidar_camera_calibration_amd/_native.py
+++ b/lidar_camera_calibration_amd/_native.py
@@ -28,11 +28,14 @@
     "ilcc_set_result_mode", "ilcc_wait_compact", "ilcc_record_floats", "ilcc_fetch_results",
     "ilcc_debug_timeline_enable", "ilcc_debug_timeline_fetch", "ilcc_debug_separate_launches",
     "ilcc_debug_cluster_home", "ilcc_debug_cluster_launch", "ilcc_debug_reference_solve",
+    "ilcc_debug_refine_split", "ilcc_debug_refine_launch", "ilcc_debug_pattern_refine_batch",
 ]
 ABI_VERSION = 5
 RESULTS_FULL, RESULTS_COMPACT = 0, 1
 CLUSTER_HOME_RULE, CLUSTER_HOME_LDS, CLUSTER_HOME_L2 = 0, 1, 2
 CLUSTER_LAUNCH_WORDS = 6
+REFINE_SPLIT_ONE_LAUNCH, REFINE_SPLIT_RULE = -1, -2
+REFINE_LAUNCH_WORDS = 8
 SOLVE_REC_DOUBLES, SOLVE_REC_INTS = 6, 4
 
 
@@ -221,6 +224,15 @@
         L.ilcc_debug_reference_solve.argtypes = [vp, fp, C.POINTER(C.c_uint8), C.POINTER(C.c_uint64), C.POINTER(C.c_int32), C.c_uint32,
                                                  C.POINTER(C.c_double), C.POINTER(C.c_int32), rp, C.POINTER(C.c_uint32)]
         L.ilcc_debug_reference_solve.restype = C.c_int32
+        if hasattr(L, "ilcc_debug_refine_split"):
+            i32p, i64p = C.POINTER(C.c_int32), C.POINTER(C.c_int64)
+            L.ilcc_debug_refine_split.argtypes = [vp, C.c_int32]
+            L.ilcc_debug_refine_split.restype = C.c_int32
+            L.ilcc_debug_refine_launch.argtypes = [vp, i32p]
+            L.ilcc_debug_refine_launch.restype = C.c_int32
+            L.ilcc_debug_pattern_refine_batch.argtypes = [vp, fp, C.POINTER(C.c_uint8), C.POINTER(C.c_uint64), C.c_uint32, i32p, i32p,
+                                                          i64p, i64p, i32p, i32p]
+            L.ilcc_debug_pattern_refine_batch.restype = C.c_int32
         L.ilcc_fetch_results.argtypes = [vp, C.c_uint32, C.c_uint32, rp]
         L.ilcc_fetch_results.restype = C.c_int32
         _lib = L
diff --git a/lidar_camera_calibration_amd/csrc/ilcc_api.cpp b/lidar_camera_calibration_amd/csrc/ilcc_api.cpp
--- a/lidar_camera_calibration_amd/csrc/ilcc_api.cpp
+++ b/lidar_camera_calibration_amd/csrc/ilcc_api.cpp
@@ -76,6 +76,8 @@
   uint32_t* d_tie_count = nullptr;
   GridPartial* d_tie_list = nullptr;
   unsigned long long* d_iters = nullptr;
+  RefineResume* d_refine_resume = nullptr;
+  uint32_t* d_refine_pending = nullptr;
   uint32_t *d_grp_alive = nullptr, *d_grp_mask = nullptr;
   size_t grp_alive_cap = 0, grp_mask_cap = 0;
   float* h_rec_dev = nullptr;
@@ -131,6 +133,10 @@
   ClusterLimits cluster_limits{};
   int32_t cluster_home = kClusterHomeRule;
   ClusterLaunch cluster_last{};
+  int32_t refine_split = kRefineSplitRule;
+  RefineLaunch refine_last{};
+  int refine_last_slot = -1;
+  uint32_t refine_last_frames = 0;
   std::vector<double> tl_rows;
   std::string err;
 };
@@ -306,6 +312,8 @@
       buffer(sl.d_tie_count, mf),
       buffer(sl.d_tie_list, mf * kTieCap),
       buffer(sl.d_iters, kBatchWords),
+      buffer(sl.d_refine_resume, mf),
+      buffer(sl.d_refine_pending, mf),
       buffer(sl.d_grp_alive, 0),
       buffer(sl.d_grp_mask, 0),
   };
@@ -476,8 +484,17 @@
   c.th_lat_hi = h->th_lat_hi;
   c.refine_hop_y = h->hop_y;
   c.refine_hop_z = h->hop_z;
+  c.refine_resume = sl.d_refine_resume;
+  c.refine_pending = sl.d_refine_pending;
+  c.refine_io = nullptr;
   c.p = h->p;
   return c;
+}
+
+void note_refine_launch(ilcc_handle* h, const Slot& sl, uint32_t n_frames, const RefineLaunch& l) {
+  h->refine_last = l;
+  h->refine_last_slot = (int)(&sl - h->slots);
+  h->refine_last_frames = n_frames;
 }
 
 int32_t check_offsets(ilcc_handle* h, const uint64_t* offsets, uint32_t n_frames) {
@@ -723,7 +740,7 @@
   HIP_TRY(h, hipEventRecord(sl.ev[kEvSearched], s));
   if (kind == kRoiPipeline) {
     if (sl.grid) {
-      launch_pattern_refine(c, s);
+      note_refine_launch(h, sl, n_frames, launch_pattern_refine(c, s, h->refine_split));
     } else {
       launch_reference_solve(c, s);
     }
@@ -1401,7 +1418,7 @@
   HIP_TRY(h, hipMemcpyAsync(sl.d_tie_count, &zero, sizeof(zero), hipMemcpyHostToDevice, s));
   HIP_TRY(h, hipMemsetAsync(sl.d_iters, 0, sizeof(unsigned long long) * kBatchWords, s));
   ILCC_TRY(enqueue_grid_search(h, sl, c, s, 1, false));
-  launch_pattern_refine(c, s);
+  note_refine_launch(h, sl, 1, launch_pattern_refine(c, s, h->refine_split));
   launch_corners(c, s, 1);
   HIP_TRY(h, hipGetLastError());
   SolveRec rec{};
@@ -1568,6 +1585,104 @@
   return ILCC_OK;
 }
 
+int32_t ilcc_debug_refine_split(ilcc_handle* h, int32_t head_sweeps) {
+  if (!h || any_batch_in_flight(h, "ilcc_debug_refine_split")) return ILCC_BAD_ARGUMENT;
+  if (head_sweeps < 0 && head_sweeps != ILCC_REFINE_SPLIT_ONE_LAUNCH && head_sweeps != ILCC_REFINE_SPLIT_RULE) {
+    h->err = "ilcc_debug_refine_split: a budget >= 0, ILCC_REFINE_SPLIT_ONE_LAUNCH or ILCC_REFINE_SPLIT_RULE";
+    return ILCC_BAD_ARGUMENT;
+  }
+  h->refine_split = head_sweeps;
+  return ILCC_OK;
+}
+
+int32_t ilcc_debug_refine_launch(ilcc_handle* h, int32_t out[ILCC_REFINE_LAUNCH_WORDS]) {
+  if (!h || !out) return ILCC_BAD_ARGUMENT;
+  if (any_batch_in_flight(h, "ilcc_debug_refine_launch")) return ILCC_BAD_ARGUMENT;
+  const RefineLaunch& l = h->refine_last;
+  const int32_t stat = (int32_t)refine_static_lds_bytes();
+  out[0] = l.head_threads;
+  out[1] = l.tail_threads;
+  out[2] = l.budget;
+  out[3] = (int32_t)l.head_lds;
+  out[4] = l.head_threads ? stat : 0;
+  out[5] = (int32_t)l.tail_lds;
+  out[6] = l.tail_threads ? stat : 0;
+  out[7] = 0;
+  if (l.tail_threads != 0 && h->refine_last_slot >= 0) {
+    HIP_TRY(h, hipSetDevice(h->device));
+    ILCC_TRY(sync_all(h));
+    std::vector<uint32_t> pending(h->refine_last_frames);
+    HIP_TRY(h, hipMemcpy(pending.data(), h->slots[h->refine_last_slot].d_refine_pending, sizeof(uint32_t) * pending.size(),
+                         hipMemcpyDeviceToHost));
+    for (uint32_t v : pending) out[7] += v != 0u ? 1 : 0;
+  }
+  return ILCC_OK;
+}
+
+int32_t ilcc_debug_pattern_refine_batch(ilcc_handle* h, const float* yz, const uint8_t* label, const uint64_t* offsets,
+                                        uint32_t n_frames, int32_t* lat, int32_t* phase, int64_t* cost_q, int64_t* alt_cost_q,
+                                        int32_t* rounds, int32_t* hops) {
+  if (!h || !lat || !phase) return ILCC_BAD_ARGUMENT;
+  Slot& sl = h->slots[0];
+  if (sl.busy) {
+    h->err = "diagnostic entry while ticket 0 is in flight";
+    return ILCC_BAD_ARGUMENT;
+  }
+  if (h->p.solver != ILCC_SOLVER_GRID) {
+    h->err = "ilcc_debug_pattern_refine_batch needs ILCC_SOLVER_GRID";
+    return ILCC_BAD_ARGUMENT;
+  }
+  ILCC_TRY(check_offsets(h, offsets, n_frames));
+  const uint64_t total = offsets[n_frames];
+  if (total > 0 && (!yz || !label)) return ILCC_BAD_ARGUMENT;
+  std::vector<RefineOut> io(n_frames);
+  for (uint32_t f = 0; f < n_frames; ++f) {
+    if (lat[3 * f] < h->th_lat_lo || lat[3 * f] > h->th_lat_hi || (phase[f] != 0 && phase[f] != 1)) {
+      h->err = "ilcc_debug_pattern_refine_batch: theta lattice coordinate outside [th_min - refine_th_margin, th_max + refine_th_margin] steps, or a phase that is not 0 or 1";
+      return ILCC_BAD_ARGUMENT;
+    }
+    io[f] = RefineOut{0, 0, {lat[3 * f], lat[3 * f + 1], lat[3 * f + 2]}, phase[f], 0, 0};
+  }
+  HIP_TRY(h, hipSetDevice(h->device));
+  const hipStream_t s = h->stream[take_stream(h)];
+  std::vector<uint32_t> n_lab(n_frames);
+  std::vector<ilcc_result> res(n_frames);
+  std::memset(res.data(), 0, sizeof(ilcc_result) * n_frames);
+  for (uint32_t f = 0; f < n_frames; ++f) n_lab[f] = (uint32_t)(offsets[f + 1] - offsets[f]);
+  RefineOut* d_io = nullptr;
+  HIP_TRY(h, hipMalloc((void**)&d_io, sizeof(RefineOut) * n_frames));
+  struct IoGuard {
+    RefineOut* p;
+    ~IoGuard() { (void)hipFree(p); }
+  } guard{d_io};
+  HIP_TRY(h, hipMemcpyAsync(sl.d_off, offsets, sizeof(uint64_t) * (n_frames + 1), hipMemcpyHostToDevice, s));
+  HIP_TRY(h, hipMemcpyAsync(sl.d_res, res.data(), sizeof(ilcc_result) * n_frames, hipMemcpyHostToDevice, s));
+  HIP_TRY(h, hipMemcpyAsync(sl.d_nlab, n_lab.data(), sizeof(uint32_t) * n_frames, hipMemcpyHostToDevice, s));
+  HIP_TRY(h, hipMemcpyAsync(d_io, io.data(), sizeof(RefineOut) * n_frames, hipMemcpyHostToDevice, s));
+  if (total > 0) {
+    HIP_TRY(h, hipMemcpyAsync(sl.d_yz, yz, sizeof(float2) * total, hipMemcpyHostToDevice, s));
+    HIP_TRY(h, hipMemcpyAsync(sl.d_lab, label, total, hipMemcpyHostToDevice, s));
+  }
+  sl.n_frames = 0;
+  Ctx c = make_ctx(h, sl, nullptr, nullptr, n_frames, 1);
+  c.refine_io = d_io;
+  note_refine_launch(h, sl, n_frames, launch_pattern_refine(c, s, h->refine_split));
+  HIP_TRY(h, hipGetLastError());
+  HIP_TRY(h, hipMemcpyAsync(io.data(), d_io, sizeof(RefineOut) * n_frames, hipMemcpyDeviceToHost, s));
+  ILCC_TRY(sync_own(h, s));
+  for (uint32_t f = 0; f < n_frames; ++f) {
+    lat[3 * f] = io[f].lat[0];
+    lat[3 * f + 1] = io[f].lat[1];
+    lat[3 * f + 2] = io[f].lat[2];
+    phase[f] = io[f].phase;
+    if (cost_q) cost_q[f] = io[f].cost_q;
+    if (alt_cost_q) alt_cost_q[f] = io[f].alt_q;
+    if (rounds) rounds[f] = io[f].rounds;
+    if (hops) hops[f] = io[f].hops;
+  }
+  return ILCC_OK;
+}
+
 int32_t ilcc_debug_cluster_launch(const ilcc_handle* h, uint32_t out[ILCC_CLUSTER_LAUNCH_WORDS]) {
   if (!h || !out) return ILCC_BAD_ARGUMENT;
   out[0] = (uint32_t)h->cluster_last.home;
diff --git a/lidar_camera_calibration_amd/csrc/ilcc_internal.h b/lidar_camera_calibration_amd/csrc/ilcc_internal.h
--- a/lidar_camera_calibration_amd/csrc/ilcc_internal.h
+++ b/lidar_camera_calibration_amd/csrc/ilcc_internal.h
@@ -62,6 +62,11 @@
 constexpr int kRefineThreads = ILCC_K7R_THREADS;
 constexpr int kRefineThreadsSmallBatch = 768;
 constexpr int kRefineList = 32;
+#ifndef ILCC_K7R_HEAD_SWEEPS
+#define ILCC_K7R_HEAD_SWEEPS (-1)
+#endif
+constexpr int kRefineHeadSweeps = ILCC_K7R_HEAD_SWEEPS;
+constexpr int32_t kRefineSplitOneLaunch = ILCC_REFINE_SPLIT_ONE_LAUNCH, kRefineSplitRule = ILCC_REFINE_SPLIT_RULE;
 constexpr int kTieCap = 256;
 constexpr float kTieEps = 2e-5f;
 constexpr int kCoverageCellsMax = 1024;
@@ -93,6 +98,13 @@
   long long cost_q, alt_q;
   int32_t lat[3];
   int32_t phase, rounds, hops;
+};
+
+struct RefineResume {
+  int32_t lat[3];
+  int32_t phase, stride, r, rounds, hops, capped;
+  int32_t at;
+  int32_t flags, n_ties;
 };
 
 struct GridTables {
@@ -181,6 +193,9 @@
   const double2* th_lattice;
   int32_t th_lat_lo, th_lat_hi;
   int32_t refine_hop_y, refine_hop_z;
+  RefineResume* refine_resume;
+  uint32_t* refine_pending;
+  RefineOut* refine_io;
   ilcc_params p;
 };
 
@@ -299,7 +314,13 @@
 void launch_group_prepass(const Ctx& c, const GridPass& full, hipStream_t s);
 uint32_t grid_cost_evals_per_count();
 void launch_reference_solve(const Ctx& c, hipStream_t s);
-void launch_pattern_refine(const Ctx& c, hipStream_t s);
+struct RefineLaunch {
+  int32_t head_threads, tail_threads;
+  int32_t budget;
+  uint32_t head_lds, tail_lds;
+};
+RefineLaunch launch_pattern_refine(const Ctx& c, hipStream_t s, int32_t split = kRefineSplitRule);
+uint32_t refine_static_lds_bytes();
 void launch_corners(const Ctx& c, hipStream_t s, int n_slots);
 void launch_pack_records(const ilcc_result* d_res, uint32_t n_frames, uint32_t n_corners, uint32_t tag_base, float* d_out,
                          hipStream_t s);
diff --git a/lidar_camera_calibration_amd/csrc/k7_common.h b/lidar_camera_calibration_amd/csrc/k7_common.h
--- a/lidar_camera_calibration_amd/csrc/k7_common.h
+++ b/lidar_camera_calibration_amd/csrc/k7_common.h
@@ -43,8 +43,15 @@
   float2* yz;
   uint8_t* lab;
 };
-__host__ __device__ inline size_t staged_points_bytes(uint32_t cap, uint32_t frames) {
-  return (sizeof(float2) + 1) * (size_t)cap * (size_t)frames;
+constexpr uint32_t kActQueue = 128;
+__host__ __device__ inline size_t staged_queue_offset(uint32_t cap, uint32_t frames) {
+  return ((sizeof(float2) + 1) * (size_t)cap * (size_t)frames + 3u) & ~(size_t)3u;
+}
+__host__ __device__ inline size_t staged_points_bytes(uint32_t cap, uint32_t frames, uint32_t queue_waves = 0) {
+  if (queue_waves == 0) return (sizeof(float2) + 1) * (size_t)cap * (size_t)frames;
+  const size_t staged = staged_queue_offset(cap, frames) + sizeof(uint16_t) * kActQueue * (size_t)queue_waves;
+  const size_t unstaged = sizeof(uint32_t) * kActQueue * (size_t)queue_waves;
+  return staged > unstaged ? staged : unstaged;
 }
 __device__ __forceinline__ StagedPoints staged_points(unsigned char* smem, uint32_t cap, uint32_t frames, uint32_t k) {
   return StagedPoints{reinterpret_cast<float2*>(smem) + (size_t)k * cap,
diff --git a/lidar_camera_calibration_amd/csrc/k7r_pattern_refine.hip b/lidar_camera_calibration_amd/csrc/k7r_pattern_refine.hip
--- a/lidar_camera_calibration_amd/csrc/k7r_pattern_refine.hip
+++ b/lidar_camera_calibration_amd/csrc/k7r_pattern_refine.hip
@@ -16,22 +16,23 @@
 struct RCand {
   int32_t q0, q1, q2, phase;
 };
-constexpr int kRefineWavesMax = kRefineThreadsSmallBatch / ILCC_WAVE;
 constexpr double kExactDoubleSum = 9007199254740992.0;
-constexpr int kActQueue = 128;
 struct RefineShared {
   RCand cand[kRefineList];
   GridPartial meta[kRefineList];
   unsigned long long acc[3][kRefineList];
-  uint32_t queue[kRefineWavesMax][kActQueue];
-};
-
+};
+
+constexpr int32_t kAtSearchStart = 0, kAtRounds = 1, kAtBasin = 2;
 struct RefineState {
   int32_t lat[3];
   int32_t phase, rounds, hops, capped;
   int32_t skip_first;
+  int32_t stride, r;
+  int32_t at;
   long long cost, alt;
 };
+constexpr int kRefineWhole = 0, kRefineHead = 1, kRefineTail = 2;
 
 __device__ __forceinline__ bool partial_less(const GridPartial& a, const GridPartial& b) {
   return a.cost < b.cost || (a.cost == b.cost && (a.d2 < b.d2 || (a.d2 == b.d2 && a.flat < b.flat)));
@@ -119,11 +120,12 @@
   const uint8_t* lab;
   uint32_t n;
   RefineShared& sh;
+  void* queue;
   int sweep;
 };
-__device__ __forceinline__ Frame begin_frame(const Ctx& c, RefineShared& sh, const float2* yz, const uint8_t* lab, uint32_t n) {
+__device__ __forceinline__ Frame begin_frame(const Ctx& c, RefineShared& sh, void* queue, const float2* yz, const uint8_t* lab, uint32_t n) {
   if (threadIdx.x < kRefineList) sh.acc[0][threadIdx.x] = 0ull;
-  return Frame{c, make_board(c.p), Lattice(c), yz, lab, n, sh, 0};
+  return Frame{c, make_board(c.p), Lattice(c), yz, lab, n, sh, queue, 0};
 }
 
 __device__ __forceinline__ int sweep_begin(Frame& fr) {
@@ -161,6 +163,7 @@
   return buf;
 }
 
+template <typename QIdx>
 __device__ __forceinline__ int stencil_sweep(Frame& fr, int n_th, const int32_t th[3], const int32_t ty[3], const int32_t tz[3],
                                              int phase, bool parity) {
   const Ctx& c = fr.c;
@@ -207,7 +210,7 @@
           }
       };
       if (skip_silent) {
-        uint32_t* queue = fr.sh.queue[wid];
+        QIdx* queue = static_cast<QIdx*>(fr.queue) + (size_t)wid * kActQueue;
         uint32_t head = 0, tail = 0;
         const bool tlw0 = phase != 0;
         for (uint32_t base = (uint32_t)(grp * ILCC_WAVE); base < n; base += n_slices) {
@@ -224,20 +227,20 @@
           }
           const unsigned long long m = __ballot(active);
           if (m != 0ull) {
-            if (active) queue[(tail + (uint32_t)__popcll(m & ((1ull << lane) - 1ull))) & (kActQueue - 1)] = p;
+            if (active) queue[(tail + (uint32_t)__popcll(m & ((1ull << lane) - 1ull))) & (kActQueue - 1u)] = (QIdx)p;
             tail += (uint32_t)__popcll(m);
             __builtin_amdgcn_fence(__ATOMIC_RELEASE, "wavefront");
             __builtin_amdgcn_wave_barrier();
             __builtin_amdgcn_fence(__ATOMIC_ACQUIRE, "wavefront");
             while (tail - head >= (uint32_t)ILCC_WAVE) {
-              eval_point(queue[(head + (uint32_t)lane) & (kActQueue - 1)]);
+              eval_point((uint32_t)queue[(head + (uint32_t)lane) & (kActQueue - 1u)]);
               head += ILCC_WAVE;
             }
             __builtin_amdgcn_fence(__ATOMIC_RELEASE, "wavefront");
             __builtin_amdgcn_wave_barrier();
           }
         }
-        if ((uint32_t)lane < tail - head) eval_point(queue[(head + (uint32_t)lane) & (kActQueue - 1)]);
+        if ((uint32_t)lane < tail - head) eval_point((uint32_t)queue[(head + (uint32_t)lane) & (kActQueue - 1u)]);
         __builtin_amdgcn_fence(__ATOMIC_RELEASE, "wavefront");
         __builtin_amdgcn_wave_barrier();
       } else {
@@ -370,24 +373,27 @@
   return !risk && !(flags & ILCC_FLAG_TIE_OVERFLOW) && gk > 0 && gk < c.p.n_th - 1 && ga > 0 && ga < n_ty - 1 && gb > 0 && gb < n_tz - 1;
 }
 
-__device__ __forceinline__ void pattern_refine(Frame& fr, RefineState& st) {
+template <typename QIdx, bool BUDGETED>
+__device__ __forceinline__ bool pattern_refine(Frame& fr, RefineState& st, int budget) {
   const Ctx& c = fr.c;
   const RefineShared& sh = fr.sh;
   const bool refine = c.p.refine_div > 0;
   const int div = fr.lat.div;
-  st.rounds = 0;
-  st.hops = 0;
-  st.capped = 0;
-  st.cost = 0;
-  st.alt = 0;
   for (;;) {
-    int stride = div, r = 0;
-    if (st.skip_first && refine && div >= 2 && c.p.refine_max_rounds >= 1) {
-      stride = div >> 1;
-      r = 1;
-    }
-    st.skip_first = 0;
-    while (refine && stride >= 1 && r < c.p.refine_max_rounds) {
+    if (st.at == kAtSearchStart) {
+      st.stride = div;
+      st.r = 0;
+      if (st.skip_first && refine && div >= 2 && c.p.refine_max_rounds >= 1) {
+        st.stride = div >> 1;
+        st.r = 1;
+      }
+      st.skip_first = 0;
+      st.at = kAtRounds;
+    }
+    int& stride = st.stride;
+    int& r = st.r;
+    while (st.at == kAtRounds && refine && stride >= 1 && r < c.p.refine_max_rounds) {
+      if (BUDGETED && budget-- <= 0) return false;
       int32_t th[3], ty[3], tz[3];
 #pragma unroll
       for (int k = 0; k < 3; ++k) {
@@ -395,7 +401,7 @@
         ty[k] = st.lat[1] + (k - 1) * stride;
         tz[k] = st.lat[2] + (k - 1) * stride;
       }
-      const int b = stencil_sweep(fr, 3, th, ty, tz, st.phase, false);
+      const int b = stencil_sweep<QIdx>(fr, 3, th, ty, tz, st.phase, false);
       long long bc = LLONG_MAX;
       int bd2 = 0, be = -1;
       for (int e = 0; e < 27; ++e) {
@@ -420,12 +426,16 @@
         stride >>= 1;
       }
     }
-    st.rounds += r;
-    if (refine && stride >= 1) st.capped = 1;
+    if (st.at == kAtRounds) {
+      st.rounds += r;
+      if (refine && stride >= 1) st.capped = 1;
+      st.at = kAtBasin;
+    }
+    if (BUDGETED && budget-- <= 0) return false;
     const int32_t th1[3] = {st.lat[0], kNoTheta, kNoTheta};
     const int32_t hy[3] = {st.lat[1] - c.refine_hop_y, st.lat[1], st.lat[1] + c.refine_hop_y};
     const int32_t hz[3] = {st.lat[2] - c.refine_hop_z, st.lat[2], st.lat[2] + c.refine_hop_z};
-    const int b = stencil_sweep(fr, 1, th1, hy, hz, st.phase, true);
+    const int b = stencil_sweep<QIdx>(fr, 1, th1, hy, hz, st.phase, true);
     st.cost = (long long)sh.acc[b][4];
     long long alt = LLONG_MAX;
     int ae = -1;
@@ -444,9 +454,10 @@
       st.lat[1] += da * c.refine_hop_y;
       st.lat[2] += db * c.refine_hop_z;
       st.phase ^= (da + db) & 1;
+      st.at = kAtSearchStart;
       continue;
     }
-    break;
+    return true;
   }
 }
 
@@ -457,6 +468,39 @@
   st.lat[2] = at.q2;
   st.phase = at.phase;
   st.skip_first = skip_first ? 1 : 0;
+  st.rounds = st.hops = st.capped = 0;
+  st.stride = st.r = 0;
+  st.at = kAtSearchStart;
+  st.cost = st.alt = 0;
+  return st;
+}
+
+__device__ __forceinline__ void store_resume(const RefineState& st, int flags, uint32_t n_ties, RefineResume* out) {
+  RefineResume r;
+  r.lat[0] = st.lat[0];
+  r.lat[1] = st.lat[1];
+  r.lat[2] = st.lat[2];
+  r.phase = st.phase;
+  r.stride = st.stride;
+  r.r = st.r;
+  r.rounds = st.rounds;
+  r.hops = st.hops;
+  r.capped = st.capped;
+  r.at = st.at;
+  r.flags = flags;
+  r.n_ties = (int32_t)n_ties;
+  *out = r;
+}
+__device__ __forceinline__ RefineState load_resume(const RefineResume& r, int& flags, uint32_t& n_ties) {
+  RefineState st = start_at(RCand{r.lat[0], r.lat[1], r.lat[2], r.phase}, false);
+  st.stride = r.stride;
+  st.r = r.r;
+  st.rounds = r.rounds;
+  st.hops = r.hops;
+  st.capped = r.capped;
+  st.at = r.at;
+  flags = r.flags;
+  n_ties = (uint32_t)r.n_ties;
   return st;
 }
 
@@ -476,14 +520,28 @@
   out->cost_q = st.cost;
   out->alt_q = st.alt;
 }
-
-template <bool LDS_POINTS>
-__device__ __forceinline__ void refine_frame(const Ctx& c, SolveRec* rec, const StagedPoints& lds, RefineShared& sh) {
+__device__ __forceinline__ void store_outcome(const RefineState& st, RefineOut* io) {
+  io->lat[0] = st.lat[0];
+  io->lat[1] = st.lat[1];
+  io->lat[2] = st.lat[2];
+  io->phase = st.phase;
+  io->rounds = st.rounds;
+  io->hops = st.hops;
+  io->cost_q = st.cost;
+  io->alt_q = st.alt;
+}
+
+template <bool LDS_POINTS, int MODE>
+__device__ __forceinline__ void refine_frame(const Ctx& c, SolveRec* rec, unsigned char* smem, RefineShared& sh, int budget) {
+  constexpr int mode = MODE;
+  using QIdx = std::conditional_t<LDS_POINTS, uint16_t, uint32_t>;
   const uint32_t f = blockIdx.x;
   const uint64_t beg = c.off[f];
   SolveRec* out = &rec[2 * f];
-  Frame fr = begin_frame(c, sh, c.yz + beg, c.lab + beg, c.n_lab[f]);
+  void* queue = LDS_POINTS ? (void*)(smem + staged_queue_offset(c.grid_lds_points, 1)) : (void*)smem;
+  Frame fr = begin_frame(c, sh, queue, c.yz + beg, c.lab + beg, c.n_lab[f]);
   if (LDS_POINTS) {
+    const StagedPoints lds = staged_points(smem, c.grid_lds_points, 1, 0);
     for (uint32_t i = threadIdx.x; i < fr.n; i += blockDim.x) {
       lds.yz[i] = fr.yz[i];
       lds.lab[i] = fr.lab[i];
@@ -493,64 +551,105 @@
   }
   __syncthreads();
 
-  GridPartial b = grid_argmin(c, f);
-  if (b.flat == 0xFFFFFFFFu) {
-    if (threadIdx.x == 0) out->valid = 0;
-    return;
-  }
   int flags = 0;
-  const uint32_t n_ties = recount_near_ties(fr, f, b, flags);
+  uint32_t n_ties = 0;
+  RefineState st;
+  if (mode == kRefineTail) {
+    st = load_resume(c.refine_resume[f], flags, n_ties);
+  } else if (c.refine_io != nullptr) {
+    const RefineOut io = c.refine_io[f];
+    st = start_at(RCand{io.lat[0], io.lat[1], io.lat[2], io.phase}, false);
+  } else {
+    GridPartial b = grid_argmin(c, f);
+    if (b.flat == 0xFFFFFFFFu) {
+      if (threadIdx.x == 0) {
+        out->valid = 0;
+        if (mode == kRefineHead) c.refine_pending[f] = 0u;
+      }
+      return;
+    }
+    n_ties = recount_near_ties(fr, f, b, flags);
+    if (threadIdx.x == 0) {
+      c.res[f].grid_index = (int32_t)b.flat;
+      c.res[f].grid_cost = b.cost;
+    }
+    const GridCell start = fr.lat.from_flat(b.flat);
+    st = start_at(start.at, first_round_is_settled(fr, start, flags));
+  }
+  const bool done = pattern_refine<QIdx, MODE == kRefineHead>(fr, st, budget);
   if (threadIdx.x == 0) {
-    c.res[f].grid_index = (int32_t)b.flat;
-    c.res[f].grid_cost = b.cost;
-  }
-  const GridCell start = fr.lat.from_flat(b.flat);
-  RefineState st = start_at(start.at, first_round_is_settled(fr, start, flags));
-  pattern_refine(fr, st);
-  if (threadIdx.x == 0) store_record(fr.lat, st, flags, n_ties, out);
-}
-
-__global__ __launch_bounds__(kRefineThreadsSmallBatch) void k7r_pattern_refine(Ctx c, SolveRec* rec) {
+    if (done) {
+      store_record(fr.lat, st, flags, n_ties, out);
+      if (c.refine_io != nullptr) store_outcome(st, &c.refine_io[f]);
+    } else {
+      store_resume(st, flags, n_ties, &c.refine_resume[f]);
+    }
+    if (mode == kRefineHead) c.refine_pending[f] = done ? 0u : 1u;
+  }
+}
+
+template <int MODE>
+__global__ __launch_bounds__(kRefineThreadsSmallBatch) void k7r_pattern_refine(Ctx c, SolveRec* rec, int budget) {
+  constexpr int mode = MODE;
   extern __shared__ __align__(16) unsigned char smem[];
   __shared__ RefineShared sh;
   const uint32_t f = blockIdx.x;
-  if (c.res[f].status != ILCC_OK) {
-    if (threadIdx.x == 0) rec[2 * f].valid = 0;
+  if (mode == kRefineTail) {
+    if (c.refine_pending[f] == 0u) return;
+  } else if (c.res[f].status != ILCC_OK) {
+    if (threadIdx.x == 0) {
+      rec[2 * f].valid = 0;
+      if (mode == kRefineHead) c.refine_pending[f] = 0u;
+    }
     return;
   }
-  const StagedPoints lds = staged_points(smem, c.grid_lds_points, 1, 0);
   if (c.n_lab[f] <= c.grid_lds_points)
-    refine_frame<true>(c, rec, lds, sh);
+    refine_frame<true, MODE>(c, rec, smem, sh, budget);
   else
-    refine_frame<false>(c, rec, lds, sh);
+    refine_frame<false, MODE>(c, rec, smem, sh, budget);
 }
 
 __global__ __launch_bounds__(kRefineThreads) void k7r_pattern_refine_test(Ctx c, RefineOut* io) {
   __shared__ RefineShared sh;
-  Frame fr = begin_frame(c, sh, c.yz, c.lab, c.n_lab[0]);
+  __shared__ uint32_t queue[(kRefineThreads / ILCC_WAVE) * kActQueue];
+  Frame fr = begin_frame(c, sh, queue, c.yz, c.lab, c.n_lab[0]);
   RefineState st = start_at(RCand{io->lat[0], io->lat[1], io->lat[2], io->phase}, false);
   __syncthreads();
-  pattern_refine(fr, st);
-  if (threadIdx.x == 0) {
-    io->lat[0] = st.lat[0];
-    io->lat[1] = st.lat[1];
-    io->lat[2] = st.lat[2];
-    io->phase = st.phase;
-    io->rounds = st.rounds;
-    io->hops = st.hops;
-    io->cost_q = st.cost;
-    io->alt_q = st.alt;
-  }
+  (void)pattern_refine<uint32_t, false>(fr, st, 0);
+  if (threadIdx.x == 0) store_outcome(st, io);
 }
 
 hipError_t set_kernel_attributes_k7r() {
-  return hipFuncSetAttribute((const void*)k7r_pattern_refine, hipFuncAttributeMaxDynamicSharedMemorySize,
-                             (int)staged_points_bytes(kGridLdsPointsMax, 1));
-}
-
-void launch_pattern_refine(const Ctx& c, hipStream_t s) {
-  const int threads = c.n_frames <= (uint32_t)kSmallBatchFrames ? kRefineThreadsSmallBatch : kRefineThreads;
-  hipLaunchKernelGGL(k7r_pattern_refine, dim3(c.n_frames), dim3(threads), staged_points_bytes(c.grid_lds_points, 1), s, c, c.solve_rec);
+  const int lds = (int)staged_points_bytes(kGridLdsPointsMax, 1, kRefineThreadsSmallBatch / ILCC_WAVE);
+  for (const void* fn : {(const void*)k7r_pattern_refine<kRefineWhole>, (const void*)k7r_pattern_refine<kRefineHead>,
+                         (const void*)k7r_pattern_refine<kRefineTail>}) {
+    const hipError_t e = hipFuncSetAttribute(fn, hipFuncAttributeMaxDynamicSharedMemorySize, lds);
+    if (e != hipSuccess) return e;
+  }
+  return hipSuccess;
+}
+
+uint32_t refine_static_lds_bytes() {
+  hipFuncAttributes a{};
+  return hipFuncGetAttributes(&a, (const void*)k7r_pattern_refine<kRefineWhole>) == hipSuccess ? (uint32_t)a.sharedSizeBytes : 0u;
+}
+
+RefineLaunch launch_pattern_refine(const Ctx& c, hipStream_t s, int32_t split) {
+  auto launch = [&](int threads, int mode, int budget) {
+    const size_t lds = staged_points_bytes(c.grid_lds_points, 1, (uint32_t)(threads / ILCC_WAVE));
+    auto* fn = mode == kRefineWhole ? k7r_pattern_refine<kRefineWhole> : mode == kRefineHead ? k7r_pattern_refine<kRefineHead> : k7r_pattern_refine<kRefineTail>;
+    hipLaunchKernelGGL(fn, dim3(c.n_frames), dim3(threads), lds, s, c, c.solve_rec, budget);
+    return (uint32_t)lds;
+  };
+  const bool small = c.n_frames <= (uint32_t)kSmallBatchFrames;
+  if (small || split == kRefineSplitOneLaunch || (split == kRefineSplitRule && kRefineHeadSweeps < 0)) {
+    const int threads = small ? kRefineThreadsSmallBatch : kRefineThreads;
+    return RefineLaunch{threads, 0, kRefineSplitOneLaunch, launch(threads, kRefineWhole, 0), 0u};
+  }
+  const int budget = split == kRefineSplitRule ? kRefineHeadSweeps : split;
+  const uint32_t head_lds = launch(kRefineThreads, kRefineHead, budget);
+  const uint32_t tail_lds = launch(kRefineThreadsSmallBatch, kRefineTail, 0);
+  return RefineLaunch{kRefineThreads, kRefineThreadsSmallBatch, budget, head_lds, tail_lds};
 }
 
 void launch_pattern_refine_test(const Ctx& c, hipStream_t s, RefineOut* d_io) {
diff --git a/lidar_camera_calibration_amd/lidar_corners_est.py b/lidar_camera_calibration_amd/lidar_corners_est.py
--- a/lidar_camera_calibration_amd/lidar_corners_est.py
+++ b/lidar_camera_calibration_amd/lidar_corners_est.py
@@ -243,6 +243,42 @@
         if st != N.OK:
             raise IlccError(st, self._err())
         return dict(zip(("home", "lds_bytes", "threads", "static_lds_bytes", "lds_per_cu", "cus"), (int(v) for v in out)))
+
+    def debug_refine_split(self, head_sweeps: int):
+        st = self._lib.ilcc_debug_refine_split(self._h, int(head_sweeps))
+        if st != N.OK:
+            raise IlccError(st, self._err())
+
+    def debug_refine_launch(self) -> dict:
+        out = (C.c_int32 * N.REFINE_LAUNCH_WORDS)()
+        st = self._lib.ilcc_debug_refine_launch(self._h, out)
+        if st != N.OK:
+            raise IlccError(st, self._err())
+        return dict(zip(("head_threads", "tail_threads", "budget", "head_lds_bytes", "head_static_lds_bytes", "tail_lds_bytes",
+                         "tail_static_lds_bytes", "handed_over"), (int(v) for v in out)))
+
+    def debug_pattern_refine_batch(self, frames, lat, phase) -> dict:
+        f = len(frames)
+        offsets = np.zeros(f + 1, dtype=np.uint64)
+        offsets[1:] = np.cumsum([len(lab) for _, lab in frames], dtype=np.uint64)
+        yz = np.ascontiguousarray(np.concatenate([np.asarray(a, np.float32).reshape(-1, 2) for a, _ in frames] or
+                                                 [np.zeros((0, 2), np.float32)]), dtype=np.float32)
+        label = np.ascontiguousarray(np.concatenate([np.asarray(b, np.uint8).reshape(-1) for _, b in frames] or
+                                                    [np.zeros(0, np.uint8)]), dtype=np.uint8)
+        q = np.ascontiguousarray(np.asarray(lat, dtype=np.int32).reshape(-1, 3))
+        ph = np.ascontiguousarray(np.asarray(phase, dtype=np.int32).reshape(-1))
+        if len(q) != f or len(ph) != f:
+            raise IlccError(N.BAD_ARGUMENT, "debug_pattern_refine_batch: one start per frame")
+        cq, aq = np.zeros(f, np.int64), np.zeros(f, np.int64)
+        rounds, hops = np.zeros(f, np.int32), np.zeros(f, np.int32)
+        i32p, i64p = C.POINTER(C.c_int32), C.POINTER(C.c_int64)
+        st = self._lib.ilcc_debug_pattern_refine_batch(
+            self._h, N.fptr(yz), label.ctypes.data_as(C.POINTER(C.c_uint8)), offsets.ctypes.data_as(C.POINTER(C.c_uint64)), f,
+            q.ctypes.data_as(i32p), ph.ctypes.data_as(i32p), cq.ctypes.data_as(i64p), aq.ctypes.data_as(i64p),
+            rounds.ctypes.data_as(i32p), hops.ctypes.data_as(i32p))
+        if st != N.OK:
+            raise IlccError(st, self._err())
+        return dict(lat=q, phase=ph, cost_q=cq, alt_cost_q=aq, rounds=rounds, hops=hops)
 
     def wait_compact(self, ticket) -> np.ndarray:
         t, n_frames = ticket
```
